# TritonDataCenter/node-zkstream

Measured on AMD Instinct MI355X. Metric: ZK ops/sec (whole node) + p50 get() RTT, 1M-znode synthetic tree, higher is better.
Workload: dtype uint8

## Files before the change

### csrc/kernels/decode.hip

```cpp
#include "zk_common.h"

namespace zk {

constexpr int DEC_T = 256;

ZK_DEV void read_stat_regs(const uint32_t* w, const ZkReplyOut& o, int64_t i) {
  const int64_t c = o.cap;
  auto b32 = [&](int k) { return (int32_t)bswap32(w[k]); };
  auto b64 = [&](int k) {
    return (int64_t)(((uint64_t)bswap32(w[k]) << 32) | bswap32(w[k + 1]));
  };
  o.stat64[0 * c + i] = b64(0);
  o.stat64[1 * c + i] = b64(2);
  o.stat64[2 * c + i] = b64(4);
  o.stat64[3 * c + i] = b64(6);
  o.stat32[0 * c + i] = b32(8);
  o.stat32[1 * c + i] = b32(9);
  o.stat32[2 * c + i] = b32(10);
  o.stat64[4 * c + i] = b64(11);
  o.stat32[3 * c + i] = b32(13);
  o.stat32[4 * c + i] = b32(14);
  o.stat64[5 * c + i] = b64(15);
}

ZK_DEV bool read_stat(const uint8_t* p, const ZkReplyOut& o, int64_t i) {
  const int64_t c = o.cap;
  o.stat64[0 * c + i] = ld_be64(p + 0);
  o.stat64[1 * c + i] = ld_be64(p + 8);
  o.stat64[2 * c + i] = ld_be64(p + 16);
  o.stat64[3 * c + i] = ld_be64(p + 24);
  o.stat32[0 * c + i] = ld_be32(p + 32);
  o.stat32[1 * c + i] = ld_be32(p + 36);
  o.stat32[2 * c + i] = ld_be32(p + 40);
  o.stat64[4 * c + i] = ld_be64(p + 44);
  o.stat32[3 * c + i] = ld_be32(p + 52);
  o.stat32[4 * c + i] = ld_be32(p + 56);
  o.stat64[5 * c + i] = ld_be64(p + 60);
  return true;
}


struct ZkGetCheck {
  const int64_t* idx;
  const int32_t* xid;
  const int32_t* data_len;
  unsigned long long* acc;
  int32_t slots;
  int64_t* tick;
  const uint8_t* slab;
  const int64_t* slot_off;
};
constexpr int CHK_SAMPLE = 16;

ZK_DEV bool wave_bytes_equal(const uint8_t* a, const uint8_t* b, int32_t n,
                             int lane) {
  uint32_t diff = 0;
  for (int32_t o = 16 * lane; o < n; o += 1024) {
    const uintptr_t ua = (uintptr_t)(a + o);
    const uint32_t* wa = (const uint32_t*)(ua & ~(uintptr_t)3);
    const uint32_t sh = (uint32_t)(ua & 3);
    const uint32_t* wb = (const uint32_t*)(b + o);
    uint32_t va[5], vb[4];
#pragma unroll
    for (int q = 0; q < 5; ++q) va[q] = wa[q];
#pragma unroll
    for (int q = 0; q < 4; ++q) vb[q] = wb[q];
    const int32_t rem = n - o;
#pragma unroll
    for (int q = 0; q < 4; ++q) {
      const int32_t keep = rem - 4 * q;
      const uint32_t mask = keep >= 4 ? 0xFFFFFFFFu
                          : keep <= 0 ? 0u : (1u << (8 * keep)) - 1u;
      diff |= (__builtin_amdgcn_alignbyte(va[q + 1], va[q], sh) ^ vb[q]) &
              mask;
    }
  }
  return __ballot(diff != 0) == 0;
}

template <bool CHECK>
__global__ __launch_bounds__(DEC_T) void decode_replies_k(
    const uint8_t* __restrict__ buf, const int64_t* __restrict__ foff,
    const int32_t* __restrict__ flen, const int64_t* __restrict__ n_dev,
    int64_t ncap, const int64_t* __restrict__ xid_tab, int64_t xid_mask,
    ZkReplyOut o, ZkGetCheck chk) {
  const uint32_t nwg = gridDim.x;
  const int64_t i = (int64_t)xcd_remap(blockIdx.x, nwg) * DEC_T + threadIdx.x;
  const bool live = i < ncap && i < *n_dev;
  if (!CHECK && !live) return;
  int64_t good = 0;
  const int64_t salt = CHECK && chk.tick != nullptr ? chk.tick[1] : 0;
  bool samp = false;
  int64_t s_off = 0, s_node = 0;
  int32_t s_len = 0;
  if (live) {
  const uint8_t* p = buf + foff[i];
  const int64_t L = flen[i];
  int32_t status = ST_OK;
  int32_t op = OP_UNKNOWN;
  int64_t poff = -1;
  int32_t plen = 0, a0 = 0, a1 = 0;
  int32_t xid = 0, err = 0;
  int64_t zxid = 0;
  uint32_t hw[4] = {0, 0, 0, 0};
  if (L >= 16) __builtin_memcpy(hw, p, 16);
  const bool tail_ok = L >= 16 + STAT_BYTES;
  uint32_t sw[STAT_BYTES / 4];
  if (L < 16) {
    status = ST_BAD_DECODE;
  } else {
    xid = (int32_t)bswap32(hw[0]);
    zxid = (int64_t)(((uint64_t)bswap32(hw[1]) << 32) | bswap32(hw[2]));
    err = (int32_t)bswap32(hw[3]);
    switch (xid) {
      case XID_NOTIFICATION: op = OP_NOTIFICATION; break;
      case XID_PING: op = OP_PING; break;
      case XID_AUTH: op = OP_AUTH; break;
      case XID_SET_WATCHES: op = OP_SET_WATCHES; break;
      default: {
        const int64_t e = xid_tab[xid & xid_mask];
        if (xid >= 0 && (int32_t)(e >> 32) == xid) op = (int32_t)e;
        else status = ST_NO_XID;
      }
    }
  }
  if (tail_ok) __builtin_memcpy(sw, p + L - STAT_BYTES, STAT_BYTES);
  if (status == ST_OK && err == ERR_OK) {
    const uint8_t* b = p + 16;
    const int64_t A = L - 16;
    switch (op) {
      case OP_GET_DATA: {
        if (A < 4) { status = ST_BAD_DECODE; break; }
        int32_t dl = ld_be32(b);
        if (dl < 0) dl = 0;
        if (4 + (int64_t)dl + STAT_BYTES > A) { status = ST_BAD_DECODE; break; }
        poff = foff[i] + 20;
        plen = dl;
        if (tail_ok && 4 + (int64_t)dl + STAT_BYTES == A) read_stat_regs(sw, o, i);
        else read_stat(b + 4 + dl, o, i);
        break;
      }
      case OP_EXISTS: case OP_SET_DATA:
        if (A < STAT_BYTES) { status = ST_BAD_DECODE; break; }
        if (tail_ok && A == STAT_BYTES) read_stat_regs(sw, o, i);
        else read_stat(b, o, i);
        break;
      case OP_CREATE: {
        if (A < 4) { status = ST_BAD_DECODE; break; }
        int32_t l = ld_be32(b);
        if (l < 0) l = 0;
        if (4 + (int64_t)l > A) { status = ST_BAD_DECODE; break; }
        poff = foff[i] + 20;
        plen = l;
        break;
      }
      case OP_GET_CHILDREN: case OP_GET_CHILDREN2: {
        if (A < 4) { status = ST_BAD_DECODE; break; }
        const int32_t cnt = max(ld_be32(b), 0);
        const int64_t k = skip_strings(b + 4, A - 4, cnt);
        if (k < 0) { status = ST_BAD_DECODE; break; }
        if (op == OP_GET_CHILDREN2 && 4 + k + STAT_BYTES > A) {
          status = ST_BAD_DECODE;
          break;
        }
        poff = foff[i] + 20;
        plen = (int32_t)k;
        a0 = cnt;
        if (op == OP_GET_CHILDREN2) {
          if (tail_ok && 4 + k + STAT_BYTES == A) read_stat_regs(sw, o, i);
          else read_stat(b + 4 + k, o, i);
        }
        break;
      }
      case OP_GET_ACL: {
        if (A < 4) { status = ST_BAD_DECODE; break; }
        const int32_t cnt = max(ld_be32(b), 0);
        const int64_t k = skip_acl(b + 4, A - 4, cnt);
        if (k < 0 || 4 + k + STAT_BYTES > A) { status = ST_BAD_DECODE; break; }
        poff = foff[i] + 20;
        plen = (int32_t)k;
        a0 = cnt;
        if (tail_ok && 4 + k + STAT_BYTES == A) read_stat_regs(sw, o, i);
        else read_stat(b + 4 + k, o, i);
        break;
      }
      case OP_NOTIFICATION: {
        if (A < 12) { status = ST_BAD_DECODE; break; }
        int32_t l = ld_be32(b + 8);
        if (l < 0) l = 0;
        if (12 + (int64_t)l > A) { status = ST_BAD_DECODE; break; }
        a0 = ld_be32(b);
        a1 = ld_be32(b + 4);
        poff = foff[i] + 28;
        plen = l;
        break;
      }
      case OP_PING: case OP_SYNC: case OP_DELETE: case OP_SET_WATCHES:
      case OP_CLOSE_SESSION: case OP_AUTH:
        break;
      default:
        status = ST_BAD_OPCODE;
    }
  }
  o.xid[i] = xid;
  o.err[i] = err;
  o.opcode[i] = op;
  o.zxid[i] = zxid;
  o.status[i] = status;
  o.pay_off[i] = poff;
  o.pay_len[i] = plen;
  o.aux0[i] = a0;
  o.aux1[i] = a1;
  if (CHECK && status == ST_OK && err == ERR_OK && op == OP_GET_DATA) {
    const int64_t v = chk.idx[i];
    good = xid == chk.xid[i] && o.stat64[i] == v + 1 &&
           plen == chk.data_len[v];
    samp = good && chk.slab != nullptr && plen > 0 &&
           ((i + salt) & (CHK_SAMPLE - 1)) == 0;
    s_off = poff;
    s_node = v;
    s_len = plen;
  }
  }
  if (CHECK) {
    uint64_t pend = __ballot(samp);
    const int lane = threadIdx.x & 63;
    while (pend) {
      const int l = (int)__builtin_ctzll(pend);
      pend &= pend - 1;
      const int64_t po = __shfl(s_off, l, 64);
      const int64_t vn = __shfl(s_node, l, 64);
      const int32_t pl = __shfl(s_len, l, 64);
      const bool eq = wave_bytes_equal(
          buf + po, chk.slab + chk.slot_off[vn] + ZK_SLOT_DATA, pl, lane);
      if (lane == l && !eq) good = 0;
    }
    if (chk.tick != nullptr && blockIdx.x == 0 && threadIdx.x == 0)
      chk.tick[1] += 1;
    __shared__ int64_t sm[DEC_T / 64 + 1];
    int64_t tot;
    block_excl_scan(good, sm, &tot);
    if (threadIdx.x == 0 && tot)
      atomicAdd(&chk.acc[blockIdx.x % (uint32_t)chk.slots],
                (unsigned long long)tot);
  }
}

__global__ __launch_bounds__(DEC_T) void expand_strings_k(
    const uint8_t* __restrict__ buf, const int64_t* __restrict__ region,
    const int32_t* __restrict__ count, const int64_t* __restrict__ base,
    int64_t n, int64_t* __restrict__ soff, int32_t* __restrict__ slen) {
  const int64_t i = (int64_t)blockIdx.x * DEC_T + threadIdx.x;
  if (i >= n) return;
  const int32_t c = count[i];
  if (c <= 0 || region[i] < 0) return;
  int64_t k = region[i];
  int64_t w = base[i];
  for (int32_t j = 0; j < c; ++j) {
    int32_t l = ld_be32(buf + k);
    if (l < 0) l = 0;
    soff[w + j] = k + 4;
    slen[w + j] = l;
    k += 4 + l;
  }
}

__global__ __launch_bounds__(DEC_T) void expand_acl_k(
    const uint8_t* __restrict__ buf, const int64_t* __restrict__ region,
    const int32_t* __restrict__ count, const int64_t* __restrict__ base,
    int64_t n, int32_t* __restrict__ perms, int64_t* __restrict__ s_off,
    int32_t* __restrict__ s_len, int64_t* __restrict__ i_off,
    int32_t* __restrict__ i_len) {
  const int64_t i = (int64_t)blockIdx.x * DEC_T + threadIdx.x;
  if (i >= n) return;
  const int32_t c = count[i];
  if (c <= 0 || region[i] < 0) return;
  int64_t k = region[i];
  int64_t w = base[i];
  for (int32_t j = 0; j < c; ++j) {
    perms[w + j] = ld_be32(buf + k);
    k += 4;
    int32_t l = max(ld_be32(buf + k), 0);
    s_off[w + j] = k + 4;
    s_len[w + j] = l;
    k += 4 + l;
    l = max(ld_be32(buf + k), 0);
    i_off[w + j] = k + 4;
    i_len[w + j] = l;
    k += 4 + l;
  }
}

__global__ __launch_bounds__(DEC_T) void decode_requests_k(
    const uint8_t* __restrict__ buf, const int64_t* __restrict__ foff,
    const int32_t* __restrict__ flen, const int64_t* __restrict__ n_dev,
    int64_t ncap, ZkReqOut o) {
  const uint32_t nwg = gridDim.x;
  const int64_t i = (int64_t)xcd_remap(blockIdx.x, nwg) * DEC_T + threadIdx.x;
  if (i >= ncap || i >= *n_dev) return;
  const ReqFields f = parse_request(buf, foff[i], flen[i]);
  o.xid[i] = f.xid;
  o.opcode[i] = f.op;
  o.status[i] = f.status;
  o.path_off[i] = f.poff;
  o.path_len[i] = f.pl;
  o.data_off[i] = f.doff;
  o.data_len[i] = f.dl;
  o.arg[i] = f.arg;
  o.vec_off[i] = f.voff;
  o.vec_count[i] = f.vc;
  o.rel_zxid[i] = f.rel;
}

__global__ __launch_bounds__(DEC_T) void decode_connect_k(
    const uint8_t* __restrict__ buf, const int64_t* __restrict__ foff,
    const int32_t* __restrict__ flen, int64_t n, int32_t* __restrict__ proto,
    int32_t* __restrict__ tmo, int64_t* __restrict__ sid,
    int64_t* __restrict__ pw_off, int32_t* __restrict__ pw_len,
    int32_t* __restrict__ status) {
  const int64_t i = (int64_t)blockIdx.x * DEC_T + threadIdx.x;
  if (i >= n) return;
  const uint8_t* p = buf + foff[i];
  const int64_t L = flen[i];
  int32_t st = ST_OK, pv = 0, to = 0, pl = 0;
  int64_t s = 0, po = -1;
  if (L < 20) {
    st = ST_BAD_DECODE;
  } else {
    pv = ld_be32(p);
    to = ld_be32(p + 4);
    s = ld_be64(p + 8);
    int32_t l = ld_be32(p + 16);
    if (l < 0) l = 0;
    if (20 + (int64_t)l > L) st = ST_BAD_DECODE;
    else { po = foff[i] + 20; pl = l; }
  }
  proto[i] = pv; tmo[i] = to; sid[i] = s; pw_off[i] = po; pw_len[i] = pl;
  status[i] = st;
}

static inline unsigned nblk(int64_t n) {
  return (unsigned)((n + DEC_T - 1) / DEC_T);
}

}

extern "C" {

int zk_decode_replies(const uint8_t* buf, const int64_t* foff,
                      const int32_t* flen, const int64_t* n_dev, int64_t ncap,
                      const int64_t* xid_tab, int64_t xid_mask,
                      const ZkReplyOut* o, hipStream_t st) {
  if (ncap <= 0) return 0;
  zk::decode_replies_k<false><<<zk::nblk(ncap), zk::DEC_T, 0, st>>>(
      buf, foff, flen, n_dev, ncap, xid_tab, xid_mask, *o,
      zk::ZkGetCheck{nullptr, nullptr, nullptr, nullptr, 1, nullptr, nullptr,
                     nullptr});
  ZK_LAUNCH_CHECK();
  return 0;
}

int zk_decode_replies_check(const uint8_t* buf, const int64_t* foff,
                            const int32_t* flen, const int64_t* n_dev,
                            int64_t ncap, const int64_t* xid_tab,
                            int64_t xid_mask, const ZkReplyOut* o,
                            const int64_t* idx, const int32_t* xid,
                            const int32_t* data_len, unsigned long long* acc,
                            int32_t slots, int64_t* tick,
                            const uint8_t* slab, const int64_t* slot_off,
                            hipStream_t st) {
  if (ncap <= 0) return 0;
  if (slots < 1 || slots > 64) return (int)hipErrorInvalidValue;
  if ((slab == nullptr) != (slot_off == nullptr))
    return (int)hipErrorInvalidValue;
  zk::decode_replies_k<true><<<zk::nblk(ncap), zk::DEC_T, 0, st>>>(
      buf, foff, flen, n_dev, ncap, xid_tab, xid_mask, *o,
      zk::ZkGetCheck{idx, xid, data_len, acc, slots, tick, slab, slot_off});
  ZK_LAUNCH_CHECK();
  return 0;
}

int zk_expand_strings(const uint8_t* buf, const int64_t* region,
                      const int32_t* count, const int64_t* base, int64_t n,
                      int64_t* soff, int32_t* slen, hipStream_t st) {
  if (n <= 0) return 0;
  zk::expand_strings_k<<<zk::nblk(n), zk::DEC_T, 0, st>>>(buf, region, count,
                                                          base, n, soff, slen);
  ZK_LAUNCH_CHECK();
  return 0;
}

int zk_expand_acl(const uint8_t* buf, const int64_t* region,
                  const int32_t* count, const int64_t* base, int64_t n,
                  int32_t* perms, int64_t* s_off, int32_t* s_len,
                  int64_t* i_off, int32_t* i_len, hipStream_t st) {
  if (n <= 0) return 0;
  zk::expand_acl_k<<<zk::nblk(n), zk::DEC_T, 0, st>>>(
      buf, region, count, base, n, perms, s_off, s_len, i_off, i_len);
  ZK_LAUNCH_CHECK();
  return 0;
}

int zk_decode_connect_responses(const uint8_t* buf, const int64_t* foff,
                                const int32_t* flen, int64_t n,
                                int32_t* proto, int32_t* tmo, int64_t* sid,
                                int64_t* pw_off, int32_t* pw_len,
                                int32_t* status, hipStream_t st) {
  if (n <= 0) return 0;
  zk::decode_connect_k<<<zk::nblk(n), zk::DEC_T, 0, st>>>(
      buf, foff, flen, n, proto, tmo, sid, pw_off, pw_len, status);
  ZK_LAUNCH_CHECK();
  return 0;
}

int zk_decode_requests(const uint8_t* buf, const int64_t* foff,
                       const int32_t* flen, const int64_t* n_dev,
                       int64_t ncap, const ZkReqOut* o, hipStream_t st) {
  if (ncap <= 0) return 0;
  zk::decode_requests_k<<<zk::nblk(ncap), zk::DEC_T, 0, st>>>(
      buf, foff, flen, n_dev, ncap, *o);
  ZK_LAUNCH_CHECK();
  return 0;
}

}
```

### csrc/kernels/frame_scan.hip

```cpp
#include "zk_common.h"

namespace zk {

constexpr int FT_S = 4096;
constexpr int FT_LMAX = FT_S / 4;
constexpr int FT_STAGE = FT_S + 16;
constexpr int64_t TERM = (int64_t)1 << 62;
constexpr int64_t TBAD = (int64_t)1 << 60;
constexpr int64_t FC_MAXP = (int64_t)1 << 24;
constexpr int FC_WIN = 4096;
constexpr int FL_T = 512;
constexpr int FL_U = 8;
constexpr int FL_NB = 2;
constexpr int FL_GW = FL_NB + 1;
constexpr int FL_BROUNDS = 8;
constexpr int FL_DBG_BLOCKS = 16;
constexpr int FL_DBG_ROWS = 6;
constexpr uint32_t FL_CHASE_WALKS = 16;
constexpr int FK_T = 64;
constexpr int LW_MINS = 4, LW_LAST = 6, LW_NOSPEC = 7, LW_GRID = 8;
constexpr int LW_BIG = 16;
constexpr int LW_END = 32;
static_assert(LW_GRID + FL_GW <= LW_BIG, "grid words");
constexpr unsigned FL_BIG_NOSPEC = 256;
constexpr int FL_GROUNDS = 6;
constexpr uint64_t FT_WAIT_TICKS = 200000;

ZK_DEV int64_t stream_len(const int64_t* n_dev, int64_t n_cap) {
  if (n_dev == nullptr) return n_cap;
  const int64_t v = *n_dev;
  return v < 0 ? 0 : (v < n_cap ? v : n_cap);
}

ZK_DEV uint64_t lb_load(const uint64_t* p) {
  return __hip_atomic_load(p, __ATOMIC_RELAXED, __HIP_MEMORY_SCOPE_AGENT);
}
ZK_DEV void lb_store(uint64_t* p, uint64_t v) {
  __hip_atomic_store(p, v, __ATOMIC_RELAXED, __HIP_MEMORY_SCOPE_AGENT);
}
ZK_DEV int64_t ld_agent(const int64_t* p) {
  return __hip_atomic_load(p, __ATOMIC_RELAXED, __HIP_MEMORY_SCOPE_AGENT);
}
ZK_DEV void st_agent(int64_t* p, int64_t v) {
  __hip_atomic_store(p, v, __ATOMIC_RELAXED, __HIP_MEMORY_SCOPE_AGENT);
}

ZK_DEV void fc_stat(uint64_t* stats, int k, uint32_t v) {
  __hip_atomic_fetch_add((uint32_t*)&stats[k], v, __ATOMIC_RELAXED,
                         __HIP_MEMORY_SCOPE_AGENT);
}

ZK_DEV int32_t lds_be32(const uint8_t* sb, int32_t p) {
  const int32_t a = p & ~3;
  const uint32_t lo = *(const uint32_t*)(sb + a);
  const uint32_t hi = *(const uint32_t*)(sb + a + 4);
  return (int32_t)bswap32(__builtin_amdgcn_alignbyte(hi, lo, p & 3));
}

constexpr int FT_BITS = FT_S / 32;
constexpr int FT_XW = 2048 / 32;

struct FcWalk {
  int64_t exit;
  int32_t cnt;
  int32_t np;
  int32_t js;
  bool term, bad;
};
ZK_DEV int64_t fc_meta(const FcWalk& w) {
  return (int64_t)w.cnt | ((int64_t)w.np << 11) | ((int64_t)(w.js + 1) << 22) |
         ((int64_t)w.term << 33) | ((int64_t)w.bad << 34);
}
ZK_DEV int32_t m_cnt(int64_t m) { return (int32_t)(m & 0x7FF); }
ZK_DEV int32_t m_np(int64_t m) { return (int32_t)((m >> 11) & 0x7FF); }
ZK_DEV int32_t m_js(int64_t m) { return (int32_t)((m >> 22) & 0x7FF) - 1; }
ZK_DEV bool m_term(int64_t m) { return (m >> 33) & 1; }
ZK_DEV bool m_bad(int64_t m) { return (m >> 34) & 1; }
constexpr int64_t M_STALE = (int64_t)1 << 35;
ZK_DEV bool m_stale(int64_t m) { return (m >> 35) & 1; }

ZK_DEV void fc_join_end(FcWalk& r, int64_t send, int64_t n) {
  if (send & TERM) {
    const int64_t q = send & ~(TERM | TBAD);
    if (q >= n && !(send & TBAD)) {
      r.exit = n;
    } else {
      r.exit = q; r.term = true; r.bad = (send & TBAD) != 0;
    }
  } else {
    r.exit = send;
  }
}

template <typename LoadL>
ZK_DEV int32_t fc_member(uint32_t crel, int32_t m0, int32_t& lb, uint32_t& lv,
                         int lane, LoadL loadL) {
  while (lb + 64 < m0 &&
         crel > (uint32_t)__builtin_amdgcn_readlane((int)lv, 63)) {
    lb += 64;
    lv = lb + lane < m0 ? loadL(lb + lane) : 0xFFFFFFFFu;
  }
  const uint64_t hit = __ballot(lv == crel);
  return hit ? lb + (int32_t)__builtin_ctzll(hit) : -1;
}

ZK_DEV void ft_record(uint16_t* L, int32_t& m, uint32_t& ent, int32_t c,
                      int lane) {
  ent = lane == (m & 63) ? (uint32_t)c : ent;
  ++m;
  if ((m & 63) == 0) L[m - 64 + lane] = (uint16_t)ent;
}

constexpr int64_t FC_DEAD = -1;
constexpr int64_t FC_LIVE = -2;
constexpr int CX_SHIFT = 48;
ZK_DEV int64_t cx_exit(int64_t v) {
  return v < 0 ? v : v & (((int64_t)1 << CX_SHIFT) - 1);
}
ZK_DEV int32_t cx_cnt(int64_t v) { return v < 0 ? 0 : (int32_t)(v >> CX_SHIFT); }

ZK_DEV int64_t ft_cand(const uint8_t* sb, const uint32_t* sbits, int32_t e,
                       int32_t nrel, int32_t maxp, int64_t send, int64_t n,
                       int64_t ts, int32_t m, int lane) {
  int32_t c = e;
  int32_t hops = 0;
  for (;;) {
    if (c >= FT_S) return (ts + c) | ((int64_t)hops << CX_SHIFT);
    if (ts + c >= n) return FC_LIVE;
    const uint32_t smw = sbits[c >> 5];
    const int32_t lraw = lds_be32(sb, c);
    if ((smw >> (c & 31)) & 1u) {
      if (send & TERM) return (send & TBAD) ? FC_DEAD : FC_LIVE;
      const int32_t cw = c >> 5;
      int32_t below = 0;
#pragma unroll
      for (int h = 0; h < 2; ++h) {
        const int32_t wi = lane + 64 * h;
        const uint32_t wd = sbits[wi];
        below += wi < cw ? __popc(wd)
                         : (wi == cw ? __popc(wd & ((1u << (c & 31)) - 1u))
                                     : 0);
      }
#pragma unroll
      for (int d = 32; d >= 1; d >>= 1) below += __shfl_xor(below, d, 64);
      return send | ((int64_t)(hops + m - below) << CX_SHIFT);
    }
    if (c + 4 > nrel) return FC_LIVE;
    const int32_t len = __builtin_amdgcn_readfirstlane(lraw);
    if ((uint32_t)len > (uint32_t)maxp) return FC_DEAD;
    const int32_t nx = c + 4 + len;
    if (nx > nrel) return FC_LIVE;
    ++hops;
    c = nx;
  }
}

constexpr int FT_NMAX = 512;
constexpr int FT_SLOTS = 352;
constexpr int32_t FT_LIMIT = FT_S;
enum : uint32_t {
  RK_NODE = 0, RK_EXIT = 1, RK_END = 2, RK_PART = 3, RK_BAD = 4, RK_SHORT = 5
};
// ... 1107 lines not shown
        x0 = y0; x1 = y1; x2 = y2; x3 = y3;
      }
      {
        const bool c = r & 2;
        const uint4 y0 = sel(c, x2, x0), y1 = sel(c, x3, x1),
                    y2 = sel(c, x0, x2), y3 = sel(c, x1, x3);
        x0 = y0; x1 = y1; x2 = y2; x3 = y3;
      }
      d[0] = x0.x; d[1] = x0.y; d[2] = x0.z; d[3] = x0.w;
      d[4] = x1.x; d[5] = x1.y; d[6] = x1.z; d[7] = x1.w;
      d[8] = x2.x; d[9] = x2.y; d[10] = x2.z; d[11] = x2.w;
      d[12] = x3.x; d[13] = x3.y; d[14] = x3.z; d[15] = x3.w;
      const uint32_t nx = (uint32_t)__shfl_down((int)d[0], 1, 64);
      d[16] = lane == 63 ? pad : nx;
    }
    const uint32_t lim = P0 < W ? (uint32_t)(maxp32 - minb + 1)
                         : LONG ? (uint32_t)(FT_LIMIT - minb)
                                : (uint32_t)(W - 3 - minb);
    uint32_t lo = 0, hi = 0;
#pragma unroll
    for (int j = 0; j < 32; ++j) {
      const uint32_t v = (uint32_t)be32_of(d[j >> 2], d[(j >> 2) + 1], j);
      lo |= ((v - (uint32_t)minb) < lim ? 1u : 0u) << j;
    }
#pragma unroll
    for (int j = 32; j < 64; ++j) {
      const uint32_t v = (uint32_t)be32_of(d[j >> 2], d[(j >> 2) + 1], j);
      hi |= ((v - (uint32_t)minb) < lim ? 1u : 0u) << (j - 32);
    }
    uint64_t mask = (uint64_t)hi << 32 | lo;
    const int32_t room = nrel - 4 - P0;
    if (room < 63) mask = room < 0 ? 0 : mask & ((2ull << room) - 1);
    const uint32_t c = (uint32_t)__popcll(mask);
    uint32_t incl = c;
#pragma unroll
    for (int s = 1; s < 64; s <<= 1) {
      const uint32_t y = __shfl_up(incl, s, 64);
      if (lane >= s) incl += y;
    }
    N = __builtin_amdgcn_readlane((int)incl, 63);
    const uint32_t base = incl - c;
    bmask[lane] = mask;
    bbase[lane] = (uint16_t)base;
    if (N <= FT_NMAX) {
      uint32_t k = base;
      uint64_t m = mask;
      while (m) {
        C.pos[k++] = (uint16_t)(P0 + __builtin_ctzll(m));
        m &= m - 1;
      }
    }
  }
  __builtin_amdgcn_wave_barrier();
  C.t_d = dbg ? wall_clock64() : 0;
  C.buf = buf; C.list = list; C.pre = pre; C.sx = sx; C.lbw = lbw;
  C.rec_entry = rec_entry; C.rec_exit = rec_exit; C.rec_meta = rec_meta;
  C.rcount = rcount; C.dbg = dbg; C.cx = cx;
  C.stats = &lbw[2 * ntiles_cap];
  C.n = n; C.t = t; C.ts = ts; C.tend = tend;
  C.nrel = nrel; C.maxp32 = maxp32; C.minb = minb; C.N = N;
  C.nospec = tflags & 1;
  C.misspec = tflags >> 8;
  C.lane = lane;
  static_assert(FT_NMAX == 512, "node buckets");
  if constexpr (G > 1) {
    static_assert(!LONG, "groups: frames within the window");
    if (N <= 128) fs_group_rest<W, 2, G>(C);
    else if (N <= 256) fs_group_rest<W, 4, G>(C);
    else if (N <= FT_NMAX) fs_group_rest<W, 8, G>(C);
    else {
      const int64_t s0 = fs_tile_rest<W, LONG, 1>(C, false);
      FtTileRegs nxt;
      if (t + 1 < (n + FT_S - 1) / FT_S) ft_load(buf, n, ts + FT_S, lane, nxt);
      ft_group_tail<W, G>(C, s0, s0 >= 0, nxt);
    }
  } else {
    if (N <= 128) fs_tile_rest<W, LONG, 2>(C, true);
    else if (N <= 256) fs_tile_rest<W, LONG, 4>(C, true);
    else if (N <= FT_NMAX) fs_tile_rest<W, LONG, 8>(C, true);
    else fs_tile_rest<W, LONG, 1>(C, false);
  }
}


template <int WIN>
ZK_DEV void fc_stage(const uint8_t* __restrict__ buf, int64_t n, int64_t wb,
                     uint8_t* win, int lane) {
  constexpr int PER = WIN / 1024;
  uint4 v[PER];
#pragma unroll
  for (int j = 0; j < PER; ++j) {
    const int64_t g = wb + 16 * (lane + 64 * j);
    v[j] = make_uint4(0, 0, 0, 0);
    if (g + 16 <= n) {
      __builtin_memcpy(&v[j], buf + g, 16);
    } else if (g < n) {
      uint8_t* b = (uint8_t*)&v[j];
      for (int k = 0; k < 16; ++k) b[k] = g + k < n ? buf[g + k] : 0;
    }
  }
#pragma unroll
  for (int j = 0; j < PER; ++j) *(uint4*)(win + 16 * (lane + 64 * j)) = v[j];
  __builtin_amdgcn_wave_barrier();
  asm volatile("s_waitcnt lgkmcnt(0)" ::: "memory");
  __builtin_amdgcn_wave_barrier();
}

template <int WIN = FC_WIN>
ZK_DEV FcWalk fc_walk(const uint8_t* __restrict__ buf, int64_t n,
                      int64_t maxp, int64_t ts, int64_t E, const uint16_t* L,
                      int32_t m0, int64_t send, uint8_t* win, uint16_t* pre,
                      int lane) {
  FcWalk r{E, 0, 0, -1, false, false};
  const int64_t tend = ts + FT_S;
  int64_t c = E;
  int64_t wb = -(int64_t)WIN;
  int32_t lb = 0;
  uint32_t lv = lane < m0 ? (uint32_t)L[lane] : 0xFFFFFFFFu;
  int32_t np = 0;
  for (;;) {
    if (c >= tend) { r.exit = c; break; }
    if (c >= n) { r.exit = n; break; }
    const uint32_t crel = (uint32_t)(c - ts);
    if (m0 > 0) {
      const int32_t j = fc_member(crel, m0, lb, lv, lane,
                                  [&](int i) { return (uint32_t)L[i]; });
      if (j >= 0) { r.js = j; break; }
    }
    if (c + 4 > n) { r.exit = c; r.term = true; break; }
    if (c < wb || c + 8 > wb + WIN) {
      wb = c & ~(int64_t)15;
      fc_stage<WIN>(buf, n, wb, win, lane);
    }
    const int32_t len =
        __builtin_amdgcn_readfirstlane(lds_be32(win, (int32_t)(c - wb)));
    if (len < 0 || (int64_t)len > maxp) {
      r.exit = c; r.term = true; r.bad = true; break;
    }
    const int64_t nx = c + 4 + len;
    if (nx > n) { r.exit = c; r.term = true; break; }
    if (lane == 0) pre[np] = (uint16_t)crel;
    ++np;
    c = nx;
  }
  r.np = np;
  r.cnt = np;
  if (r.js >= 0) {
    r.cnt = np + (m0 - r.js);
    fc_join_end(r, send, n);
  }
  return r;
}

constexpr unsigned long long FL_SMALL = 1024;

ZK_DEV int64_t rfl64(int64_t v) {
  const uint32_t lo = (uint32_t)__builtin_amdgcn_readfirstlane((int)(uint32_t)v);
  const uint32_t hi =
      (uint32_t)__builtin_amdgcn_readfirstlane((int)(uint32_t)((uint64_t)v >> 32));
  return (int64_t)(((uint64_t)hi << 32) | lo);
}

ZK_DEV bool fl_accept(const int64_t* rec_entry, const int64_t* rec_exit,
                      int64_t ntiles, int64_t k, int64_t E, int64_t x) {
  if (ld_agent(&rec_exit[k - 1]) != E) return false;
  if (k < 2) return true;
  const bool suspect = ld_agent(&rec_entry[k - 1]) != ld_agent(&rec_exit[k - 2]);
  if (!suspect) return true;
  const int64_t ox = ld_agent(&rec_exit[k]);
  if (x == ox || k + 1 >= ntiles) return true;
  return ld_agent(&rec_entry[k + 1]) != ox;
}

ZK_DEV uint32_t fl_local_round(const uint8_t* __restrict__ buf, int64_t n,
                               int64_t ntiles, int64_t maxp,
                               const int64_t* __restrict__ sx,
                               const uint16_t* __restrict__ list,
                               const int32_t* __restrict__ rcount,
                               uint16_t* pre, int64_t* rec_entry,
                               int64_t* rec_exit, int64_t* rec_meta,
                               const int32_t* lloc, int nloc, uint8_t* win) {
  const int lane = threadIdx.x & 63, wv = threadIdx.x >> 6;
  uint8_t* mywin = win + (size_t)wv * (FC_WIN + 16);
  uint32_t walked = 0;
  for (int j = wv; j < nloc; j += FL_T / 64) {
    const int64_t k = lloc[j];
    const int64_t E = rfl64(ld_agent(&rec_exit[k - 1]));
    if (E < k * FT_S ||
        __builtin_amdgcn_readfirstlane(m_term(ld_agent(&rec_meta[k - 1]))))
// ... 104 lines not shown
    if (E < k * FT_S) continue;
    const int32_t m0 = __builtin_amdgcn_readfirstlane(rcount[k]);
    const FcWalk fw = fc_walk(buf, n, maxp, k * FT_S, E, list + k * FT_LMAX,
                              m0, sx[k], mywin, pre + k * FT_LMAX, lane);
    ++walked;
    if (lane == 0) {
      if (fl_accept(rec_entry, rec_exit, ntiles, k, E, fw.exit)) {
        st_agent(&rec_entry[k], E);
        st_agent(&rec_exit[k], fw.exit);
        st_agent(&rec_meta[k], fc_meta(fw));
      } else {
        st_agent(&rec_entry[k], -1);
      }
    }
  }
  if (lane == 0 && walked) fc_stat(stats, 2, walked);
  if (bid == 0 && tid == 0) fc_stat(stats, 3, 1);
  return fl_sync(g);
}

ZK_DEV void fl_check(int64_t ntiles, const int64_t* __restrict__ rec_entry,
                     const int64_t* __restrict__ rec_exit,
                     const int64_t* __restrict__ rec_meta, int64_t* base,
                     int64_t* bsum, uint64_t* mins,
                     unsigned long long* nbroken, int32_t* blist) {
  const int lane = threadIdx.x & 63;
  const int64_t INF = INT64_MAX;
  const int64_t nw = (int64_t)gridDim.x * (FL_T / 64);
  const int64_t nbl = (ntiles + FK_T - 1) / FK_T;
  int64_t fb = INF, fterm = INF;
  for (int64_t b = (int64_t)blockIdx.x * (FL_T / 64) + (threadIdx.x >> 6);
       b < nbl; b += nw) {
    const int64_t k = b * FK_T + lane;
    int64_t cnt = 0;
    bool brk = false;
    if (k < ntiles) {
      const int64_t mk = rec_meta[k];
      const bool nxt = k + 1 < ntiles;
      const int64_t e = nxt ? rec_entry[k + 1] : 0;
      const int64_t x = rec_exit[k];
      cnt = m_cnt(mk);
      if (m_term(mk)) {
        fterm = min(fterm, k);
      } else if (nxt && (e < 0 || e != x)) {
        brk = true;
        fb = min(fb, k + 1);
      }
    }
    const uint64_t bm = __ballot(brk);
    if (bm) {
      unsigned long long b0 = 0;
      if (lane == 0) b0 = atomicAdd(nbroken, (unsigned long long)__popcll(bm));
      b0 = __shfl(b0, 0, 64);
      if (brk) {
        const uint64_t below = lane ? (bm & ((~0ull) >> (64 - lane))) : 0ull;
        __hip_atomic_store(&blist[b0 + __popcll(below)], (int32_t)(k + 1),
                           __ATOMIC_RELAXED, __HIP_MEMORY_SCOPE_AGENT);
      }
    }
    int64_t inc = cnt;
#pragma unroll
    for (int d = 1; d < 64; d <<= 1) {
      const int64_t v = __shfl_up(inc, d, 64);
      if (lane >= d) inc += v;
    }
    if (k < ntiles) st_agent(&base[k], inc - cnt);
    if (lane == 63) st_agent(&bsum[b], inc);
  }
  for (int d = 32; d >= 1; d >>= 1) {
    fb = min(fb, (int64_t)__shfl_xor(fb, d, 64));
    fterm = min(fterm, (int64_t)__shfl_xor(fterm, d, 64));
  }
  if (lane == 0) {
    if (fb != INF) atomicMax((unsigned long long*)&mins[0],
                             (unsigned long long)(ntiles - fb));
    if (fterm != INF) atomicMax((unsigned long long*)&mins[1],
                                (unsigned long long)(ntiles - fterm));
  }
}

ZK_DEV void fl_bases(int64_t n, int64_t ntiles, int64_t ft,
                     const int64_t* rec_exit, const int64_t* rec_meta,
                     const int64_t* base, int64_t* bsum, int64_t cap,
                     int64_t* result, int64_t* lastk, int64_t* red) {
  const int tid = threadIdx.x;
  const int64_t INF = INT64_MAX;
  const int64_t last = ft == INF ? ntiles - 1 : ft;
  const int64_t nbl = last / FK_T + 1;
  const int64_t per = (nbl + FL_T - 1) / FL_T;
  const int64_t b0 = (int64_t)tid * per;
  const int64_t b1 = min(b0 + per, nbl);
  int64_t sum = 0;
  for (int64_t b = b0; b < b1; ++b) sum += ld_agent(&bsum[b]);
  int64_t tot;
  int64_t run = block_excl_scan(sum, red, &tot);
  const int64_t blast = last / FK_T;
  for (int64_t b = b0; b < b1; ++b) {
    const int64_t v = ld_agent(&bsum[b]);
    bsum[b] = run;
    if (b == blast) {
      const int64_t ml = ld_agent(&rec_meta[last]);
      const int64_t total = run + ld_agent(&base[last]) + m_cnt(ml);
      *lastk = last;
      result[0] = total;
      result[3] = total > cap ? 1 : 0;
      if (ft == INF) {
        result[1] = n;
        result[2] = 0;
      } else {
        result[1] = ld_agent(&rec_exit[ft]);
        result[2] = m_bad(ml) ? 1 : 0;
      }
    }
    run += v;
  }
}

constexpr int FL_WL = 1024;
constexpr int FL_HS = 2048;
constexpr int FL_WR = 48;
constexpr int FL_DB = 8192;
static_assert(FL_SMALL <= FL_WL, "the check's list fits the first round");

struct FlChase {
  uint32_t* dirty;
  int* overflow;
  uint64_t* stats;
  int64_t* clk;
};

ZK_DEV void fl_dirty(FlChase& ch, int64_t t) {
  const int64_t b = t / FK_T;
  if (b < FL_DB) atomicOr(&ch.dirty[b >> 5], 1u << (b & 31));
}

ZK_DEV int live_count(const int64_t* c5) {
  int live = 0;
#pragma unroll
  for (int j = 0; j < 5; ++j) live += c5[j] != FC_DEAD;
  return live;
}


ZK_DEV uint64_t readlane64(uint64_t v, int l) {
  const uint32_t lo = (uint32_t)__builtin_amdgcn_readlane((int)(uint32_t)v, l);
  const uint32_t hi =
      (uint32_t)__builtin_amdgcn_readlane((int)(uint32_t)(v >> 32), l);
  return ((uint64_t)hi << 32) | lo;
}

ZK_DEV int64_t fl_chase_run(const uint8_t* __restrict__ buf, int64_t n,
                            int64_t ntiles, int64_t maxp,
                            const int64_t* __restrict__ sx,
                            const uint16_t* __restrict__ list,
                            const int32_t* __restrict__ rcount, uint16_t* pre,
                            int64_t* rec_entry, int64_t* rec_exit,
                            int64_t* rec_meta, const uint64_t* lbw,
                            const int64_t* cx,
                            uint8_t* mywin, FlChase& ch, int64_t k0,
                            bool exact, bool& term, uint32_t& walked,
                            uint32_t walk_budget = 0) {
  const int lane = threadIdx.x & 63;
  term = false;
  k0 = rfl64(k0);
  exact = __builtin_amdgcn_readfirstlane((int)exact) != 0;
  int64_t k = k0;
  int64_t E = rfl64(ld_agent(&rec_exit[k - 1]));
  if (E < k * FT_S ||
      __builtin_amdgcn_readfirstlane(m_term(ld_agent(&rec_meta[k - 1]))))
    return -1;
  if (!exact && rfl64(ld_agent(&rec_entry[k])) == E) return -1;
  bool first = true;
  for (;;) {
    if (E >= (k + 1) * FT_S) {
      if (!exact) return k - 1;
      const int64_t kend = min(E / FT_S, ntiles);
      const FcWalk cov{E, 0, 0, -1, false, false};
      for (int64_t c = k + lane; c < kend; c += 64) {
        st_agent(&rec_entry[c], E);
        st_agent(&rec_exit[c], E);
        st_agent(&rec_meta[c], fc_meta(cov));
        fl_dirty(ch, c);
      }
      if (kend >= ntiles) return kend - 1;
      k = kend;
      first = false;
      continue;
    }
    const int64_t tl = k + lane;
    const int64_t ts_l = tl * FT_S;
    uint64_t wd = 0;
    int64_t en = INT64_MIN, ent = INT64_MIN, ox = INT64_MIN + 1;
    int64_t c5[5];
    int32_t n5[5];
#pragma unroll
    for (int j = 0; j < 5; ++j) {
// ... 165 lines not shown
    ++rounds;
    const int nxt = cur ^ 1;
    for (int i = tid; i < FL_HS; i += FL_T) hs[i] = 0;
    if (tid == 0) s_n = 0;
    __syncthreads();
    auto push = [&](int64_t k) {
      const uint32_t key = (uint32_t)k + 1;
      uint32_t h = (key * 2654435761u) >> (32 - 11);
      for (;;) {
        const uint32_t old = atomicCAS(&hs[h], 0u, key);
        if (old == 0) break;
        if (old == key) return;
        h = (h + 1) & (FL_HS - 1);
      }
      const int i = atomicAdd(&s_n, 1);
      if (i < FL_WL) wl[nxt][i] = (int32_t)k;
      else *ch.overflow = 1;
    };
    int32_t lo = INT32_MAX;
    for (int j = lane; j < ncur; j += 64) lo = min(lo, wl[cur][j]);
    for (int d = 32; d >= 1; d >>= 1) lo = min(lo, __shfl_xor(lo, d, 64));
    for (int j = wv; j < ncur; j += FL_T / 64) {
      bool term;
      const bool ex = wl[cur][j] == lo;
      if (ex && ch.clk && lane == 0) ch.clk[6] = wall_clock64();
      const int64_t kend = fl_chase_run(buf, n, ntiles, maxp, sx, list,
                                        rcount, pre, rec_entry, rec_exit,
                                        rec_meta, lbw, cx, mywin,
                                        ch, wl[cur][j], wl[cur][j] == lo,
                                        term, walked);
      if (ex && ch.clk && lane == 0) ch.clk[7] = wall_clock64();
      if (lane == 0)
        wk[j] = kend < 0 ? 0 : (int32_t)(kend + 1) | (term ? (1 << 30) : 0);
    }
    __syncthreads();
    for (int j = tid; j < ncur; j += FL_T) {
      const int64_t k0 = wl[cur][j];
      if (ld_agent(&rec_entry[k0]) != ld_agent(&rec_exit[k0 - 1]) &&
          !m_term(ld_agent(&rec_meta[k0 - 1])))
        push(k0);
      const int32_t e = wk[j];
      if (e == 0 || (e & (1 << 30))) continue;
      const int64_t kend = (e & ((1 << 30) - 1)) - 1;
      if (kend + 1 < ntiles &&
          ld_agent(&rec_entry[kend + 1]) != ld_agent(&rec_exit[kend]))
        push(kend + 1);
    }
    __syncthreads();
    if (tid == 0) s_cur = *ch.overflow ? -1 : s_n;
    __syncthreads();
    ncur = s_cur;
    cur = nxt;
    __syncthreads();
    if (ncur < 0) break;
  }
  if (lane == 0 && walked) fc_stat(stats, 2, walked);
  if (tid == 0 && rounds) fc_stat(stats, 3, rounds);
  return ncur == 0 && !*ch.overflow;
}

ZK_DEV void fl_chase_recount(int64_t ntiles, const int64_t* rec_meta,
                             int64_t* base, int64_t* bsum, FlChase& ch) {
  static_assert(FK_T == 64, "a count block is a wave");
  const int lane = threadIdx.x & 63, wv = threadIdx.x >> 6;
  const int64_t nbl = (ntiles + FK_T - 1) / FK_T;
  for (int64_t b = wv; b < nbl; b += FL_T / 64) {
    if (!((ch.dirty[b >> 5] >> (b & 31)) & 1u)) continue;
    const int64_t k = b * FK_T + lane;
    const int64_t c = k < ntiles ? m_cnt(ld_agent(&rec_meta[k])) : 0;
    int64_t inc = c;
    for (int d = 1; d < 64; d <<= 1) {
      const int64_t v = __shfl_up(inc, d, 64);
      if (lane >= d) inc += v;
    }
    if (k < ntiles) st_agent(&base[k], inc - c);
    if (lane == 63) st_agent(&bsum[b], inc);
  }
  __syncthreads();
}

ZK_DEV void fl_count_scan(int64_t n, int64_t ntiles, int64_t ft,
                          const int64_t* rec_exit, const int64_t* rec_meta,
                          int64_t* base, int64_t* bsum, int64_t cap,
                          int64_t* result, int64_t* lastk, int64_t* red) {
  const int tid = threadIdx.x;
  const int64_t INF = INT64_MAX;
  const int64_t last = ft == INF ? ntiles - 1 : ft;
  const int64_t per = (last + 1 + FL_T - 1) / FL_T;
  const int64_t k0 = (int64_t)tid * per;
  const int64_t k1 = min(k0 + per, last + 1);
  int64_t sum = 0;
  for (int64_t kb = k0; kb < k1; kb += FL_U) {
    int64_t v[FL_U];
#pragma unroll
    for (int u = 0; u < FL_U; ++u)
      v[u] = kb + u < k1 ? ld_agent(&rec_meta[kb + u]) : 0;
#pragma unroll
    for (int u = 0; u < FL_U; ++u) sum += m_cnt(v[u]);
  }
  int64_t tot;
  int64_t run = block_excl_scan(sum, red, &tot);
  for (int64_t kb = k0; kb < k1; kb += FL_U) {
    int64_t v[FL_U];
#pragma unroll
    for (int u = 0; u < FL_U; ++u)
      v[u] = kb + u < k1 ? ld_agent(&rec_meta[kb + u]) : 0;
#pragma unroll
    for (int u = 0; u < FL_U; ++u) {
      if (kb + u < k1) base[kb + u] = run;
      run += m_cnt(v[u]);
    }
  }
  for (int64_t k = last + 1 + tid; k < ntiles; k += FL_T) base[k] = -1;
  for (int64_t b = tid; b <= last / FK_T; b += FL_T) bsum[b] = 0;
  if (tid == 0) {
    *lastk = last;
    result[0] = tot;
    result[3] = tot > cap ? 1 : 0;
    if (ft == INF) {
      result[1] = n;
      result[2] = 0;
    } else {
      const int64_t mf = ld_agent(&rec_meta[ft]);
      result[1] = ld_agent(&rec_exit[ft]);
      result[2] = m_term(mf) && m_bad(mf) ? 1 : 0;
    }
  }
}

ZK_DEV void fl_links(int64_t from, int64_t ntiles,
                     const int64_t* rec_entry, const int64_t* rec_exit,
                     const int64_t* rec_meta, int64_t* red, int64_t& fb_out,
                     int64_t& ft_out) {
  const int tid = threadIdx.x, lane = tid & 63, wv = tid >> 6;
  const int64_t INF = INT64_MAX;
  int64_t fb = INF, fterm = INF;
  for (int64_t k0 = max(from - 1, (int64_t)0) + tid; k0 < ntiles;
       k0 += FL_U * FL_T) {
    int64_t mk[FL_U], e[FL_U], x[FL_U];
#pragma unroll
    for (int u = 0; u < FL_U; ++u) {
      const int64_t k = k0 + (int64_t)u * FL_T;
      const bool in = k < ntiles, nx = k + 1 < ntiles;
      mk[u] = in ? ld_agent(&rec_meta[k]) : 0;
      e[u] = nx ? ld_agent(&rec_entry[k + 1]) : 0;
      x[u] = in ? ld_agent(&rec_exit[k]) : 0;
    }
#pragma unroll
    for (int u = 0; u < FL_U; ++u) {
      const int64_t k = k0 + (int64_t)u * FL_T;
      if (k >= ntiles) break;
      if (m_term(mk[u])) {
        fterm = min(fterm, k);
      } else if (k + 1 < ntiles && k + 1 >= from) {
        if (e[u] < 0 || e[u] != x[u]) fb = min(fb, k + 1);
      }
    }
  }
  for (int d = 32; d >= 1; d >>= 1) {
    fb = min(fb, (int64_t)__shfl_xor(fb, d, 64));
    fterm = min(fterm, (int64_t)__shfl_xor(fterm, d, 64));
  }
  if (lane == 0) { red[wv] = fb; red[FL_T / 64 + wv] = fterm; }
  __syncthreads();
  fb = INF;
  fterm = INF;
  for (int j = 0; j < FL_T / 64; ++j) {
    fb = min(fb, red[j]);
    fterm = min(fterm, red[FL_T / 64 + j]);
  }
  __syncthreads();
  fb_out = fb;
  ft_out = fterm;
}

ZK_DEV int64_t fl_list_broken(int64_t ntiles, const int64_t* rec_entry,
                              const int64_t* rec_exit, const int64_t* rec_meta,
                              int32_t* blist, int64_t* red, int64_t& fb_out,
                              int64_t& ft_out) {
  const int tid = threadIdx.x, lane = tid & 63, wv = tid >> 6;
  const int64_t INF = INT64_MAX;
  const int64_t per = (ntiles + FL_T - 1) / FL_T;
  const int64_t k0 = (int64_t)tid * per, k1 = min(k0 + per, ntiles);
  int64_t cnt = 0, fb = INF, fterm = INF;
  for (int pass = 0; pass < 2; ++pass) {
    int64_t w = 0;
    if (pass == 1) {
      int64_t tot;
      w = block_excl_scan(cnt, red, &tot);
      red[2 * (FL_T / 64) + 1] = tot;
      if (cnt == 0) break;
    }
    for (int64_t kb = k0; kb < k1; kb += FL_U) {
      int64_t mp[FL_U], mk[FL_U], e[FL_U], x[FL_U];
#pragma unroll
      for (int u = 0; u < FL_U; ++u) {
        const int64_t k = kb + u;
        const bool in = k < k1;
        mk[u] = in ? ld_agent(&rec_meta[k]) : 0;
        mp[u] = in && k >= 1 ? ld_agent(&rec_meta[k - 1]) : 0;
        e[u] = in ? ld_agent(&rec_entry[k]) : 0;
        x[u] = in && k >= 1 ? ld_agent(&rec_exit[k - 1]) : 0;
      }
#pragma unroll
      for (int u = 0; u < FL_U; ++u) {
        const int64_t k = kb + u;
        if (k >= k1) break;
        const bool brk = k >= 1 && !m_term(mp[u]) && e[u] != x[u];
        if (pass == 0) {
          if (brk) { ++cnt; fb = min(fb, k); }
          if (m_term(mk[u])) fterm = min(fterm, k);
        } else if (brk) {
          blist[w++] = (int32_t)k;
        }
      }
    }
  }
  __syncthreads();
  const int64_t total = red[2 * (FL_T / 64) + 1];
  __syncthreads();
  for (int d = 32; d >= 1; d >>= 1) {
    fb = min(fb, (int64_t)__shfl_xor(fb, d, 64));
    fterm = min(fterm, (int64_t)__shfl_xor(fterm, d, 64));
  }
  if (lane == 0) { red[wv] = fb; red[FL_T / 64 + wv] = fterm; }
  __syncthreads();
  fb = INF;
  fterm = INF;
  for (int j = 0; j < FL_T / 64; ++j) {
    fb = min(fb, red[j]);
    fterm = min(fterm, red[FL_T / 64 + j]);
  }
  __syncthreads();
  fb_out = fb;
  ft_out = fterm;
  return total;
}

__global__ __launch_bounds__(FL_T) void fs_link(
    const uint8_t* __restrict__ buf, const int64_t* __restrict__ n_dev,
    int64_t n_cap, int64_t maxp, const int64_t* __restrict__ sx,
    const uint16_t* __restrict__ list, const int32_t* __restrict__ rcount,
    uint16_t* pre, int64_t* rec_entry, int64_t* rec_exit, int64_t* rec_meta,
    int64_t* __restrict__ base, int64_t cap, int64_t* __restrict__ result,
    uint64_t* stats, int32_t* __restrict__ blist,
    int64_t* __restrict__ bsum, uint64_t* mins,
    int64_t* __restrict__ lastk, unsigned long long* g,
    const uint64_t* lbw, const int64_t* __restrict__ cx,
    int64_t* __restrict__ ldbg) {
  __shared__ __attribute__((aligned(16)))
      uint8_t win[(FL_T / 64) * (FC_WIN + 16)];
  __shared__ int64_t red[2 * (FL_T / 64) + 2];
  __shared__ int64_t s_next;
  const int tid = threadIdx.x, lane = tid & 63, wv = tid >> 6;
  const int64_t n = stream_len(n_dev, n_cap);
  const int64_t ntiles = (n + FT_S - 1) / FT_S;
  if (ntiles == 0) {
    if (blockIdx.x == 0) {
      if (tid < 4) result[tid] = 0;
      if (tid == 0) *lastk = -1;
    }
    return;
  }
  const int64_t INF = INT64_MAX;
  const int64_t t_in = ldbg != nullptr ? wall_clock64() : 0;
  fl_check(ntiles, rec_entry, rec_exit, rec_meta, base, bsum, mins, &g[FL_NB],
           blist);
  if (ldbg != nullptr && tid == 0 && blockIdx.x < FL_DBG_BLOCKS) {
    ldbg[8 + 2 * blockIdx.x] = t_in;
    ldbg[8 + 2 * blockIdx.x + 1] = wall_clock64();
  }
  const bool big = (uint32_t)ld_agent((const int64_t*)&stats[LW_NOSPEC]) >
                   FL_BIG_NOSPEC;
  if (big) {
    unsigned long long* gb = (unsigned long long*)(stats + LW_BIG);
    bool ok = fl_sync(gb);
    for (int r = 0; r < FL_GROUNDS && ok; ++r)
      ok = fl_round(buf, n, ntiles, maxp, sx, list, rcount, pre, rec_entry,
                    rec_exit, rec_meta, blist, gb, r, red, win, stats);
    if (blockIdx.x != 0) return;
    __syncthreads();
    if (tid == 0) {
      gb[2] = 0;
      for (int r = 0; r < FL_GROUNDS; ++r) gb[4 + 2 * r] = 0;
    }
  }
  __shared__ int s_last;
  __syncthreads();
  if (big) {
    if (tid == 0) s_last = 1;
  } else if (tid == 0) {
    __threadfence();
    const unsigned long long a = __hip_atomic_fetch_add(
        &g[0], 1ull, __ATOMIC_ACQ_REL, __HIP_MEMORY_SCOPE_AGENT);
    const int last = a + 1 == gridDim.x;
    if (last)
      __hip_atomic_store(&g[0], 0ull, __ATOMIC_RELAXED,
                         __HIP_MEMORY_SCOPE_AGENT);
    __threadfence();
    s_last = last;
  }
  __syncthreads();
  if (!s_last) return;
  const uint64_t mb0 = ld_agent((const int64_t*)&mins[0]);
  const uint64_t mt0 = ld_agent((const int64_t*)&mins[1]);
  const unsigned long long nb0 = __hip_atomic_load(
      &g[FL_NB], __ATOMIC_RELAXED, __HIP_MEMORY_SCOPE_AGENT);
  const int64_t fb0 = mb0 ? ntiles - (int64_t)mb0 : INF;
  const int64_t ft0 = mt0 ? ntiles - (int64_t)mt0 : INF;
  if (!big && (fb0 == INF || fb0 > ft0)) {
    if (ldbg != nullptr && tid == 0) ldbg[40] = wall_clock64();
    fl_bases(n, ntiles, ft0, rec_exit, rec_meta, base, bsum, cap, result,
             lastk, red);
    if (ldbg != nullptr && tid == 0) ldbg[41] = wall_clock64();
    return;
  }
  __shared__ uint32_t dirty[FL_DB / 32];
  __shared__ int s_ovf;
  FlChase ch{dirty, &s_ovf, stats, ldbg};
  for (int i = tid; i < FL_DB / 32; i += FL_T) dirty[i] = 0;
  if (tid == 0) s_ovf = 0;
  __syncthreads();
  const bool clk = ldbg != nullptr && tid == 0;
  if (clk) ldbg[5] = t_in;
  int64_t from = 1, ft = INF;
  int64_t nb = (int64_t)nb0;
  bool changed = big;
  if (!big && nb > (int64_t)FL_SMALL && fb0 != INF) {
    if (wv == 0) {
      bool term = false;
      uint32_t walked = 0;
      const int64_t kend = fl_chase_run(buf, n, ntiles, maxp, sx, list, rcount,
                                        pre, rec_entry, rec_exit, rec_meta, lbw,
                                        cx, win, ch, fb0, true, term, walked,
                                        FL_CHASE_WALKS);
      (void)kend;
      if (lane == 0) {
        if (walked) fc_stat(stats, 2, walked);
        fc_stat(stats, 3, 1);
      }
    }
    __syncthreads();
    changed = true;
  }
  for (int round = 0; round < FL_BROUNDS; ++round) {
    if (changed) {
      int64_t fbv, ftv;
      nb = fl_list_broken(ntiles, rec_entry, rec_exit, rec_meta, blist, red,
                          fbv, ftv);
      if (fbv == INF || fbv > ftv) {
        fl_count_scan(n, ntiles, ftv, rec_exit, rec_meta, base, bsum, cap,
                      result, lastk, red);
        if (clk) ldbg[4] = wall_clock64() | (2ll << 56);
        return;
      }
    }
    if (nb <= (int64_t)FL_SMALL && (ntiles + FK_T - 1) / FK_T <= FL_DB) {
      if (clk && round == 0) ldbg[0] = wall_clock64();
      const bool settled = fl_chase(buf, n, ntiles, maxp, sx, list, rcount,
                                    pre, rec_entry, rec_exit, rec_meta, lbw,
                                    cx, blist, (int)nb, win, stats, ch);
      if (clk && round == 0) ldbg[1] = ldbg[2] = wall_clock64();
      int64_t fbv, ftv;
      fl_links(1, ntiles, rec_entry, rec_exit, rec_meta, red, fbv, ftv);
      if (clk && round == 0) ldbg[3] = wall_clock64();
      if (settled && (fbv == INF || fbv > ftv)) {
        if (changed) {
          fl_count_scan(n, ntiles, ftv, rec_exit, rec_meta, base, bsum, cap,
                        result, lastk, red);
          if (clk) ldbg[4] = wall_clock64() | (2ll << 56);
          return;
        }
        fl_chase_recount(ntiles, rec_meta, base, bsum, ch);
        fl_bases(n, ntiles, ftv, rec_exit, rec_meta, base, bsum, cap, result,
                 lastk, red);
        if (clk) ldbg[4] = wall_clock64() | (1ll << 56);
        return;
      }
      if (!settled) break;
    } else {
      const uint32_t w = fl_local_round(buf, n, ntiles, maxp, sx, list,
                                        rcount, pre, rec_entry, rec_exit,
                                        rec_meta, blist, (int)nb, win);
      if (lane == 0 && w) fc_stat(stats, 2, w);
      if (tid == 0) fc_stat(stats, 3, 1);
      __syncthreads();
    }
    changed = true;
  }
  for (;;) {
    int64_t fb, fterm;
    fl_links(from, ntiles, rec_entry, rec_exit, rec_meta, red, fb, fterm);
    if (fb == INF || fb > fterm) {
      ft = fterm;
      break;
    }
    if (wv == 0) {
      bool term = false;
      uint32_t walked = 0;
      const int64_t kend = fl_chase_run(buf, n, ntiles, maxp, sx, list, rcount,
                                        pre, rec_entry, rec_exit, rec_meta, lbw,
                                        cx, win, ch, fb, true, term, walked);
      if (lane == 0) {
        s_next = kend < fb ? -fb : kend + 1;
        if (walked) fc_stat(stats, 2, walked);
        fc_stat(stats, 3, 1);
      }
    }
    __syncthreads();
    from = s_next;
    __syncthreads();
    if (from < 0) {
      ft = -from - 1;
      break;
    }
  }
  fl_count_scan(n, ntiles, ft, rec_exit, rec_meta, base, bsum, cap, result,
                lastk, red);
  if (clk) ldbg[4] = wall_clock64() | (3ll << 56);
}

__global__ __launch_bounds__(256) void fs_rows(
    const uint8_t* __restrict__ buf, const int64_t* __restrict__ n_dev,
    int64_t n_cap, const uint16_t* __restrict__ list,
    const uint16_t* __restrict__ pre, const int64_t* __restrict__ rec_meta,
    const int64_t* __restrict__ rec_entry,
    const int64_t* __restrict__ rec_exit,
    const int64_t* __restrict__ base, const int64_t* __restrict__ bsum,
    const int64_t* __restrict__ lastk, int64_t* __restrict__ foff,
    int32_t* __restrict__ flen, int64_t cap, uint64_t* __restrict__ lbw,
    uint64_t* __restrict__ lbw_tail) {
  __shared__ __attribute__((aligned(16))) uint8_t stage[4][FT_STAGE];
  const int lane = threadIdx.x & 63;
  const int wv = __builtin_amdgcn_readfirstlane((int)(threadIdx.x >> 6));
  const int64_t t = (int64_t)blockIdx.x * 4 + wv;
  const int64_t n = stream_len(n_dev, n_cap);
  if (t == 0) {
    if (lane == 0) {
      lbw_tail[LW_MINS] = 0;
      lbw_tail[LW_MINS + 1] = 0;
      lbw_tail[LW_NOSPEC] = 0;
      lbw_tail[LW_GRID + FL_NB] = 0;
    }
    if (lane < LW_END - LW_BIG) lbw_tail[LW_BIG + lane] = 0;
  }
  if (t * FT_S >= n) return;
  if (lane == 0) {
    lbw[2 * t] = 0;
    lbw[2 * t + 1] = 0;
  }
  if (t > *lastk) return;
  const int64_t b = bsum[t / FK_T] + base[t];
  const int64_t m = rec_meta[t];
  const int64_t x = rec_exit[t];
  const int32_t cnt = m_cnt(m), np = m_np(m), js = m_js(m);
  const int64_t ts = t * FT_S;
  const uint16_t* P = pre + t * FT_LMAX;
  const uint16_t* R = list + t * FT_LMAX + (js < 0 ? 0 : js);
  if (m_stale(m)) {
    uint8_t* sb = stage[wv];
    fc_stage<FT_S>(buf, n, ts, sb, lane);
    if (lane == 0) {
      uint8_t* pb = sb + FT_S;
      for (int k = 0; k < 16; ++k)
        pb[k] = ts + FT_S + k < n ? buf[ts + FT_S + k] : 0;
    }
    __builtin_amdgcn_wave_barrier();
    asm volatile("s_waitcnt lgkmcnt(0)" ::: "memory");
    int32_t c = __builtin_amdgcn_readfirstlane((int32_t)(rec_entry[t] - ts));
    int32_t ent = 0;
    for (int32_t k = 0; k < cnt; ++k) {
      ent = lane == (k & 63) ? c : ent;
      const int32_t len = __builtin_amdgcn_readfirstlane(lds_be32(sb, c));
      c += 4 + len;
      if ((k & 63) == 63 || k == cnt - 1) {
        const int32_t last = k & 63;
        const int32_t nxt = __shfl_down(ent, 1, 64);
        if (lane <= last) {
          const int64_t p = ts + ent;
          const int64_t q = lane < last ? ts + nxt
                                        : (k == cnt - 1 ? x : ts + c);
          const int64_t idx = b + (k & ~63) + lane;
          if (idx < cap) {
            foff[idx] = p + 4;
            flen[idx] = (int32_t)(q - p - 4);
          }
        }
      }
    }
    return;
  }
  for (int32_t k = lane; k < cnt; k += 64) {
    const int64_t p = ts + (k < np ? P[k] : R[k - np]);
    const int32_t k1 = k + 1;
    const int64_t q = k1 < cnt ? ts + (k1 < np ? P[k1] : R[k1 - np]) : x;
    const int64_t idx = b + k;
    if (idx < cap) {
      foff[idx] = p + 4;
      flen[idx] = (int32_t)(q - p - 4);
    }
  }
}

__global__ __launch_bounds__(64) void fs_small(
    const uint8_t* __restrict__ buf, const int64_t* __restrict__ n_dev,
    int64_t n_cap, int64_t maxp, int64_t* __restrict__ foff,
    int32_t* __restrict__ flen, int64_t cap, int64_t* __restrict__ result) {
  __shared__ __attribute__((aligned(16))) uint8_t sb[FT_STAGE];
  const int lane = threadIdx.x;
  const int64_t n = stream_len(n_dev, n_cap);
  fc_stage<FT_S>(buf, n, 0, sb, lane);
  int32_t c = 0, k = 0;
  bool bad = false;
  const int32_t n32 = (int32_t)n;
  while (c + 4 <= n32) {
    const int32_t len = __builtin_amdgcn_readfirstlane(lds_be32(sb, c));
    if (len < 0 || (int64_t)len > maxp) { bad = true; break; }
    if (c + 4 + len > n32) break;
    if (lane == 0 && k < cap) {
      foff[k] = c + 4;
      flen[k] = len;
    }
    ++k;
    c += 4 + len;
  }
  if (lane == 0) {
    result[0] = k;
    result[1] = c;
    result[2] = bad ? 1 : 0;
    result[3] = k > cap ? 1 : 0;
  }
}

struct FsPlan {
  int64_t tiles;
  size_t off_list, off_pre, off_sx, off_lbw, off_rent, off_rexit, off_rmeta,
      off_rcnt, off_base, off_blist, off_bsum, off_cx, total;
};

static FsPlan fs_plan(int64_t n) {
  FsPlan p{};
  const int64_t tiles = n > 0 ? (n + FT_S - 1) / FT_S : 1;
  p.tiles = tiles;
  size_t o = 0;
  auto take = [&](size_t bytes) { size_t r = o; o += (bytes + 255) & ~(size_t)255; return r; };
  p.off_list = take((size_t)tiles * FT_LMAX * 2);
  p.off_pre = take((size_t)tiles * FT_LMAX * 2);
  p.off_sx = take((size_t)tiles * 8);
  p.off_lbw = take((size_t)(2 * tiles + LW_END) * 8);
  p.off_rent = take((size_t)tiles * 8);
  p.off_rexit = take((size_t)tiles * 8);
  p.off_rmeta = take((size_t)tiles * 8);
  p.off_rcnt = take((size_t)tiles * 4);
  p.off_base = take((size_t)tiles * 8);
  p.off_blist = take((size_t)tiles * 4);
  p.off_bsum = take((size_t)(tiles / FK_T + 1) * 8);
  p.off_cx = take((size_t)tiles * 5 * 8);
  p.total = o;
  return p;
}

static unsigned fl_blocks() { return 16; }

static int32_t fs_minb() { return 8; }

constexpr int32_t FS_LONG = 2;

constexpr int32_t FS_WIN_LONG = 1 << 16;

constexpr int FS_TPB = 4;

static int fs_window(int32_t window) {
  window &= FS_WIN_LONG - 1;
  return window <= 256 ? 256 : window <= 512 ? 512
       : window <= 1024 ? 1024 : 2048;
}

static int64_t* g_dbg = nullptr;
static int64_t g_dbg_tiles = 0;
static int64_t* fs_dbg_buf(int64_t tiles) {
  static int on = -1;
  if (on < 0) on = getenv("ZKMI_FS_DBG") != nullptr;
  if (!on) return nullptr;
  if (tiles > g_dbg_tiles) {
    if (g_dbg) (void)hipFree(g_dbg);
    if (hipMalloc(&g_dbg, (tiles + FL_DBG_ROWS) * 8 * 8) != hipSuccess)
      return nullptr;
    (void)hipMemset(g_dbg, 0, (tiles + FL_DBG_ROWS) * 8 * 8);
    g_dbg_tiles = tiles;
  }
  return g_dbg;
}

}

extern "C" {

int64_t zk_frame_scan_workspace(int64_t n) {
  return (int64_t)zk::fs_plan(n).total;
}

int zk_frame_scan(const uint8_t* buf, const int64_t* n_dev, int64_t n_cap,
                  int64_t maxp, uint8_t* ws, int64_t ws_bytes, int64_t* foff,
                  int32_t* flen, int64_t cap, int64_t* result, int32_t window,
                  int32_t clean, int32_t flags, hipStream_t st) {
  using namespace zk;
  const int W = fs_window(window);
  if (window & FS_WIN_LONG) flags |= FS_LONG;
  if (maxp > FC_MAXP || maxp < 0) return -3;
  FsPlan p = fs_plan(n_cap);
  if ((int64_t)p.total > ws_bytes) return -1;
  const int64_t tiles = p.tiles;
  if (n_cap <= FT_S && !(flags & (1 | 0xFFFF00)) &&
      fs_dbg_buf(tiles) == nullptr) {
    fs_small<<<1, 64, 0, st>>>(buf, n_dev, n_cap, maxp, foff, flen, cap,
                               result);
    ZK_LAUNCH_CHECK();
    return 0;
  }
  uint16_t* list = (uint16_t*)(ws + p.off_list);
  uint16_t* pre = (uint16_t*)(ws + p.off_pre);
  int64_t* sx = (int64_t*)(ws + p.off_sx);
  uint64_t* lbw = (uint64_t*)(ws + p.off_lbw);
  int64_t* rent = (int64_t*)(ws + p.off_rent);
  int64_t* rexit = (int64_t*)(ws + p.off_rexit);
  int64_t* rmeta = (int64_t*)(ws + p.off_rmeta);
  int32_t* rcnt = (int32_t*)(ws + p.off_rcnt);
  int64_t* base = (int64_t*)(ws + p.off_base);
  int32_t* blist = (int32_t*)(ws + p.off_blist);
  int64_t* bsum = (int64_t*)(ws + p.off_bsum);
  int64_t* cx = (int64_t*)(ws + p.off_cx);
  uint64_t* mins = lbw + 2 * tiles + LW_MINS;
  int64_t* lastk = (int64_t*)(lbw + 2 * tiles + LW_LAST);
  unsigned long long* grid = (unsigned long long*)(lbw + 2 * tiles + LW_GRID);
  if (!clean &&
      hipMemsetAsync(lbw, 0, (size_t)(2 * tiles + LW_END) * 8, st) !=
          hipSuccess)
    return -4;
  int64_t* dbg = fs_dbg_buf(tiles);
  constexpr int tpb = FS_TPB;
  int G = ((flags >> 4) & 15) + 1;
  if ((flags & (FS_LONG | 1 | 0xFFFF00)) || W > 512) G = 1;
  G = G >= 8 ? 8 : G >= 4 ? 4 : G >= 2 ? 2 : 1;
  const int64_t waves = (tiles + G - 1) / G;
  const unsigned tblocks = (unsigned)((waves + tpb - 1) / tpb);
#define ZK_FS_TILE(WW, LL)                                                   \
  fs_tile<WW, LL, 1><<<tblocks, 64 * tpb, FT_LDS * tpb, st>>>(               \
      buf, n_dev, n_cap, maxp, list, pre, sx, lbw, rent, rexit, rmeta, rcnt, \
      tiles, dbg, fs_minb(), flags, cx)
#define ZK_FS_GROUP(WW, GG)                                                  \
  fs_tile<WW, false, GG><<<tblocks, 64 * tpb, FT_LDS * tpb, st>>>(           \
      buf, n_dev, n_cap, maxp, list, pre, sx, lbw, rent, rexit, rmeta, rcnt, \
      tiles, dbg, fs_minb(), flags, cx)
  if (G == 8) {
    if (W == 256) ZK_FS_GROUP(256, 8);
    else ZK_FS_GROUP(512, 8);
  } else if (G == 4) {
    if (W == 256) ZK_FS_GROUP(256, 4);
    else ZK_FS_GROUP(512, 4);
  } else if (G == 2) {
    if (W == 256) ZK_FS_GROUP(256, 2);
    else ZK_FS_GROUP(512, 2);
  } else if (flags & FS_LONG) {
    switch (W) {
      case 256: ZK_FS_TILE(256, true); break;
      case 512: ZK_FS_TILE(512, true); break;
      case 1024: ZK_FS_TILE(1024, true); break;
      default: ZK_FS_TILE(2048, true); break;
    }
  } else {
    switch (W) {
      case 256: ZK_FS_TILE(256, false); break;
      case 512: ZK_FS_TILE(512, false); break;
      case 1024: ZK_FS_TILE(1024, false); break;
      default: ZK_FS_TILE(2048, false); break;
    }
  }
#undef ZK_FS_TILE
#undef ZK_FS_GROUP
  ZK_LAUNCH_CHECK();
  fs_link<<<fl_blocks(), FL_T, 0, st>>>(buf, n_dev, n_cap, maxp, sx, list, rcnt,
                                 pre, rent, rexit, rmeta, base, cap, result,
                                 lbw + 2 * tiles, blist, bsum, mins, lastk,
                                 grid, lbw, cx, dbg ? dbg + 8 * tiles : nullptr);
  ZK_LAUNCH_CHECK();
  fs_rows<<<(unsigned)((tiles + 3) / 4), 256, 0, st>>>(
      buf, n_dev, n_cap, list, pre, rmeta, rent, rexit, base, bsum, lastk,
      foff, flen, cap, lbw, lbw + 2 * tiles);
  ZK_LAUNCH_CHECK();
  return 0;
}

int zk_frame_scan_stats(const uint8_t* ws, int64_t n_cap, int32_t window,
                        uint32_t* out4, hipStream_t st) {
  using namespace zk;
  (void)window;
  FsPlan p = fs_plan(n_cap);
  const uint64_t* lbw = (const uint64_t*)(ws + p.off_lbw);
  for (int k = 0; k < 4; ++k)
    if (hipMemcpyAsync(out4 + k, lbw + 2 * p.tiles + (k + 1) % 4, 4,
                       hipMemcpyDeviceToHost, st) != hipSuccess)
      return -1;
  if (hipStreamSynchronize(st) != hipSuccess) return -1;
  if (hipMemsetAsync((void*)(lbw + 2 * p.tiles), 0, 4 * 8, st) !=
      hipSuccess)
    return -1;
  return hipStreamSynchronize(st) == hipSuccess ? 0 : -1;
}

int zk_frame_scan_dbg(int64_t* host, int64_t tiles) {
  if (!zk::g_dbg || tiles > zk::g_dbg_tiles + zk::FL_DBG_ROWS) return -1;
  return hipMemcpy(host, zk::g_dbg, tiles * 8 * 8, hipMemcpyDeviceToHost) ==
                 hipSuccess ? 0 : -1;
}

}
```

### csrc/kernels/tree.hip

```cpp
#include "zk_tree.h"

namespace zk {

__global__ __launch_bounds__(TR_T) void tree_fill_k(ZkTree t, int64_t n0,
                                                   int64_t n,
                                                   const int32_t* __restrict__ nkids,
                                                   int64_t now_ms) {
  const int64_t v = n0 + (int64_t)blockIdx.x * TR_T + threadIdx.x;
  if (v >= n) return;
  const ZkNodeStore& s = t.store;
  uint8_t* slot = s.slab + s.slot_off[v];
  const int32_t dl = s.data_len[v];
  fill_stat(slot, v + 1, v + 1, now_ms, now_ms, 0, nkids[v], 0, 0, dl,
            nkids[v], v + 1);
  st_be32(slot + 68, 0);
  st_be32(slot + ZK_SLOT_LEN, dl > 0 ? dl : -1);
  t.cn[v] = cn_pack(nkids[v], nkids[v]);
  t.pzxid[v] = v + 1;
  t.eph[v] = 0;
  t.dirty[v] = 0;
}

__global__ __launch_bounds__(TR_T) void free_count_k(ZkTree t,
                                                    int64_t* __restrict__ bsum) {
  __shared__ int32_t c[TR_T / 64];
  const int64_t nn = min(t.counters[TC_NODES], t.store.cap);
  const int64_t v = (int64_t)blockIdx.x * TR_T + threadIdx.x;
  const bool f = v < nn && t.node_parent[v] == NODE_FREE;
  const uint64_t m = __ballot(f);
  if ((threadIdx.x & 63) == 0) c[threadIdx.x >> 6] = __popcll(m);
  __syncthreads();
  if (threadIdx.x == 0) {
    int64_t s = 0;
    for (int k = 0; k < TR_T / 64; ++k) s += c[k];
    bsum[blockIdx.x] = s;
  }
}

__global__ __launch_bounds__(TR_T) void free_scatter_k(
    ZkTree t, const int64_t* __restrict__ bbase,
    const int64_t* __restrict__ total) {
  __shared__ int32_t c[TR_T / 64];
  const int64_t head = t.counters[TC_FREE_HEAD];
  const int64_t nn = min(t.counters[TC_NODES], t.store.cap);
  const int64_t v = (int64_t)blockIdx.x * TR_T + threadIdx.x;
  const bool f = v < nn && t.node_parent[v] == NODE_FREE;
  const uint64_t m = __ballot(f);
  const int w = threadIdx.x >> 6;
  if ((threadIdx.x & 63) == 0) c[w] = __popcll(m);
  __syncthreads();
  int64_t r = bbase[blockIdx.x] +
              __builtin_amdgcn_mbcnt_hi((uint32_t)(m >> 32),
                                        __builtin_amdgcn_mbcnt_lo((uint32_t)m, 0));
  for (int k = 0; k < w; ++k) r += c[k];
  if (f) t.free_list[(head + r) % t.free_cap] = v;
  if (blockIdx.x == 0 && threadIdx.x == 0) {
    t.counters[TC_FREE_TAIL] = head + *total;
    t.counters[TC_FREE_PUB] = head + *total;
  }
}

__global__ __launch_bounds__(TR_T) void tree_build_k(ZkTree t, int64_t n0,
                                                    int64_t n) {
  const int64_t v = n0 + (int64_t)blockIdx.x * TR_T + threadIdx.x;
  if (v >= n || t.node_parent[v] == NODE_FREE) return;
  tree_insert(t, v, t.path_arena + t.node_path_off[v], t.node_path_len[v],
              t.store.data_len[v]);
}

}

extern "C" {

int zk_tree_fill(const ZkTree* t, int64_t n0, int64_t n, const int32_t* nkids,
                 int64_t now_ms, hipStream_t st) {
  if (n <= n0) return 0;
  const int64_t m = n - n0;
  zk::tree_fill_k<<<(unsigned)((m + zk::TR_T - 1) / zk::TR_T), zk::TR_T, 0,
                    st>>>(*t, n0, n, nkids, now_ms);
  ZK_LAUNCH_CHECK();
  return 0;
}

// ... 45 lines not shown
  int64_t node, zx, par, slot;
  const uint8_t* path;
};

ZK_DEV int64_t served_reply_size(int32_t op, int32_t err, int32_t dl,
                                 int32_t rpl) {
  const int64_t sz = 4 + 16;
  if (err != ERR_OK) return sz;
  switch (op) {
    case OP_GET_DATA: return sz + 4 + max(dl, 0) + STAT_BYTES;
    case OP_EXISTS: case OP_SET_DATA: return sz + STAT_BYTES;
    case OP_CREATE: return sz + 4 + max(rpl, 0);
    default: return sz;
  }
}

ZK_DEV int32_t seq_num(const ZkTree& t, int64_t i) {
  if (t.seqno == nullptr) return -1;
  const int64_t x = t.seqno[i];
  return x < 0 ? -1 : (int32_t)(uint32_t)x;
}
ZK_DEV int64_t seq_par(const ZkTree& t, int64_t i) {
  return t.seqno == nullptr || t.seqno[i] < 0 ? -1 : t.seqno[i] >> 32;
}

ZK_DEV int32_t do_create(const ZkTree& t, Lane& L, const uint8_t* data,
                         int32_t nacl, int64_t session, int64_t now_ms,
                         int64_t v, int64_t i) {
  const ZkNodeStore& s = t.store;
  const bool eph = L.flags & CF_EPHEMERAL, seq = L.flags & CF_SEQUENTIAL;
  const int32_t pre = seq ? seq_num(t, i) : -1;
  if (nacl <= 0) return ERR_INVALID_ACL;
  if (v < 0) return ERR_SYSTEM;
  const int64_t vpo = t.node_path_off[v];
  const int64_t vso = s.slot_off[v];
  const uint8_t* path = L.path;
  const int32_t pl = L.pl;
  int32_t cut = pl - 1;
  while (cut > 0 && path[cut] != '/') --cut;
  const int64_t par = cut > 0 ? tree_find(t, path, cut) : -1;
  if (cut > 0 && par < 0) return ERR_NO_NODE;
  if (par >= 0 && t.eph[par] != 0)
    return ERR_NO_CHILDREN_FOR_EPHEMERALS;
  const int32_t npl = pl + (seq ? 10 : 0);
  const bool taken = seq && par >= 0 && pre < 0;
  const int32_t seqno = !seq || par < 0 ? 0
                        : pre >= 0      ? pre
                                        : cn_cver(cn_add(t, par, 1, 1));
  uint8_t* pd = t.path_arena + vpo;
  copy_bytes(pd, path, pl);
  if (seq) put_seq10(pd + pl, seqno);
  const int32_t dl = L.dl;
  uint8_t* slot = s.slab + vso;
  fill_stat(slot, L.zx, L.zx, now_ms, now_ms, 0, 0, 0, eph ? session : 0, dl,
            0, L.zx);
  st_be32(slot + ZK_SLOT_LEN, dl > 0 ? dl : -1);
  copy_bytes(slot + ZK_SLOT_DATA, data, dl);
  t.node_path_len[v] = npl;
  s.data_len[v] = dl;
  t.cn[v] = 0;
  t.pzxid[v] = L.zx;
  t.node_parent[v] = par;
  t.node_pw[v] = pw_pack(pd - t.path_arena, npl);
  const int64_t ins = pre >= 0 ? tree_insert<true>(t, v, pd, npl, dl, vso)
                               : tree_insert(t, v, pd, npl, dl, vso);
  if (ins != v) {
    if (taken) cn_add(t, par, 0, -1);
    return ins == TREE_INSERT_TIMEOUT ? ERR_SYSTEM : ERR_NODE_EXISTS;
  }
  t.eph[v] = eph ? session : 0;
  if (par >= 0) {
    if (seq) {
      atomicMax((unsigned long long*)&t.pzxid[par], (unsigned long long)L.zx);
    } else {
      parent_touch(t, par, 1, true, L.zx);
    }
  }
  L.par = par;
  L.node = v;
  L.slot = s.slot_off[v];
  return ERR_OK;
}

template <bool PARSE, bool RO = false>
__global__ __launch_bounds__(TR_T) void tree_serve_k(
    ZkTree t, const uint8_t* __restrict__ rx, ZkReqOut q,
    const int64_t* __restrict__ foff, const int32_t* __restrict__ flen,
    const int64_t* __restrict__ n_dev, int64_t ncap, int32_t* __restrict__ r_op,
    int32_t* __restrict__ r_xid, int32_t* __restrict__ r_err,
    int64_t* __restrict__ r_node, int64_t* __restrict__ r_zxid,
    int64_t* __restrict__ r_path_off, int32_t* __restrict__ r_path_len,
    int64_t* __restrict__ r_slot, int64_t* __restrict__ r_sizes,
    int64_t* __restrict__ r_bsum, int64_t session, int64_t now_ms,
    const uint8_t* __restrict__ rank, int32_t pass, int32_t last_pass,
    int64_t snap_base, int64_t snap_cap, int64_t* __restrict__ snap_top,
    int32_t wslot, int64_t* __restrict__ fired) {
  session = sess_of(t, session);
  const uint32_t blk = xcd_remap(blockIdx.x, gridDim.x);
  const int64_t i = (int64_t)blk * TR_T + threadIdx.x;
  const bool in_batch = i < ncap && i < *n_dev;
  const int32_t rb = rank != nullptr && in_batch ? (int32_t)rank[i] : 0;
  const int32_t rk = rb & ORD_RANK;
  const bool live = in_batch && (rk == pass || (last_pass && rk > pass));
  const bool refused = live && rk > pass;
  ReqFields rq{ST_BAD_DECODE, 0, OP_PING, 0, 0, 0, 0, -1, -1, -1, 0};
  if (live) {
    if (PARSE) {
      rq = parse_request(rx, foff[i], flen[i]);
    } else {
      rq.status = q.status[i];
      rq.xid = q.xid[i];
      rq.op = q.opcode[i];
      rq.arg = q.arg[i];
      rq.pl = q.path_len[i];
      rq.dl = q.data_len[i];
      rq.vc = q.vec_count[i];
      rq.poff = q.path_off[i];
      rq.doff = q.data_off[i];
    }
  }
  const bool ok_req = live && !refused && rq.status == ST_OK;
  const ZkNodeStore& s = t.store;
  Lane L;
  L.op = live ? rq.op : OP_PING;
  L.err = refused ? ERR_SYSTEM : (live && !ok_req ? ERR_BAD_ARGUMENTS : ERR_OK);
  L.node = -1;
  L.slot = -1;
  L.dlen = 0;
  L.par = -1;
  L.flags = 0;
  L.path = nullptr;
  L.pl = L.dl = 0;
  if (ok_req) {
    L.path = rx + rq.poff;
    L.pl = rq.pl;
    L.dl = max(rq.dl, 0);
    L.flags = rq.arg;
  }
  const bool write = ok_req && (L.op == OP_CREATE || L.op == OP_SET_DATA ||
                                L.op == OP_DELETE);
  const int64_t zbase = t.counters[TC_ZXID];
  L.zx = write ? zbase + i + 1 : zbase;
  const bool create = !RO && ok_req && L.op == OP_CREATE;
  int64_t v = -1;
  int32_t npl = 0, cap = 0;
  if (create) {
    npl = L.pl + ((L.flags & CF_SEQUENTIAL) ? 10 : 0);
    cap = max(L.dl, 128);
  }
  if (RO && ok_req && L.op != OP_GET_DATA && L.op != OP_EXISTS)
    L.err = ERR_UNIMPLEMENTED;
  if (!RO) {
    const int64_t pub = t.counters[TC_FREE_PUB];
    const int64_t h = block_ticket(&t.counters[TC_FREE_HEAD], create);
    if (create && h < pub) v = t.free_list[h % t.free_cap];
    const bool fresh = create && v < 0;
    const int64_t nv = block_ticket(&t.counters[TC_NODES], fresh);
    if (fresh && nv < s.cap) v = nv;
    const bool new_path = v >= 0 && (fresh || npl > t.node_path_cap[v]);
    const bool new_slot = v >= 0 && (fresh || cap > s.slot_cap[v]);
    const int32_t pcap = (npl + 15) & ~15;
    const int64_t po = wave_bytes(&t.counters[TC_PATH_TOP],
                                  new_path ? pcap : 0);
    const int64_t sb = new_slot ? slot_bytes(cap) : 0;
    const int64_t so = wave_bytes(&t.counters[TC_SLAB_TOP], sb);
    if (new_path) {
      if (po + pcap <= t.path_cap) {
        t.node_path_off[v] = po;
        t.node_path_len[v] = npl;
        t.node_path_cap[v] = pcap;
      } else {
        t.node_path_len[v] = 0;
        t.node_path_cap[v] = 0;
      }
    }
    if (new_slot) {
      if (so + sb <= t.slab_cap) {
        s.slot_off[v] = so;
        s.slot_cap[v] = cap;
      } else {
        s.slot_cap[v] = -1;
      }
    }
    if (v >= 0 && ((new_path && po + pcap > t.path_cap) ||
                   (new_slot && so + sb > t.slab_cap))) {
      L.err = ERR_SYSTEM;
    }
  }
  int64_t freed = -1;
  bool numbered = !RO && live && seq_num(t, i) >= 0;
  if (ok_req && L.err == ERR_OK) {
// ... 73 lines not shown
      default:
        L.err = ERR_UNIMPLEMENTED;
    }
  }
  if (numbered) cn_add(t, seq_par(t, i), 0, -1);
  if (t.wt_key != nullptr && ok_req) {
    const bool wflag = rq.arg == 1;
    if (L.op == OP_GET_DATA && wflag && L.err == ERR_OK) {
      wt_arm(t, L.path, L.pl, WK_DATA, wslot);
    } else if (L.op == OP_EXISTS && wflag &&
               (L.err == ERR_OK || L.err == ERR_NO_NODE)) {
      wt_arm(t, L.path, L.pl, WK_DATA, wslot);
    } else if (L.err == ERR_OK && (L.op == OP_SET_DATA ||
                                   L.op == OP_CREATE ||
                                   L.op == OP_DELETE)) {
      const int64_t node = L.op == OP_DELETE ? freed : L.node;
      const int64_t pw = t.node_pw[node];
      const int64_t ppw = L.par >= 0 ? t.node_pw[L.par] : 0;
      const uint8_t* np = node_path(t, pw);
      const int32_t nl = pw_len(pw);
      uint64_t m0 = wt_fire(t, np, nl, WK_DATA), m1 = 0, m2 = 0;
      if (L.op == OP_DELETE) m1 = wt_fire(t, np, nl, WK_CHILD) & ~m0;
      if (L.op != OP_SET_DATA && L.par >= 0)
        m2 = wt_fire(t, node_path(t, ppw), pw_len(ppw), WK_CHILD);
      if (fired != nullptr) {
        int64_t* f = fired + (int64_t)WT_REC * i;
        f[0] = (int64_t)m0;
        f[1] = (int64_t)m1;
        f[2] = (int64_t)m2;
        f[3] = pw;
        f[4] = ppw;
      }
    }
  }
  if (rank != nullptr) {
    const bool snap = (rb & ORD_SNAP) && live && L.err == ERR_OK &&
                      (L.op == OP_GET_DATA || L.op == OP_EXISTS ||
                       L.op == OP_SET_DATA);
    const int64_t dl = snap && L.op == OP_GET_DATA ? L.dlen : 0;
    const int64_t sb = snap ? slot_bytes((int32_t)dl) : 0;
    const int64_t so = wave_bytes(snap_top, sb);
    if (snap) {
      if (so + sb <= snap_cap) {
        copy_bytes(s.slab + snap_base + so, s.slab + L.slot,
                   (int32_t)(ZK_SLOT_DATA + dl));
        L.slot = snap_base + so;
      } else {
        L.err = ERR_SYSTEM;
      }
    }
  }
  if (create && L.err != ERR_OK && v >= 0) freed = v;
  if (!RO) {
    wave_free(t, freed);
    wave_mark_dirty(t, L.err == ERR_OK ? L.par : -1);
  }
  if (r_sizes != nullptr) {
    __shared__ int64_t sm[TR_T / 64 + 1];
    int64_t sz = 0;
    if (live) {
      const bool get = L.err == ERR_OK && L.op == OP_GET_DATA;
      const bool mk = L.err == ERR_OK && L.op == OP_CREATE;
      sz = served_reply_size(L.op, L.err, get ? L.dlen : 0,
                             mk ? t.node_path_len[L.node] : 0);
      r_sizes[i] = sz;
    } else if (in_batch && rk < pass) {
      sz = r_sizes[i];
    } else if (!in_batch && i < ncap) {
      r_sizes[i] = 0;
    }
    int64_t tot;
    block_excl_scan(sz, sm, &tot);
    if (threadIdx.x == 0) r_bsum[blk] = tot;
  }
  if (!live) return;
  r_op[i] = L.op;
  r_xid[i] = rq.xid;
  r_err[i] = L.err;
  r_node[i] = L.op == OP_DELETE ? -1 : L.node;
  r_zxid[i] = L.zx;
  if (r_slot != nullptr) r_slot[i] = L.op == OP_DELETE ? -1 : L.slot;
}

int serve_launch(const ServeLaunch& s, hipStream_t st) {
  if (s.ncap <= 0) return 0;
  const ZkServeOut& o = *s.out;
  if ((o.sizes == nullptr) != (o.block_sums == nullptr)) return -1;
  const bool parse = s.q == nullptr;
  const auto k = !parse        ? tree_serve_k<false>
                 : s.read_only ? tree_serve_k<true, true>
                               : tree_serve_k<true>;
  k<<<(unsigned)((s.ncap + TR_T - 1) / TR_T), TR_T, 0, st>>>(
      *s.tree, s.rx, parse ? ZkReqOut{} : *s.q, s.foff, s.flen, s.n_dev,
      s.ncap, o.opcode, o.xid, o.err, o.node, o.zxid, o.path_off, o.path_len,
      o.slot, o.sizes, o.block_sums, s.session, s.now_ms, s.rank, s.pass,
      s.last_pass, s.snap_base, s.snap_cap, s.snap_top, s.wslot, s.fired);
  ZK_LAUNCH_CHECK();
  return 0;
}

}

extern "C" {

int zk_tree_serve(const ZkTree* t, const uint8_t* rx, const ZkReqOut* q,
                  const int64_t* n_dev, int64_t ncap, const ZkServeOut* out,
                  int64_t session, int64_t now_ms, hipStream_t st) {
  if (ncap <= 0) return 0;
  zk::ServeLaunch s;
  s.tree = t, s.rx = rx, s.q = q, s.n_dev = n_dev, s.ncap = ncap;
  s.out = out, s.session = session, s.now_ms = now_ms;
  const int rc = zk::serve_launch(s, st);
  return rc ? rc : zk::finish_launch(t, n_dev, 0, 1, st);
}

int zk_tree_serve_frames(const ZkTree* t, const uint8_t* rx,
                         const int64_t* foff, const int32_t* flen,
                         const int64_t* n_dev, int64_t ncap,
                         const ZkServeOut* out, int64_t session,
                         int64_t now_ms, int32_t wslot, int64_t* fired,
                         int32_t read_only, hipStream_t st) {
  zk::ServeLaunch s;
  s.tree = t, s.rx = rx, s.foff = foff, s.flen = flen, s.n_dev = n_dev;
  s.ncap = ncap, s.out = out, s.session = session, s.now_ms = now_ms;
  s.wslot = wslot, s.fired = fired, s.read_only = read_only;
  return zk::serve_launch(s, st);
}

}

namespace zk {

constexpr int FIN_T = 1024;

ZK_DEV void finish_body(const ZkTree& t, const int64_t* n_dev,
                        int64_t bump_zxid, int32_t publish) {
  int64_t* c = t.counters;
  const int64_t nd = __hip_atomic_load(&c[TC_DIRTY], __ATOMIC_RELAXED,
                                       __HIP_MEMORY_SCOPE_AGENT);
  for (int64_t k = threadIdx.x; k < nd; k += blockDim.x) {
    const int64_t p = __hip_atomic_load(&t.dirty_list[k], __ATOMIC_RELAXED,
                                        __HIP_MEMORY_SCOPE_AGENT);
    uint8_t* slot = t.store.slab + t.store.slot_off[p];
    const int64_t cn = __hip_atomic_load(&t.cn[p], __ATOMIC_RELAXED,
                                         __HIP_MEMORY_SCOPE_AGENT);
    st_be32(slot + 36, cn_cver(cn));
    st_be32(slot + 56, cn_nchild(cn));
    st_be64(slot + 60, __hip_atomic_load(&t.pzxid[p], __ATOMIC_RELAXED,
                                         __HIP_MEMORY_SCOPE_AGENT));
    t.dirty[p] = 0;
  }
  __syncthreads();
  if (threadIdx.x != 0) return;
  auto ld = [&](int k) {
    return __hip_atomic_load(&c[k], __ATOMIC_RELAXED, __HIP_MEMORY_SCOPE_AGENT);
  };
  if (publish) {
    if (ld(TC_FREE_HEAD) > ld(TC_FREE_PUB)) c[TC_FREE_HEAD] = ld(TC_FREE_PUB);
    c[TC_FREE_PUB] = ld(TC_FREE_TAIL);
  }
  c[TC_DIRTY] = 0;
  c[TC_ZXID] = ld(TC_ZXID) + (n_dev != nullptr ? *n_dev : bump_zxid);
}

template <int NT = FIN_T>
__global__ __launch_bounds__(NT) void tree_finish_k(ZkTree t,
                                                   const int64_t* n_dev,
                                                   int64_t bump_zxid,
                                                   int32_t publish) {
  finish_body(t, n_dev, bump_zxid, publish);
}

template <int NT>
__global__ __launch_bounds__(NT) void tree_finish_scan_k(
    ZkTree t, const int64_t* n_dev, int64_t bump_zxid, int32_t publish,
    const int64_t* __restrict__ bsum, int64_t nb, int64_t* __restrict__ bbase,
    int64_t* __restrict__ total) {
  if (blockIdx.x == 0) {
    finish_body(t, n_dev, bump_zxid, publish);
    return;
  }
  constexpr int FS_V = 8;
  __shared__ int64_t sm[NT / 64 + 1];
  int64_t carry = 0;
  for (int64_t c0 = 0; c0 < nb; c0 += (int64_t)NT * FS_V) {
    const int64_t b = c0 + (int64_t)threadIdx.x * FS_V;
    int64_t v[FS_V];
    int64_t s = 0;
#pragma unroll
    for (int j = 0; j < FS_V; ++j) {
      v[j] = b + j < nb ? bsum[b + j] : 0;
      s += v[j];
    }
    int64_t tot;
    int64_t p = carry + block_excl_scan(s, sm, &tot);
#pragma unroll
    for (int j = 0; j < FS_V; ++j) {
      if (b + j < nb) bbase[b + j] = p;
      p += v[j];
    }
    carry += tot;
  }
  if (threadIdx.x == 0) *total = carry;
}

template <bool DBG>
__global__ __launch_bounds__(TR_T) void tree_expire_k(
    ZkTree t, int64_t session, int64_t ncap,
// ... 155 lines not shown
```

### csrc/kernels/zk_abi.h

```cpp
#pragma once
#include <hip/hip_runtime_api.h>
#include <stddef.h>
#include <stdint.h>

extern "C" {


struct ZkReqBatch {
  const int32_t* opcode;
  const int32_t* xid;
  const int32_t* arg;
  const int64_t* path_off;
  const int32_t* path_len;
  const int64_t* data_off;
  const int32_t* data_len;
  const int32_t* acl_id;
  const uint8_t* path_arena;
  const uint8_t* data_arena;
  const int64_t* acl_off;
  const int32_t* acl_len;
  const uint8_t* acl_arena;
};

struct ZkNodeStore {
// ... 22 lines not shown

struct ZkReplyOut {
  int32_t* xid;
  int32_t* err;
  int32_t* opcode;
  int32_t* status;
  int64_t* zxid;
  int64_t* stat64;
  int32_t* stat32;
  int64_t* pay_off;
  int32_t* pay_len;
  int32_t* aux0;
  int32_t* aux1;
  int64_t cap;
};

struct ZkReqOut {
  int32_t* xid;
  int32_t* opcode;
  int32_t* status;
  int64_t* path_off;
  int32_t* path_len;
  int64_t* data_off;
  int32_t* data_len;
  int32_t* arg;
  int64_t* vec_off;
  int32_t* vec_count;
  int64_t* rel_zxid;
  int64_t cap;
};

struct ZkServeOut {
  int32_t *opcode, *xid, *err;
  int64_t *node, *zxid, *path_off;
  int32_t* path_len;
  int64_t *slot, *sizes, *block_sums;
};

struct ZkTree {
  int64_t* ht;
  int64_t mask;
  int64_t* node_path_off;
  int32_t* node_path_len;
  int64_t* node_parent;
  uint8_t* path_arena;
  int64_t path_cap;
  int64_t slab_cap;
  int64_t* counters;
  ZkNodeStore store;
  int64_t* free_list;
  int64_t free_cap;
  int64_t* cn;
  int64_t* pzxid;
  int32_t* dirty;
  int64_t* dirty_list;
  int64_t* node_pw;
  int32_t* node_path_cap;
  int64_t* eph;
  int64_t* wt_key;
  unsigned long long* wt_mask;
  int64_t wt_hmask;
  const int64_t* seqno;
};

struct ZkSessionTable {
  int64_t* sid;
  uint8_t* passwd;
  int32_t* timeout;
  int32_t* state;
  int64_t* next;
  int64_t cap;
  int64_t span;
};

struct ZkAclTable {
  int64_t* node_acl;
  int64_t cap;
  uint8_t* arena;
  int64_t arena_cap;
  int64_t* key;
  int64_t* val;
  int64_t hmask;
  int64_t* ctr;
};

int64_t zk_scan_workspace(int64_t n);
int zk_scan_set_mode(int mode);
int zk_scan_small_i64_mode(const int64_t*, int64_t*, int64_t, int64_t*, int,
                           hipStream_t);
int zk_scan_excl_i64(const int64_t*, int64_t*, int64_t, int64_t*, int64_t*,
                     hipStream_t);
int zk_scan_excl_i32(const int32_t*, int64_t*, int64_t, int64_t*, int64_t*,
                     hipStream_t);
int zk_encode_requests(const ZkReqBatch*, int64_t, int64_t*, int64_t*,
                       int64_t*, int64_t*, uint8_t*, int64_t, int64_t*,
                       int64_t, int32_t*, int32_t, hipStream_t);
int zk_encode_requests_presized(const ZkReqBatch*, int64_t, const int64_t*,
                                const int64_t*, int64_t*, int64_t*, int64_t*,
                                uint8_t*, int64_t, int64_t*, int64_t,
                                int32_t*, int32_t, hipStream_t);
int zk_encode_set_watches(const int64_t*, const int32_t*, const uint8_t*,
                          int64_t, int64_t, int64_t, int64_t, int64_t*,
                          int64_t*, int64_t*, int64_t*, uint8_t*, int64_t,
                          int32_t*, hipStream_t);
int zk_encode_connect_requests(const int32_t*, const int64_t*, const int32_t*,
                               const int64_t*, const int64_t*, const int32_t*,
                               const uint8_t*, int64_t, int64_t*, int64_t*,
                               int64_t*, int64_t*, uint8_t*, hipStream_t);
int zk_encode_responses(const ZkRespBatch*, const ZkNodeStore*,
                        const int64_t*, int64_t, int64_t*, int64_t*,
                        int64_t*, int64_t*, uint8_t*, int64_t, int32_t*,
                        int32_t, int32_t, hipStream_t);
int64_t zk_frame_scan_workspace(int64_t n);
int zk_frame_scan(const uint8_t*, const int64_t*, int64_t, int64_t,
                  uint8_t*, int64_t, int64_t*, int32_t*, int64_t, int64_t*,
                  int32_t, int32_t, int32_t, hipStream_t);
int zk_frame_scan_stats(const uint8_t*, int64_t, int32_t, uint32_t*,
                        hipStream_t);
int zk_frame_scan_dbg(int64_t* host, int64_t tiles);
int zk_decode_replies(const uint8_t*, const int64_t*, const int32_t*,
                      const int64_t*, int64_t, const int64_t*, int64_t,
                      const ZkReplyOut*, hipStream_t);
int zk_decode_replies_check(const uint8_t*, const int64_t*, const int32_t*,
                            const int64_t*, int64_t, const int64_t*, int64_t,
                            const ZkReplyOut*, const int64_t*, const int32_t*,
                            const int32_t*, unsigned long long*, int32_t,
                            int64_t*, const uint8_t*, const int64_t*,
                            hipStream_t);
int zk_expand_strings(const uint8_t*, const int64_t*, const int32_t*,
                      const int64_t*, int64_t, int64_t*, int32_t*,
                      hipStream_t);
int zk_expand_acl(const uint8_t*, const int64_t*, const int32_t*,
                  const int64_t*, int64_t, int32_t*, int64_t*, int32_t*,
                  int64_t*, int32_t*, hipStream_t);
int zk_decode_requests(const uint8_t*, const int64_t*, const int32_t*,
                       const int64_t*, int64_t, const ZkReqOut*, hipStream_t);
int zk_decode_connect_responses(const uint8_t*, const int64_t*,
                                const int32_t*, int64_t, int32_t*, int32_t*,
                                int64_t*, int64_t*, int32_t*, int32_t*,
                                hipStream_t);
int zk_tree_fill(const ZkTree*, int64_t, int64_t, const int32_t*, int64_t,
                 hipStream_t);
int zk_tree_build(const ZkTree*, int64_t, int64_t, hipStream_t);
int zk_tree_ht_reset(const ZkTree*, hipStream_t);
int64_t zk_tree_free_workspace(int64_t cap);
int zk_tree_free_compact(const ZkTree*, int64_t*, hipStream_t);
int zk_tree_serve(const ZkTree*, const uint8_t*, const ZkReqOut*,
                  const int64_t*, int64_t, const ZkServeOut*, int64_t,
                  int64_t, hipStream_t);
int zk_tree_serve_frames(const ZkTree*, const uint8_t*, const int64_t*,
                         const int32_t*, const int64_t*, int64_t,
                         const ZkServeOut*, int64_t, int64_t, int32_t,
                         int64_t*, int32_t, hipStream_t);
int zk_tree_finish_scan(const ZkTree*, const int64_t*, int64_t, int32_t,
                        int64_t, int64_t*, int64_t*, hipStream_t);
int zk_tree_serve_ordered(const ZkTree*, const uint8_t*, const ZkReqOut*,
                          const int64_t*, int64_t, const ZkServeOut*, int64_t,
                          int64_t, uint8_t*, int64_t, int32_t, int64_t,
                          int64_t, int32_t, int64_t*, hipStream_t);
int zk_watch_events(const int32_t*, const int32_t*, const int64_t*, int64_t,
                    const int64_t*, int64_t*, int64_t, int32_t*, int32_t*,
                    int64_t*, int32_t*, int64_t*, hipStream_t);
int zk_watch_resume(const ZkTree*, const uint8_t*, const int64_t*,
                    const int32_t*, const int64_t*, int64_t, int32_t,
                    int64_t*, int64_t, int64_t, int32_t*, int64_t*, int32_t*,
                    int64_t*, hipStream_t);
int64_t zk_tree_order_workspace(int64_t);
int64_t zk_tree_order_stats_offset(int64_t);
int zk_tree_expire(const ZkTree*, int64_t, int64_t, unsigned long long*,
                   hipStream_t);
int64_t zk_tree_seq_workspace(int64_t ncap);
int64_t zk_tree_seq_zeroed(int64_t ncap);
void zk_tree_seq_debug(int64_t* buf);
void zk_tree_expire_debug(int32_t* buf);
int zk_tree_seq_order(const ZkTree*, const uint8_t*, const int64_t*,
                      const int32_t*, const int64_t*, int64_t, uint8_t*,
                      int64_t, int64_t*, hipStream_t);
int zk_tree_digest(const ZkTree*, unsigned long long*, hipStream_t);
int64_t zk_tree_list_workspace(int64_t ncap);
int zk_tree_list(const ZkTree*, const uint8_t*, const int64_t*,
                 const int32_t*, const int64_t*, int64_t, int32_t, int64_t,
                 int32_t*, uint8_t*, int64_t, uint8_t*, int64_t, int64_t*,
                 int64_t*, int32_t*, int32_t, hipStream_t);
int64_t zk_tree_acl_workspace(int64_t ncap);
int zk_tree_acl_record(const ZkAclTable*, const uint8_t*, const int64_t*,
                       const int32_t*, const int64_t*, int64_t,
                       const int32_t*, const int32_t*, const int64_t*,
                       uint8_t*, int64_t, hipStream_t);
int zk_tree_acl_get(const ZkTree*, const ZkAclTable*, const uint8_t*,
                    const int64_t*, const int32_t*, const int64_t*, int64_t,
                    uint8_t*, int64_t, uint8_t*, int64_t, int64_t*, int64_t*,
                    int32_t*, int32_t, hipStream_t);
int zk_bench_gen_get(int64_t, uint64_t, int64_t, int64_t, int32_t,
                     const int64_t*, int64_t*, int32_t*, int64_t*, int32_t*,
                     const int64_t*, int64_t*, int64_t*, hipStream_t);
int zk_bench_xids(int64_t, const int64_t*, int32_t*, hipStream_t);
int zk_bench_storm_hs(int32_t, int32_t, int32_t, const int32_t*,
                      const int64_t*, const int32_t*, const int32_t*,
                      const int64_t*, const uint8_t*, const int64_t*,
                      int64_t*, uint8_t*, bool*, hipStream_t);
int zk_bench_check_writes(int64_t, const int32_t*, const int32_t*,
                          const int32_t*, const int32_t*, const int32_t*,
                          const int32_t*, int32_t, const int64_t*,
                          unsigned long long*, unsigned long long*,
                          hipStream_t);
int zk_bench_check_get(int64_t, const int32_t*, const int32_t*,
                       const int32_t*, const int32_t*, const int64_t*,
                       const int32_t*, const int64_t*, const int32_t*,
                       const int32_t*, unsigned long long*, hipStream_t);
int zk_bench_check_notif(int64_t, int64_t, const uint64_t*, const int64_t*,
                         int64_t, int64_t,
                         const int64_t*, const int32_t*, const uint8_t*,
                         const uint8_t*, const int32_t*, const int32_t*,
                         const int32_t*, const int32_t*, const int32_t*,
                         const int64_t*, const int32_t*, unsigned long long*,
                         hipStream_t);
int64_t zk_route_workspace(int64_t n, int32_t world);
int zk_route_requests(int64_t, int32_t, int32_t, const int64_t*,
                      const int32_t*, const uint8_t*, const int64_t*,
                      const int32_t*, int32_t*, int64_t*, int32_t*, int64_t*,
                      int32_t*, int64_t*, int64_t*, hipStream_t);
int zk_seg_pack(const uint8_t*, int64_t, const int64_t*, const int64_t*,
                int64_t, const int64_t*, const int64_t*, int32_t, int32_t,
                int64_t, uint8_t*, unsigned long long*, uint8_t*, int32_t,
                hipStream_t);
int zk_seg_unpack(const uint8_t*, int32_t, int32_t, int64_t, uint8_t*,
                  int64_t*, int64_t*, unsigned long long*, const uint8_t*,
                  int32_t, hipStream_t);
int zk_session_connect(const uint8_t*, const int64_t*, const int32_t*,
                       const int64_t*, int64_t, const ZkSessionTable*,
                       int64_t, uint64_t, int32_t, int32_t, const int64_t*,
                       uint8_t*, int64_t*, int32_t*, hipStream_t);
int zk_session_close(const ZkSessionTable*, const int64_t*, int64_t,
                     int64_t, hipStream_t);
int zk_session_install(const ZkSessionTable*, const int64_t*, int64_t,
                       int64_t, hipStream_t);
int zk_scan_small_i64(const int64_t*, int64_t*, int64_t, int64_t*,
                      hipStream_t);
}

static_assert(sizeof(void*) == 8, "LP64 only");
static_assert(sizeof(ZkReqBatch) == 13 * 8, "ZkReqBatch layout");
static_assert(sizeof(ZkNodeStore) == 5 * 8, "ZkNodeStore layout");
static_assert(sizeof(ZkRespBatch) == 10 * 8, "ZkRespBatch layout");
static_assert(sizeof(ZkReplyOut) == 12 * 8, "ZkReplyOut layout");
static_assert(sizeof(ZkReqOut) == 12 * 8, "ZkReqOut layout");
static_assert(sizeof(ZkServeOut) == 10 * 8, "ZkServeOut layout");
static_assert(sizeof(ZkSessionTable) == 7 * 8, "ZkSessionTable layout");
static_assert(sizeof(ZkAclTable) == 8 * 8, "ZkAclTable layout");
static_assert(offsetof(ZkAclTable, arena) == 2 * 8, "ZkAclTable.arena");
static_assert(offsetof(ZkAclTable, hmask) == 6 * 8, "ZkAclTable.hmask");
static_assert(sizeof(ZkTree) == 27 * 8, "ZkTree layout");
static_assert(offsetof(ZkTree, store) == 9 * 8, "ZkTree.store");
static_assert(offsetof(ZkTree, free_list) == 14 * 8, "ZkTree.free_list");
static_assert(offsetof(ZkTree, wt_hmask) == 25 * 8, "ZkTree.wt_hmask");
static_assert(offsetof(ZkRespBatch, slot) == 9 * 8, "ZkRespBatch.slot");
static_assert(offsetof(ZkReplyOut, cap) == 11 * 8, "ZkReplyOut.cap");
static_assert(offsetof(ZkReqOut, rel_zxid) == 10 * 8, "ZkReqOut.rel_zxid");
```

### csrc/kernels/zk_tree.h

```cpp
#pragma once
#include "zk_common.h"

namespace zk {

constexpr int TR_T = 256;
enum : int {
  TC_NODES = 0, TC_ZXID = 1, TC_PATH_TOP = 2, TC_SLAB_TOP = 3,
  TC_FREE_HEAD = 4, TC_FREE_TAIL = 5, TC_FREE_PUB = 6, TC_DIRTY = 7,
  TC_SESS = 8, TC_N = 9
};
constexpr int64_t SESS_DEV = -2;
ZK_DEV int64_t sess_of(const ZkTree& t, int64_t session) {
  return session == SESS_DEV ? t.counters[TC_SESS] : session;
}
constexpr int64_t NODE_FREE = -2;

constexpr int32_t ORD_RANK = 0x7f, ORD_SNAP = 0x80;

ZK_DEV int64_t slot_bytes(int32_t data_cap) {
  return ZK_SLOT_DATA + (((int64_t)data_cap + 15) & ~(int64_t)15) + 4;
}

ZK_DEV int lane_id() {
  return __builtin_amdgcn_mbcnt_hi(~0u, __builtin_amdgcn_mbcnt_lo(~0u, 0));
// ... 432 lines not shown
}

ZK_DEV uint64_t wt_fire(const ZkTree& t, const uint8_t* p, int32_t n,
                        int kind) {
  if (t.wt_key == nullptr) return 0;
  const int64_t s = wt_slot(t, path_hash(p, n) | 1ull, false);
  if (s < 0) return 0;
  unsigned long long* m = &t.wt_mask[2 * s + kind];
  if (__hip_atomic_load(m, __ATOMIC_RELAXED, __HIP_MEMORY_SCOPE_AGENT) == 0)
    return 0;
  return atomicExch(m, 0ull);
}

ZK_DEV const uint8_t* node_path(const ZkTree& t, int64_t pw) {
  return t.path_arena + (pw >> 24);
}
ZK_DEV int32_t pw_len(int64_t pw) { return (int32_t)(pw & 0xFFFFFF); }

ZK_DEV void fill_stat(uint8_t* st, int64_t cz, int64_t mz, int64_t ct,
                      int64_t mt, int32_t ver, int32_t cver, int32_t aver,
                      int64_t owner, int32_t dlen, int32_t nkids, int64_t pz) {
  st_be64(st + 0, cz); st_be64(st + 8, mz); st_be64(st + 16, ct);
  st_be64(st + 24, mt); st_be32(st + 32, ver); st_be32(st + 36, cver);
  st_be32(st + 40, aver); st_be64(st + 44, owner); st_be32(st + 52, dlen);
  st_be32(st + 56, nkids); st_be64(st + 60, pz);
}

ZK_DEV int64_t cn_pack(int32_t cver, int32_t nchild) {
  return (int64_t)((uint64_t)(uint32_t)cver << 32 | (uint32_t)nchild);
}
ZK_DEV int32_t cn_cver(int64_t x) { return (int32_t)((uint64_t)x >> 32); }
ZK_DEV int32_t cn_nchild(int64_t x) { return (int32_t)(uint32_t)x; }
ZK_DEV int64_t cn_add(const ZkTree& t, int64_t v, int32_t dc, int32_t dk) {
  return (int64_t)atomicAdd((unsigned long long*)&t.cn[v],
                            (unsigned long long)(((int64_t)dc << 32) + dk));
}

ZK_DEV void parent_touch(const ZkTree& t, int64_t par, int32_t dkids,
                         bool bump_cver, int64_t zx) {
  cn_add(t, par, bump_cver ? 1 : 0, dkids);
  atomicMax((unsigned long long*)&t.pzxid[par], (unsigned long long)zx);
}

ZK_DEV void wave_mark_dirty(const ZkTree& t, int64_t par) {
  bool first = false;
  if (par >= 0 && __hip_atomic_load(&t.dirty[par], __ATOMIC_RELAXED,
                                    __HIP_MEMORY_SCOPE_AGENT) == 0)
    first = atomicExch(&t.dirty[par], 1) == 0;
  const int64_t k = block_ticket(&t.counters[TC_DIRTY], first);
  if (first) t.dirty_list[k] = par;
}

ZK_DEV void wave_free(const ZkTree& t, int64_t v,
                      unsigned long long* count = nullptr) {
  if (v >= 0) t.node_parent[v] = NODE_FREE;
  const int64_t k = block_ticket(&t.counters[TC_FREE_TAIL], v >= 0, count);
  if (v >= 0) t.free_list[k % t.free_cap] = v;
}

ZK_DEV void wave_mark_dirty_at(const ZkTree& t, int64_t par, int32_t flag) {
  const bool first = par >= 0 && flag == 0 && atomicExch(&t.dirty[par], 1) == 0;
  const int64_t k = block_ticket(&t.counters[TC_DIRTY], first);
  if (first) t.dirty_list[k] = par;
}


struct ServeLaunch {
  const ZkTree* tree = nullptr;
  const uint8_t* rx = nullptr;
  const ZkReqOut* q = nullptr;
  const int64_t* foff = nullptr;
  const int32_t* flen = nullptr;
  const int64_t* n_dev = nullptr;
  int64_t ncap = 0;
  const ZkServeOut* out = nullptr;
  int64_t session = 0, now_ms = 0;
  const uint8_t* rank = nullptr;
  int32_t pass = 0, last_pass = 1;
  int64_t snap_base = 0, snap_cap = 0;
  int64_t* snap_top = nullptr;
  int32_t wslot = -1;
  int64_t* fired = nullptr;
  int32_t read_only = 0;
};
int serve_launch(const ServeLaunch& s, hipStream_t st);

int finish_launch(const ZkTree* t, const int64_t* n_dev, int64_t bump,
                  int32_t publish, hipStream_t st);

int bscan_launch(int64_t* bsum, int64_t nb, hipStream_t st);

}
```

### csrc/torch/zkmi_ops.cpp

```cpp
#include <ATen/ATen.h>
#include <c10/hip/HIPStream.h>
#include <torch/library.h>

#include <cstdint>
#include <string>
#include <vector>

#include "../kernels/zk_abi.h"


namespace {

using at::Tensor;
using c10::ScalarType;

hipStream_t cur_stream() { return c10::hip::getCurrentHIPStream().stream(); }

void hip_ok(int rc, const char* what) {
  TORCH_CHECK(rc == 0, "zkmi: ", what, " failed (hip error ", rc, ")");
}

const char* dtname(ScalarType t) { return c10::toString(t); }

template <typename T>
// ... 373 lines not shown
                int64_t window, bool clean, int64_t flags) {
  TORCH_CHECK(n_cap >= 0 && n_cap <= buf.numel(),
              "zkmi: frame_scan length ", n_cap, " past the buffer (",
              buf.numel(), " bytes)");
  TORCH_CHECK(ws.numel() >= zk_frame_scan_workspace(n_cap),
              "zkmi: frame_scan workspace too small");
  const int64_t cap = foff.numel();
  hip_ok(zk_frame_scan(
             P<uint8_t>(buf, U8, 1, "buf"),
             Popt<int64_t>(n_dev, I64, 1, "n", &buf), n_cap, max_packet,
             P<uint8_t>(ws, U8, 1, "ws", &buf), ws.numel(),
             P<int64_t>(foff, I64, 1, "frame_off", &buf),
             P<int32_t>(flen, I32, cap, "frame_len", &buf), cap,
             P<int64_t>(result, I64, 4, "result", &buf), (int32_t)window,
             clean ? 1 : 0, (int32_t)flags, cur_stream()),
         "frame_scan");
}

std::vector<int64_t> frame_scan_stats(const Tensor& ws, int64_t n_cap,
                                      int64_t window) {
  uint32_t o[4] = {0, 0, 0, 0};
  hip_ok(zk_frame_scan_stats(P<uint8_t>(ws, U8, 1, "ws"), n_cap,
                             (int32_t)window, o, cur_stream()),
         "frame_scan_stats");
  return {o[0], o[1], o[2], o[3]};
}

Tensor frame_scan_dbg(int64_t tiles) {
  Tensor out = at::zeros({tiles, 8}, at::kLong);
  hip_ok(zk_frame_scan_dbg(out.data_ptr<int64_t>(), tiles), "frame_scan_dbg");
  return out;
}

void decode_replies(const Tensor& buf, const Tensor& foff, const Tensor& flen,
                    const Tensor& n_dev, const Tensor& xid_tab,
                    int64_t xid_mask, const std::vector<Tensor>& out) {
  const int64_t cap = foff.numel();
  ZkReplyOut o = reply_out(out, cap, &buf);
  hip_ok(zk_decode_replies(
             P<uint8_t>(buf, U8, 1, "buf"),
             P<int64_t>(foff, I64, cap, "frame_off", &buf),
             P<int32_t>(flen, I32, cap, "frame_len", &buf),
             P<int64_t>(n_dev, I64, 1, "count", &buf), cap,
             P<int64_t>(xid_tab, I64, xid_mask + 1, "xid_tab", &buf),
             xid_mask, &o, cur_stream()),
         "decode_replies");
}

void decode_replies_check(const Tensor& buf, const Tensor& foff,
                          const Tensor& flen, const Tensor& n_dev,
                          const Tensor& xid_tab, int64_t xid_mask,
                          const std::vector<Tensor>& out, const Tensor& idx,
                          const Tensor& xid, const Tensor& data_len,
                          const Tensor& acc,
                          const c10::optional<Tensor>& tick,
                          const c10::optional<Tensor>& slab,
                          const c10::optional<Tensor>& slot_off) {
  const int64_t cap = foff.numel();
  ZkReplyOut o = reply_out(out, cap, &buf);
  const int32_t slots = (int32_t)std::min<int64_t>(acc.numel(), 64);
  TORCH_CHECK(slots >= 1, "zkmi: decode_replies_check needs an acc slot");
  TORCH_CHECK(slab.has_value() == slot_off.has_value(),
              "zkmi: decode_replies_check: slab and slot_off go together");
  if (slot_off.has_value())
    TORCH_CHECK(slot_off->numel() >= data_len.numel(),
                "zkmi: decode_replies_check: slot_off shorter than data_len");
  hip_ok(zk_decode_replies_check(
             P<uint8_t>(buf, U8, 1, "buf"),
             P<int64_t>(foff, I64, cap, "frame_off", &buf),
             P<int32_t>(flen, I32, cap, "frame_len", &buf),
             P<int64_t>(n_dev, I64, 1, "count", &buf), cap,
             P<int64_t>(xid_tab, I64, xid_mask + 1, "xid_tab", &buf),
             xid_mask, &o, P<int64_t>(idx, I64, cap, "idx", &buf),
             P<int32_t>(xid, I32, cap, "xid", &buf),
             P<int32_t>(data_len, I32, 1, "data_len", &buf),
             reinterpret_cast<unsigned long long*>(
                 P<int64_t>(acc, I64, slots, "acc", &buf)),
             slots, Popt<int64_t>(tick, I64, 2, "tick", &buf),
             Popt<uint8_t>(slab, U8, 1, "slab", &buf),
             Popt<int64_t>(slot_off, I64, 1, "slot_off", &buf), cur_stream()),
         "decode_replies_check");
}

void expand_strings(const Tensor& buf, const Tensor& region,
                    const Tensor& count, const Tensor& base,
                    const Tensor& soff, const Tensor& slen) {
  const int64_t n = region.numel();
  hip_ok(zk_expand_strings(
             P<uint8_t>(buf, U8, 1, "buf"),
             P<int64_t>(region, I64, n, "region", &buf),
             P<int32_t>(count, I32, n, "count", &buf),
             P<int64_t>(base, I64, n, "base", &buf), n,
             P<int64_t>(soff, I64, 1, "str_off", &buf),
             P<int32_t>(slen, I32, soff.numel(), "str_len", &buf),
             cur_stream()),
         "expand_strings");
}

void expand_acl(const Tensor& buf, const Tensor& region, const Tensor& count,
                const Tensor& base, const Tensor& perms, const Tensor& so,
                const Tensor& sl, const Tensor& io, const Tensor& il) {
  const int64_t n = region.numel();
  const int64_t m = perms.numel();
  hip_ok(zk_expand_acl(
             P<uint8_t>(buf, U8, 1, "buf"),
             P<int64_t>(region, I64, n, "region", &buf),
             P<int32_t>(count, I32, n, "count", &buf),
             P<int64_t>(base, I64, n, "base", &buf), n,
             P<int32_t>(perms, I32, 1, "perms", &buf),
             P<int64_t>(so, I64, m, "scheme_off", &buf),
             P<int32_t>(sl, I32, m, "scheme_len", &buf),
             P<int64_t>(io, I64, m, "id_off", &buf),
             P<int32_t>(il, I32, m, "id_len", &buf), cur_stream()),
         "expand_acl");
}

void decode_requests(const Tensor& buf, const Tensor& foff,
                     const Tensor& flen, const Tensor& n_dev,
                     const std::vector<Tensor>& out) {
  const int64_t cap = foff.numel();
  ZkReqOut o = req_out(out, cap, &buf);
  hip_ok(zk_decode_requests(
             P<uint8_t>(buf, U8, 1, "buf"),
             P<int64_t>(foff, I64, cap, "frame_off", &buf),
             P<int32_t>(flen, I32, cap, "frame_len", &buf),
             P<int64_t>(n_dev, I64, 1, "count", &buf), cap, &o,
             cur_stream()),
         "decode_requests");
}

void decode_connect_responses(const Tensor& buf, const Tensor& foff,
                              const Tensor& flen, int64_t n,
                              const Tensor& proto, const Tensor& tmo,
                              const Tensor& sid, const Tensor& pw_off,
                              const Tensor& pw_len, const Tensor& status) {
  const int64_t m = std::max<int64_t>(n, 1);
  hip_ok(zk_decode_connect_responses(
             P<uint8_t>(buf, U8, 1, "buf"),
             P<int64_t>(foff, I64, n, "frame_off", &buf),
             P<int32_t>(flen, I32, n, "frame_len", &buf), n,
             P<int32_t>(proto, I32, m, "proto", &buf),
             P<int32_t>(tmo, I32, m, "timeout", &buf),
             P<int64_t>(sid, I64, m, "sid", &buf),
             P<int64_t>(pw_off, I64, m, "passwd_off", &buf),
             P<int32_t>(pw_len, I32, m, "passwd_len", &buf),
             P<int32_t>(status, I32, m, "status", &buf), cur_stream()),
         "decode_connect_responses");
}

void tree_fill(const std::vector<Tensor>& t, int64_t n0, int64_t n,
               const Tensor& nkids, int64_t now_ms) {
  ZkTree s = tree(t);
  TORCH_CHECK(n0 >= 0 && n <= s.store.cap, "zkmi: tree_fill range");
  hip_ok(zk_tree_fill(&s, n0, n, P<int32_t>(nkids, I32, n, "nkids", &t[0]),
                      now_ms, cur_stream()),
         "tree_fill");
}

int64_t tree_free_workspace(int64_t cap) {
  return zk_tree_free_workspace(cap);
}

void tree_free_compact(const std::vector<Tensor>& t, const Tensor& ws) {
  ZkTree s = tree(t);
  hip_ok(zk_tree_free_compact(
             &s, P<int64_t>(ws, I64, zk_tree_free_workspace(s.store.cap),
                            "ws", &t[0]),
             cur_stream()),
         "tree_free_compact");
}

void tree_finish_scan(const std::vector<Tensor>& t,
                      const c10::optional<Tensor>& n_dev, int64_t bump,
                      bool publish, int64_t ncap, const Tensor& ws,
                      const Tensor& total) {
  ZkTree s = tree(t);
  const int64_t nb = (ncap + 255) / 256;
  hip_ok(zk_tree_finish_scan(&s, Popt<int64_t>(n_dev, I64, 1, "count", &t[0]),
                             bump, publish ? 1 : 0, ncap,
                             P<int64_t>(ws, I64, 2 * nb, "ws", &t[0]),
                             P<int64_t>(total, I64, 1, "total", &t[0]),
                             cur_stream()),
         "tree_finish_scan");
}

void tree_ht_reset(const std::vector<Tensor>& t) {
  ZkTree s = tree(t);
  hip_ok(zk_tree_ht_reset(&s, cur_stream()), "tree_ht_reset");
}

void tree_build(const std::vector<Tensor>& t, int64_t n0, int64_t n) {
  ZkTree s = tree(t);
  TORCH_CHECK(n0 >= 0 && n <= s.store.cap, "zkmi: tree_build range");
  hip_ok(zk_tree_build(&s, n0, n, cur_stream()), "tree_build");
}

void tree_serve(const std::vector<Tensor>& t, const Tensor& rx,
                const std::vector<Tensor>& q, const Tensor& n_dev,
                int64_t ncap, const std::vector<Tensor>& r, int64_t session,
                int64_t now_ms) {
  ZkTree s = tree(t);
  const Tensor* d = &t[0];
  ZkReqOut qo = req_out(q, ncap, d);
  ZkServeOut ro = serve_out(r, ncap, d);
  hip_ok(zk_tree_serve(&s, P<uint8_t>(rx, U8, 1, "rx", d), &qo,
                       P<int64_t>(n_dev, I64, 1, "count", d), ncap, &ro,
                       session, now_ms, cur_stream()),
         "tree_serve");
}

void tree_serve_frames(const std::vector<Tensor>& t, const Tensor& rx,
                       const Tensor& foff, const Tensor& flen,
                       const Tensor& n_dev, int64_t ncap,
                       const std::vector<Tensor>& r, int64_t session,
                       int64_t now_ms, int64_t wslot,
                       const c10::optional<Tensor>& fired,
                       const c10::optional<Tensor>& seqno, bool read_only) {
  ZkTree s = tree(t);
  const Tensor* d = &t[0];
  ZkServeOut ro = serve_out(r, ncap, d);
  s.seqno = Popt<int64_t>(seqno, I64, ncap, "seqno", d);
  TORCH_CHECK(wslot >= -1 && wslot < 64, "zkmi: watcher slot -1..63");
  hip_ok(zk_tree_serve_frames(
             &s, P<uint8_t>(rx, U8, 1, "rx", d),
             P<int64_t>(foff, I64, ncap, "frame_off", d),
             P<int32_t>(flen, I32, ncap, "frame_len", d),
             P<int64_t>(n_dev, I64, 1, "count", d), ncap, &ro, session,
             now_ms, (int32_t)wslot, Popt<int64_t>(fired, I64, 5 * ncap, "fired", d),
             read_only ? 1 : 0, cur_stream()),
         "tree_serve_frames");
}

int64_t tree_order_workspace(int64_t n) {
  TORCH_CHECK(n >= 0, "zkmi: tree_order_workspace n");
  return zk_tree_order_workspace(n);
}

int64_t tree_order_stats_offset(int64_t n) {
  TORCH_CHECK(n >= 0, "zkmi: tree_order_stats_offset n");
  return zk_tree_order_stats_offset(n);
}

void tree_serve_ordered(const std::vector<Tensor>& t, const Tensor& rx,
                        const std::vector<Tensor>& q, const Tensor& n_dev,
                        int64_t ncap, const std::vector<Tensor>& r,
                        int64_t session, int64_t now_ms, const Tensor& ws,
                        int64_t passes, const c10::optional<Tensor>& scratch,
                        int64_t wslot, const c10::optional<Tensor>& fired,
                        const c10::optional<Tensor>& seqno) {
  TORCH_CHECK(wslot >= -1 && wslot < 64, "zkmi: watcher slot -1..63");
  ZkTree s = tree(t);
  const Tensor* d = &t[0];
  s.seqno = Popt<int64_t>(seqno, I64, ncap, "seqno", d);
  ZkReqOut qo = req_out(q, ncap, d);
  ZkServeOut ro = serve_out(r, ncap, d);
  TORCH_CHECK(passes >= 1 && passes <= 127, "zkmi: passes in 1..127");
  const int64_t need_ws = zk_tree_order_workspace(ncap);
  uint8_t* w = P<uint8_t>(ws, U8, need_ws, "order workspace", d);
  int64_t snap_base = 0, snap_cap = 0;
  if (scratch.has_value() && scratch->defined()) {
    const Tensor& sc = *scratch;
    P<uint8_t>(sc, U8, 0, "scratch", d);
    TORCH_CHECK(sc.storage().is_alias_of(t[6].storage()),
                "zkmi: scratch must be a view of the tree's slab");
    snap_base = (int64_t)((const uint8_t*)sc.data_ptr() -
                          (const uint8_t*)t[6].data_ptr());
    TORCH_CHECK(snap_base >= s.slab_cap && snap_base % 16 == 0,
                "zkmi: scratch must start 16-aligned past the tree's slab");
    snap_cap = sc.numel();
  }
  hip_ok(zk_tree_serve_ordered(
             &s, P<uint8_t>(rx, U8, 1, "rx", d), &qo,
             P<int64_t>(n_dev, I64, 1, "count", d), ncap, &ro, session,
             now_ms, w, ws.numel(), (int32_t)passes, snap_base, snap_cap,
             (int32_t)wslot, Popt<int64_t>(fired, I64, 5 * ncap, "fired", d),
             cur_stream()),
         "tree_serve_ordered");
}

void watch_events(const Tensor& r_op, const Tensor& r_err, const Tensor& n_dev,
                  int64_t ncap, const Tensor& fired, const Tensor& bsum,
                  const Tensor& ev_slot, const Tensor& ev_type,
                  const Tensor& ev_poff, const Tensor& ev_plen,
                  const Tensor& ev_total) {
  const Tensor* d = &r_op;
  const int64_t cap = ev_slot.numel();
  hip_ok(zk_watch_events(
             P<int32_t>(r_op, I32, ncap, "r.opcode"),
             P<int32_t>(r_err, I32, ncap, "r.err", d),
             P<int64_t>(n_dev, I64, 1, "count", d), ncap,
             P<int64_t>(fired, I64, 5 * ncap, "fired", d),
             P<int64_t>(bsum, I64, (ncap + 255) / 256, "bsum", d), cap,
             P<int32_t>(ev_slot, I32, cap, "ev_slot", d),
             P<int32_t>(ev_type, I32, cap, "ev_type", d),
             P<int64_t>(ev_poff, I64, cap, "ev_path_off", d),
             P<int32_t>(ev_plen, I32, cap, "ev_path_len", d),
             P<int64_t>(ev_total, I64, 2, "ev_total", d), cur_stream()),
         "watch_events");
}

void watch_resume(const std::vector<Tensor>& t, const Tensor& rx,
                  const Tensor& foff, const Tensor& flen, const Tensor& n_dev,
                  int64_t ncap, int64_t wslot, const Tensor& ent,
                  const Tensor& ev_type, const Tensor& ev_poff,
                  const Tensor& ev_plen, const Tensor& out) {
  ZkTree s = tree(t);
  TORCH_CHECK(s.wt_key != nullptr, "zkmi: watch_resume needs a watch table");
  TORCH_CHECK(wslot >= 0 && wslot < 64, "zkmi: watcher slot 0..63");
  const Tensor* d = &t[0];
  const int64_t cap = ev_type.numel();
  hip_ok(zk_watch_resume(
             &s, P<uint8_t>(rx, U8, 1, "rx", d),
             P<int64_t>(foff, I64, ncap, "frame_off", d),
// ... 402 lines not shown
  ZkSessionTable s = session_table(tab, span);
  TORCH_CHECK(server_id >= 1 && server_id < 128 &&
                  (span == 0 || server_id * span <= s.cap),
              "zkmi: session_connect server_id out of range for the span");
  const Tensor* r = &buf;
  hip_ok(zk_session_connect(
             P<uint8_t>(buf, U8, 1, "buf"),
             P<int64_t>(foff, I64, ncap, "frame_off", r),
             P<int32_t>(flen, I32, ncap, "frame_len", r),
             P<int64_t>(n_dev, I64, 1, "count", r), ncap, &s, server_id,
             (uint64_t)secret, (int32_t)min_to, (int32_t)max_to,
             P<int64_t>(zxid_now, I64, 1, "zxid_now", r),
             P<uint8_t>(out, U8, 41 * ncap, "out", r),
             P<int64_t>(resp_sid, I64, ncap, "resp_sid", r),
             P<int32_t>(outcome, I32, ncap, "outcome", r), cur_stream()),
         "session_connect");
}

void session_close(const std::vector<Tensor>& tab, const Tensor& sids,
                   int64_t server_id, int64_t span) {
  ZkSessionTable s = session_table(tab, span);
  hip_ok(zk_session_close(&s, P<int64_t>(sids, I64, 0, "sids", &tab[0]),
                          sids.numel(), server_id, cur_stream()),
         "session_close");
}

void session_install(const std::vector<Tensor>& tab, const Tensor& rec,
                     int64_t server_id, int64_t span) {
  ZkSessionTable s = session_table(tab, span);
  TORCH_CHECK(rec.numel() % 4 == 0, "zkmi: session records are 4 x int64");
  hip_ok(zk_session_install(&s, P<int64_t>(rec, I64, 0, "records", &tab[0]),
                            rec.numel() / 4, server_id, cur_stream()),
         "session_install");
}

}

TORCH_LIBRARY(zkmi, m) {
  m.def("scan_workspace(int n) -> int", &scan_workspace);
  m.def("scan_set_mode(int mode) -> int", &scan_set_mode);
  m.def("scan_small(Tensor x, Tensor(a!) base, Tensor(b!) total, "
        "bool mfma) -> ()", &scan_small);
  m.def("scan_excl(Tensor x, Tensor(a!) base, Tensor(b!) total, "
        "Tensor(c!) ws) -> ()", &scan_excl);
  m.def("encode_requests(Tensor[] batch, int n, Tensor(a!) sizes, "
        "Tensor(b!) rec_off, Tensor(c!) total, Tensor(d!) ws, "
        "Tensor(e!) out, Tensor(f!)? xid_tab, int xid_mask, Tensor(g!) err, "
        "bool terminate) -> ()", &encode_requests);
  m.def("encode_requests_presized(Tensor[] batch, int n, Tensor sizes, "
        "Tensor bsum, Tensor(b!) rec_off, Tensor(c!) total, Tensor(d!) ws, "
        "Tensor(e!) out, Tensor(f!)? xid_tab, int xid_mask, Tensor(g!) err, "
        "bool terminate) -> ()", &encode_requests_presized);
  m.def("encode_set_watches(Tensor poff, Tensor plen, Tensor arena, int n, "
        "int c0, int c1, int rel_zxid, Tensor(a!) sizes, Tensor(b!) off, "
        "Tensor(c!) total, Tensor(d!) ws, Tensor(e!) out, Tensor(f!) err) "
        "-> ()", &encode_set_watches);
  m.def("encode_connect_requests(Tensor proto, Tensor zxid, Tensor timeout, "
        "Tensor sid, Tensor passwd_off, Tensor passwd_len, Tensor arena, "
        "int n, Tensor(a!) sizes, Tensor(b!) off, Tensor(c!) total, "
        "Tensor(d!) ws, Tensor(e!) out) -> ()", &encode_connect_requests);
  m.def("encode_responses(Tensor[] resp, Tensor? slot, Tensor[] store, "
        "Tensor count, int ncap, Tensor(a!) sizes, Tensor(b!) rec_off, "
        "Tensor(c!) total, Tensor(d!) ws, Tensor(e!) out, Tensor(f!) err, "
        "bool presized, bool terminate, bool prescanned=False) -> ()",
        &encode_responses);
  m.def("frame_scan_workspace(int n) -> int", &frame_scan_workspace);
  m.def("frame_scan(Tensor buf, Tensor? n, int n_cap, int max_packet, "
        "Tensor(a!) ws, Tensor(b!) frame_off, Tensor(c!) frame_len, "
        "Tensor(d!) result, int window, bool clean=False, int flags=0) "
        "-> ()",
        &frame_scan);
  m.def("frame_scan_stats(Tensor ws, int n_cap, int window) -> int[]",
        &frame_scan_stats);
  m.def("frame_scan_dbg(int tiles) -> Tensor", &frame_scan_dbg);
  m.def("decode_replies(Tensor buf, Tensor frame_off, Tensor frame_len, "
        "Tensor count, Tensor xid_tab, int xid_mask, Tensor(a!)[] out) -> ()",
        &decode_replies);
  m.def("decode_replies_check(Tensor buf, Tensor frame_off, Tensor frame_len, "
        "Tensor count, Tensor xid_tab, int xid_mask, Tensor(a!)[] out, "
        "Tensor idx, Tensor xid, Tensor data_len, Tensor(b!) acc, "
        "Tensor(c!)? tick=None, Tensor? slab=None, Tensor? slot_off=None) "
        "-> ()",
        &decode_replies_check);
  m.def("expand_strings(Tensor buf, Tensor region, Tensor count, "
        "Tensor base, Tensor(a!) str_off, Tensor(b!) str_len) -> ()",
        &expand_strings);
  m.def("expand_acl(Tensor buf, Tensor region, Tensor count, Tensor base, "
        "Tensor(a!) perms, Tensor(b!) scheme_off, Tensor(c!) scheme_len, "
        "Tensor(d!) id_off, Tensor(e!) id_len) -> ()", &expand_acl);
  m.def("decode_requests(Tensor buf, Tensor frame_off, Tensor frame_len, "
        "Tensor count, Tensor(a!)[] out) -> ()", &decode_requests);
  m.def("decode_connect_responses(Tensor buf, Tensor frame_off, "
        "Tensor frame_len, int n, Tensor(a!) proto, Tensor(b!) timeout, "
        "Tensor(c!) sid, Tensor(d!) passwd_off, Tensor(e!) passwd_len, "
        "Tensor(f!) status) -> ()", &decode_connect_responses);
  m.def("tree_fill(Tensor(a!)[] tree, int n0, int n, Tensor nkids, "
        "int now_ms) -> ()", &tree_fill);
  m.def("tree_build(Tensor(a!)[] tree, int n0, int n) -> ()", &tree_build);
  m.def("tree_ht_reset(Tensor(a!)[] tree) -> ()", &tree_ht_reset);
  m.def("tree_finish_scan(Tensor(a!)[] tree, Tensor? count, int bump, "
        "bool publish, int ncap, Tensor(b!) ws, Tensor(c!) total) -> ()",
        &tree_finish_scan);
  m.def("tree_free_workspace(int cap) -> int", &tree_free_workspace);
  m.def("tree_free_compact(Tensor(a!)[] tree, Tensor(b!) ws) -> ()",
        &tree_free_compact);
  m.def("tree_serve(Tensor(a!)[] tree, Tensor rx, Tensor[] requests, "
        "Tensor count, int ncap, Tensor(b!)[] out, int session, int now_ms) "
        "-> ()", &tree_serve);
  m.def("tree_serve_frames(Tensor(a!)[] tree, Tensor rx, Tensor frame_off, "
        "Tensor frame_len, Tensor count, int ncap, Tensor(b!)[] out, "
        "int session, int now_ms, int wslot=-1, Tensor(c!)? fired=None, "
        "Tensor? seqno=None, bool read_only=False) -> ()",
        &tree_serve_frames);
  m.def("tree_order_workspace(int n) -> int", &tree_order_workspace);
  m.def("tree_order_stats_offset(int n) -> int", &tree_order_stats_offset);
  m.def("tree_serve_ordered(Tensor(a!)[] tree, Tensor rx, Tensor[] requests, "
        "Tensor count, int ncap, Tensor(b!)[] out, int session, int now_ms, "
        "Tensor(c!) ws, int passes, Tensor? scratch, int wslot=-1, "
        "Tensor(d!)? fired=None, Tensor? seqno=None) -> ()",
        &tree_serve_ordered);
  m.def("tree_seq_workspace(int n) -> int", &tree_seq_workspace);
  m.def("tree_seq_zeroed(int n) -> int", &tree_seq_zeroed);
  m.def("tree_seq_debug(Tensor buf) -> ()", &tree_seq_debug);
  m.def("tree_expire_debug(Tensor buf) -> ()", &tree_expire_debug);
  m.def("tree_seq_order(Tensor(a!)[] tree, Tensor rx, Tensor frame_off, "
        "Tensor frame_len, Tensor count, int ncap, Tensor(b!) ws, "
        "Tensor(c!) seqno) -> ()", &tree_seq_order);
  m.def("tree_digest(Tensor[] tree, Tensor(a!) out) -> ()", &tree_digest);
  m.def("tree_list_workspace(int n) -> int", &tree_list_workspace);
  m.def("tree_list(Tensor(a!)[] tree, Tensor rx, Tensor frame_off, "
        "Tensor frame_len, Tensor count, int ncap, int wslot, int max_frame, "
        "Tensor(b!) want, Tensor(c!) ws, Tensor(d!) out, int out_cap, "
        "Tensor(e!) rec_off, Tensor(f!) total, Tensor(g!) err, "
        "bool terminate=False) -> ()",
        &tree_list);
  m.def("tree_acl_workspace(int n) -> int", &tree_acl_workspace);
  m.def("tree_acl_record(Tensor(a!)[] acl, Tensor rx, Tensor frame_off, "
        "Tensor frame_len, Tensor count, int ncap, Tensor r_op, "
        "Tensor r_err, Tensor r_node, Tensor(b!) ws) -> ()",
        &tree_acl_record);
  m.def("tree_acl_get(Tensor[] tree, Tensor[] acl, Tensor rx, "
        "Tensor frame_off, Tensor frame_len, Tensor count, int ncap, "
        "Tensor(a!) ws, Tensor(b!) out, int out_cap, Tensor(c!) rec_off, "
        "Tensor(d!) total, Tensor(e!) err, bool terminate=False) -> ()",
        &tree_acl_get);
  m.def("watch_events(Tensor r_op, Tensor r_err, Tensor count, int ncap, "
        "Tensor fired, Tensor(a!) bsum, Tensor(b!) ev_slot, "
        "Tensor(c!) ev_type, Tensor(d!) ev_path_off, Tensor(e!) ev_path_len, "
        "Tensor(f!) ev_total) -> ()", &watch_events);
  m.def("watch_resume(Tensor(a!)[] tree, Tensor rx, Tensor frame_off, "
        "Tensor frame_len, Tensor count, int ncap, int wslot, "
        "Tensor(b!) ent, Tensor(c!) ev_type, Tensor(d!) ev_path_off, "
        "Tensor(e!) ev_path_len, Tensor(f!) out) -> ()", &watch_resume);
  m.def("tree_expire(Tensor(a!)[] tree, int session, int ncap, "
        "Tensor(b!) removed) -> ()", &tree_expire);
  m.def("bench_gen_get(int n, int seed, int leaf0, int nleaves, "
        "int xid_base, Tensor node_pw, Tensor(a!) idx, Tensor(b!) xid, "
        "Tensor(c!) path_off, Tensor(d!) path_len, Tensor? state=None, "
        "Tensor(e!)? sizes=None, Tensor(f!)? bsum=None) -> ()",
        &bench_gen_get);
  m.def("bench_xids(int n, Tensor base, Tensor(a!) xid) -> ()", &bench_xids);
  m.def("bench_storm_hs(bool resume, bool prev, int timeout, Tensor status, "
        "Tensor sid, Tensor tmo, Tensor outcome, Tensor bound, Tensor resp, "
        "Tensor want, Tensor(a!) cred_sid, Tensor(b!) cred_pw, "
        "Tensor(c!) hs_ok) -> ()", &bench_storm_hs);
  m.def("bench_check_writes(int n, Tensor status, Tensor err, Tensor rxid, "
        "Tensor xid, Tensor pay_len, Tensor? want_len, int want_len_c, "
        "Tensor zxid, Tensor(a!) ok, Tensor(b!) zmax) -> ()",
        &bench_check_writes);
  m.def("bench_check_get(int n, Tensor[] reply, Tensor idx, Tensor xid, "
        "Tensor data_len, Tensor(a!) acc) -> ()", &bench_check_get);
  m.def("bench_check_notif(int total, int n_per, Tensor seeds, int leaf0, "
        "int nleaves, Tensor node_path_off, Tensor node_path_len, "
        "Tensor path_arena, Tensor rx, Tensor[] reply, Tensor(a!) acc, "
        "Tensor? want=None) -> ()", &bench_check_notif);
  m.def("route_workspace(int n, int world) -> int", &route_workspace);
  m.def("route_requests(int n, int world, Tensor path_off, Tensor path_len, "
        "Tensor arena, Tensor idx, Tensor xid, Tensor(a!) owner, "
        "Tensor(b!) idx_s, Tensor(c!) xid_s, Tensor(d!) path_off_s, "
        "Tensor(e!) path_len_s, Tensor(f!) counts, Tensor(g!) ws, "
        "int self=0) -> ()",
        &route_requests);
  m.def("seg_pack(Tensor src, Tensor rec_off, Tensor? nrec, int nrec_cap, "
        "Tensor total, Tensor counts, int world, int self, int slot_cap, "
        "Tensor(a!) out, Tensor(b!) stats, Tensor(c!)? self_out=None, "
        "bool inplace=False) -> ()",
        &seg_pack);
  m.def("seg_unpack(Tensor inp, int world, int self, int slot_cap, "
        "Tensor(a!) out, Tensor(b!) total, Tensor(c!) counts, "
        "Tensor(d!)? stats=None, Tensor? self_in=None, "
        "bool inplace=False) -> ()", &seg_unpack);
  m.def("session_connect(Tensor buf, Tensor frame_off, Tensor frame_len, "
        "Tensor count, int ncap, Tensor(a!)[] table, int server_id, "
        "int secret, int min_to, int max_to, Tensor zxid_now, Tensor(b!) out, "
        "Tensor(c!) resp_sid, Tensor(d!) outcome, int span=0) -> ()",
        &session_connect);
// ... 6 lines not shown
```

### zkmi/ops/batch.py

```python

from dataclasses import dataclass

import numpy as np

import torch

from .. import consts
from .. import jute
from . import _lib

SENTINEL_XID = -(1 << 63)
I64 = torch.int64
I32 = torch.int32
U8 = torch.uint8

_FS_GROUP = 8


def _dev(device):
    return torch.device(device) if device is not None else \
        torch.device('cuda', torch.cuda.current_device())


class XidTable(object):
# ... 153 lines not shown
    t_poff = torch.from_numpy(poff).to(dev)
    t_plen = torch.from_numpy(plen).to(dev)
    t_ar = torch.from_numpy(np.frombuffer(bytes(arena) or b'\0',
                                          np.uint8).copy()).to(dev)
    sizes = torch.empty(max(n, 1), dtype=I64, device=dev)
    off = torch.zeros(max(n, 1), dtype=I64, device=dev)
    total = torch.zeros(1, dtype=I64, device=dev)
    ws = torch.empty(L.scan_workspace(max(n, 1)), dtype=I64, device=dev)
    cap = 64 + len(arena) + 4 * n
    out = torch.empty(cap, dtype=U8, device=dev)
    err = torch.zeros(1, dtype=I32, device=dev)
    with _on(stream):
        L.encode_set_watches(t_poff, t_plen, t_ar, n, len(data_paths),
                             len(exist_paths), rel_zxid, sizes, off, total,
                             ws, out, err)
    frame_len = 32 + len(arena) + 4 * n
    return out[:frame_len]



def encode_connect_requests(reqs, device=None, stream=None):
    L = _lib.lib()
    dev = _dev(device)
    n = len(reqs)
    arena = bytearray()
    pwo, pwl = [], []
    for r in reqs:
        pw = r.get('passwd', b'\0' * 8)
        pwo.append(len(arena))
        pwl.append(len(pw))
        arena += pw
    T = lambda v, dt: torch.tensor(v, dtype=dt, device=dev)
    proto = T([r.get('protocolVersion', 0) for r in reqs], I32)
    zx = T([r.get('lastZxidSeen', 0) for r in reqs], I64)
    tmo = T([r['timeOut'] for r in reqs], I32)
    sid = T([r.get('sessionId', 0) for r in reqs], I64)
    t_pwo, t_pwl = T(pwo, I64), T(pwl, I32)
    t_ar = torch.from_numpy(np.frombuffer(bytes(arena) or b'\0',
                                          np.uint8).copy()).to(dev)
    sizes = torch.empty(max(n, 1), dtype=I64, device=dev)
    off = torch.empty(max(n, 1), dtype=I64, device=dev)
    total = torch.zeros(1, dtype=I64, device=dev)
    ws = torch.empty(L.scan_workspace(max(n, 1)), dtype=I64, device=dev)
    size = n * 32 + len(arena)
    cap = size + 16
    out = torch.empty(cap, dtype=U8, device=dev)
    with _on(stream):
        L.encode_connect_requests(proto, zx, tmo, sid, t_pwo, t_pwl, t_ar, n,
                                  sizes, off, total, ws, out)
    return out[:size]


def decode_connect_responses(buf, frames, n, stream=None):
    L = _lib.lib()
    dev = buf.device
    e = lambda dt: torch.empty(max(n, 1), dtype=dt, device=dev)
    o = {'protocolVersion': e(I32), 'timeOut': e(I32), 'sessionId': e(I64),
         'passwd_off': e(I64), 'passwd_len': e(I32), 'status': e(I32)}
    with _on(stream):
        L.decode_connect_responses(
            buf, frames.off, frames.length, n, o['protocolVersion'],
            o['timeOut'], o['sessionId'], o['passwd_off'], o['passwd_len'],
            o['status'])
    return {k: v[:n] for k, v in o.items()}



@dataclass
class FrameTable:
    off: torch.Tensor
    length: torch.Tensor
    result: torch.Tensor

    @property
    def count(self):
        return self.result[0:1]

    def host_result(self):
        r = self.result.cpu().tolist()
        return {'frames': r[0], 'consumed': r[1], 'bad': bool(r[2]),
                'overflow': bool(r[3])}


FS_WINDOWS = (256, 512, 1024, 2048)
FS_WIN_LONG = 1 << 16
FS_WINDOW_AUTO_MAX = 2048


def frame_window(max_frame):
    cap = FS_WINDOW_AUTO_MAX
    cap = min(max(cap, FS_WINDOWS[0]), FS_WINDOWS[-1])
    for w in FS_WINDOWS:
        if max_frame <= w and w <= cap:
            return w
    top = max(w for w in FS_WINDOWS if w <= cap)
    return top | FS_WIN_LONG


def _scan_len(buf, n):
    if n is None:
        return None, buf.numel()
    if isinstance(n, torch.Tensor):
        if n.dtype != I64 or n.device != buf.device or n.numel() < 1:
            raise TypeError('frame_scan: device length must be an int64 '
                            'tensor on the buffer\'s device')
        return n, buf.numel()
    n = int(n)
    if n > buf.numel():
        raise ValueError('frame_scan: n=%d past the buffer (%d bytes)'
                         % (n, buf.numel()))
    return None, n


class FrameScanner:

    def __init__(self, cap, device, window=2048,
                 max_packet=consts.MAX_PACKET, frame_hint=None, group=None):
        self.cap = cap
        self.window = window
        if group is None:
            group = _FS_GROUP if frame_hint is not None and \
                frame_hint >= 128 else 1
        self.group = group
        self.max_packet = max_packet
        self.table = FrameTable(torch.empty(cap, dtype=I64, device=device),
                                torch.empty(cap, dtype=I32, device=device),
                                torch.empty(4, dtype=I64, device=device))
        self.ws = torch.empty(0, dtype=U8, device=device)
        self.ws_for = -1
        self.clean_for = -1

    def scan(self, buf, n, stream=None, nospec=False, misspec=0):
        L = _lib.lib()
        n_dev, ncap = _scan_len(buf, n)
        if ncap > self.ws_for:
            cover = max(ncap, 2 * self.ws_for)
            wsb = L.frame_scan_workspace(cover)
            self.ws = torch.empty(max(wsb, 256), dtype=U8,
                                  device=buf.device)
            self.ws_for = cover
            self.clean_for = -1
        t = self.table
        with _on(stream):
            L.frame_scan(buf, n_dev, ncap, self.max_packet, self.ws, t.off,
                         t.length, t.result, int(self.window),
                         ncap == self.clean_for,
                         (1 if nospec else 0) | (int(misspec) << 8) |
                         ((self.group - 1) << 4))
        self.clean_for = ncap
        self.last_cap = ncap
        return t

    def chain_stats(self, stream=None):
        if getattr(self, 'last_cap', None) is None:
            return {'no_spec': 0, 'rewalked': 0, 'rounds': 0, 'looked_up': 0}
        with _on(stream):
            out = _lib.lib().frame_scan_stats(self.ws, self.last_cap,
                                              int(self.window))
        return {'no_spec': out[0], 'rewalked': out[1], 'rounds': out[2],
                'looked_up': out[3]}


def frame_scan(buf, n=None, max_packet=consts.MAX_PACKET, cap=None,
               stream=None, workspace=None, window=2048):
    L = _lib.lib()
    n_dev, ncap = _scan_len(buf, n)
    dev = buf.device
    if cap is None:
        cap = max(ncap // 4, 1)
    wsb = L.frame_scan_workspace(ncap)
    if workspace is None or workspace.numel() < wsb:
        workspace = torch.empty(max(wsb, 256), dtype=U8, device=dev)
    off = torch.empty(cap, dtype=I64, device=dev)
    ln = torch.empty(cap, dtype=I32, device=dev)
    res = torch.empty(4, dtype=I64, device=dev)
    with _on(stream):
        L.frame_scan(buf, n_dev, ncap, max_packet, workspace, off, ln, res,
                     int(window))
    return FrameTable(off, ln, res)



STAT64 = ('czxid', 'mzxid', 'ctime', 'mtime', 'ephemeralOwner', 'pzxid')
STAT32 = ('version', 'cversion', 'aversion', 'dataLength', 'numChildren')


@dataclass
class ReplyBatch:
    xid: torch.Tensor
    err: torch.Tensor
    opcode: torch.Tensor
    status: torch.Tensor
    zxid: torch.Tensor
    stat64: torch.Tensor
    stat32: torch.Tensor
    pay_off: torch.Tensor
    pay_len: torch.Tensor
    aux0: torch.Tensor
    aux1: torch.Tensor
    count: torch.Tensor

    def tensors(self):
        return [self.xid, self.err, self.opcode, self.status, self.zxid,
                self.stat64, self.stat32, self.pay_off, self.pay_len,
                self.aux0, self.aux1]


def alloc_replies(cap, device):
    dev = _dev(device)
    return ReplyBatch(
        torch.empty(cap, dtype=I32, device=dev),
        torch.empty(cap, dtype=I32, device=dev),
        torch.empty(cap, dtype=I32, device=dev),
        torch.empty(cap, dtype=I32, device=dev),
        torch.empty(cap, dtype=I64, device=dev),
        torch.zeros(6, cap, dtype=I64, device=dev),
        torch.zeros(5, cap, dtype=I32, device=dev),
        torch.empty(cap, dtype=I64, device=dev),
        torch.empty(cap, dtype=I32, device=dev),
        torch.empty(cap, dtype=I32, device=dev),
        torch.empty(cap, dtype=I32, device=dev),
        None)


def decode_replies(buf, frames, xid_table, out=None, stream=None,
                   check=None, tick=None):
    L = _lib.lib()
    cap = frames.off.numel()
    if out is None:
        out = alloc_replies(cap, buf.device)
    out.count = frames.count
    with _on(stream):
        if check is None:
            L.decode_replies(buf, frames.off, frames.length, frames.count,
                             xid_table.tab, xid_table.mask, out.tensors())
        else:
            idx, xid, data_len, acc = check[:4]
            slab, slot_off = check[4:6] if len(check) > 4 else (None, None)
            L.decode_replies_check(buf, frames.off, frames.length,
                                   frames.count, xid_table.tab,
                                   xid_table.mask, out.tensors(), idx, xid,
                                   data_len, acc, tick, slab, slot_off)
    return out


def exclusive_scan(x, stream=None):
    L = _lib.lib()
    n = x.numel()
    dev = x.device
    base = torch.empty(max(n, 1), dtype=I64, device=dev)
    total = torch.zeros(1, dtype=I64, device=dev)
    ws = torch.empty(L.scan_workspace(max(n, 1)), dtype=I64, device=dev)
    if x.dtype not in (torch.int32, torch.int64):
        raise TypeError('exclusive_scan: int32 or int64 input')
    with _on(stream):
        L.scan_excl(x, base, total, ws)
    return base[:n], total


def _scan_i32(counts, stream=None):
    L = _lib.lib()
    n = counts.numel()
    dev = counts.device
    base = torch.empty(max(n, 1), dtype=I64, device=dev)
    total = torch.zeros(1, dtype=I64, device=dev)
    ws = torch.empty(L.scan_workspace(max(n, 1)), dtype=I64, device=dev)
    with _on(stream):
        L.scan_excl(counts, base, total, ws)
    return base, total


def expand_strings(buf, region, count, stream=None):
    L = _lib.lib()
    n = region.numel()
    base, total = _scan_i32(count, stream)
    m = int(total.item())
    soff = torch.empty(max(m, 1), dtype=I64, device=buf.device)
    slen = torch.empty(max(m, 1), dtype=I32, device=buf.device)
    with _on(stream):
        L.expand_strings(buf, region, count, base[:n], soff, slen)
    return base[:n], soff[:m], slen[:m]


def expand_acl(buf, region, count, stream=None):
    L = _lib.lib()
    n = region.numel()
    base, total = _scan_i32(count, stream)
    m = int(total.item())
    dev = buf.device
    perms = torch.empty(max(m, 1), dtype=I32, device=dev)
    so = torch.empty(max(m, 1), dtype=I64, device=dev)
    sl = torch.empty(max(m, 1), dtype=I32, device=dev)
    io = torch.empty(max(m, 1), dtype=I64, device=dev)
    il = torch.empty(max(m, 1), dtype=I32, device=dev)
    with _on(stream):
        L.expand_acl(buf, region, count, base[:n], perms, so, sl, io, il)
    return base[:n], perms[:m], so[:m], sl[:m], io[:m], il[:m]



@dataclass
class RequestTable:
    xid: torch.Tensor
    opcode: torch.Tensor
    status: torch.Tensor
    path_off: torch.Tensor
    path_len: torch.Tensor
    data_off: torch.Tensor
    data_len: torch.Tensor
    arg: torch.Tensor
    vec_off: torch.Tensor
    vec_count: torch.Tensor
    rel_zxid: torch.Tensor
    count: torch.Tensor
# ... 128 lines not shown
```

Before: 2.055 billion.

## Fuse frame row emission into decode and serve kernels via deferred tile rows

Adds a deferred mode to frame_scan that skips the separate row-emission pass and records a frame-block to tile map instead. Decode and tree-serve kernels can then rebuild each frame's offset and length from the tile metadata themselves, writing the frame table as they go. This removes one kernel launch and a round trip of frame offsets through global memory. In exchange each consumer workgroup does extra tile lookups, and scan and consume must be paired through a pending-tiles handshake. The path is opt-in through rows=False and a tiles argument.

```diff
diff --git a/csrc/kernels/decode.hip b/csrc/kernels/decode.hip
--- a/csrc/kernels/decode.hip
+++ b/csrc/kernels/decode.hip
@@ -1,4 +1,5 @@
 #include "zk_common.h"
+#include "zk_frame_rows.h"
 
 namespace zk {
 
@@ -78,24 +79,41 @@
   return __ballot(diff != 0) == 0;
 }
 
-template <bool CHECK>
-__global__ __launch_bounds__(DEC_T) void decode_replies_k(
+static_assert(DEC_T == FR_T, "a workgroup per block of FR_T frames");
+template <bool CHECK, bool TILES>
+ZK_DEV void decode_replies_body(
     const uint8_t* __restrict__ buf, const int64_t* __restrict__ foff,
     const int32_t* __restrict__ flen, const int64_t* __restrict__ n_dev,
     int64_t ncap, const int64_t* __restrict__ xid_tab, int64_t xid_mask,
-    ZkReplyOut o, ZkGetCheck chk) {
+    const ZkReplyOut& o, const ZkGetCheck& chk, const ZkFrameTiles* T,
+    int64_t* __restrict__ rows_off, int32_t* __restrict__ rows_len) {
   const uint32_t nwg = gridDim.x;
-  const int64_t i = (int64_t)xcd_remap(blockIdx.x, nwg) * DEC_T + threadIdx.x;
-  const bool live = i < ncap && i < *n_dev;
-  if (!CHECK && !live) return;
+  const uint32_t blk = xcd_remap(blockIdx.x, nwg);
+  const int64_t i = (int64_t)blk * DEC_T + threadIdx.x;
+  bool live = i < ncap && i < *n_dev;
+  int64_t fo = 0;
+  int32_t fl = 0;
+  if (TILES) {
+    __shared__ FrLds rows;
+    const int64_t nf = *n_dev;
+    live = fr_row(*T, blk, nf < ncap ? nf : ncap, rows, fo, fl);
+    if (live) {
+      rows_off[i] = fo;
+      rows_len[i] = fl;
+    }
+    fr_housekeep(*T);
+  } else if (!CHECK && !live) {
+    return;
+  }
   int64_t good = 0;
   const int64_t salt = CHECK && chk.tick != nullptr ? chk.tick[1] : 0;
   bool samp = false;
   int64_t s_off = 0, s_node = 0;
   int32_t s_len = 0;
   if (live) {
-  const uint8_t* p = buf + foff[i];
-  const int64_t L = flen[i];
+  if (!TILES) fo = foff[i];
+  const uint8_t* p = buf + fo;
+  const int64_t L = TILES ? fl : flen[i];
   int32_t status = ST_OK;
   int32_t op = OP_UNKNOWN;
   int64_t poff = -1;
@@ -134,7 +152,7 @@
         int32_t dl = ld_be32(b);
         if (dl < 0) dl = 0;
         if (4 + (int64_t)dl + STAT_BYTES > A) { status = ST_BAD_DECODE; break; }
-        poff = foff[i] + 20;
+        poff = fo + 20;
         plen = dl;
         if (tail_ok && 4 + (int64_t)dl + STAT_BYTES == A) read_stat_regs(sw, o, i);
         else read_stat(b + 4 + dl, o, i);
@@ -150,7 +168,7 @@
         int32_t l = ld_be32(b);
         if (l < 0) l = 0;
         if (4 + (int64_t)l > A) { status = ST_BAD_DECODE; break; }
-        poff = foff[i] + 20;
+        poff = fo + 20;
         plen = l;
         break;
       }
@@ -163,7 +181,7 @@
           status = ST_BAD_DECODE;
           break;
         }
-        poff = foff[i] + 20;
+        poff = fo + 20;
         plen = (int32_t)k;
         a0 = cnt;
         if (op == OP_GET_CHILDREN2) {
@@ -177,7 +195,7 @@
         const int32_t cnt = max(ld_be32(b), 0);
         const int64_t k = skip_acl(b + 4, A - 4, cnt);
         if (k < 0 || 4 + k + STAT_BYTES > A) { status = ST_BAD_DECODE; break; }
-        poff = foff[i] + 20;
+        poff = fo + 20;
         plen = (int32_t)k;
         a0 = cnt;
         if (tail_ok && 4 + k + STAT_BYTES == A) read_stat_regs(sw, o, i);
@@ -191,7 +209,7 @@
         if (12 + (int64_t)l > A) { status = ST_BAD_DECODE; break; }
         a0 = ld_be32(b);
         a1 = ld_be32(b + 4);
-        poff = foff[i] + 28;
+        poff = fo + 28;
         plen = l;
         break;
       }
@@ -244,6 +262,28 @@
       atomicAdd(&chk.acc[blockIdx.x % (uint32_t)chk.slots],
                 (unsigned long long)tot);
   }
+}
+
+template <bool CHECK>
+__global__ __launch_bounds__(DEC_T) void decode_replies_k(
+    const uint8_t* __restrict__ buf, const int64_t* __restrict__ foff,
+    const int32_t* __restrict__ flen, const int64_t* __restrict__ n_dev,
+    int64_t ncap, const int64_t* __restrict__ xid_tab, int64_t xid_mask,
+    ZkReplyOut o, ZkGetCheck chk) {
+  decode_replies_body<CHECK, false>(buf, foff, flen, n_dev, ncap, xid_tab,
+                                    xid_mask, o, chk, nullptr, nullptr,
+                                    nullptr);
+}
+
+template <bool CHECK>
+__global__ __launch_bounds__(DEC_T) void decode_replies_tiles_k(
+    ZkFrameTiles T, int64_t* __restrict__ rows_off,
+    int32_t* __restrict__ rows_len, const int64_t* __restrict__ n_dev,
+    int64_t ncap, const int64_t* __restrict__ xid_tab, int64_t xid_mask,
+    ZkReplyOut o, ZkGetCheck chk) {
+  decode_replies_body<CHECK, true>(T.buf, nullptr, nullptr, n_dev, ncap,
+                                   xid_tab, xid_mask, o, chk, &T, rows_off,
+                                   rows_len);
 }
 
 __global__ __launch_bounds__(DEC_T) void expand_strings_k(
@@ -380,6 +420,39 @@
   return 0;
 }
 
+int zk_decode_replies_tiles(const ZkFrameTiles* tiles, int64_t* foff,
+                            int32_t* flen, const int64_t* n_dev, int64_t ncap,
+                            const int64_t* xid_tab, int64_t xid_mask,
+                            const ZkReplyOut* o, hipStream_t st) {
+  if (ncap <= 0) return (int)hipErrorInvalidValue;
+  zk::decode_replies_tiles_k<false><<<zk::nblk(ncap), zk::DEC_T, 0, st>>>(
+      *tiles, foff, flen, n_dev, ncap, xid_tab, xid_mask, *o,
+      zk::ZkGetCheck{nullptr, nullptr, nullptr, nullptr, 1, nullptr, nullptr,
+                     nullptr});
+  ZK_LAUNCH_CHECK();
+  return 0;
+}
+
+int zk_decode_replies_check_tiles(const ZkFrameTiles* tiles, int64_t* foff,
+                                  int32_t* flen, const int64_t* n_dev,
+                                  int64_t ncap, const int64_t* xid_tab,
+                                  int64_t xid_mask, const ZkReplyOut* o,
+                                  const int64_t* idx, const int32_t* xid,
+                                  const int32_t* data_len,
+                                  unsigned long long* acc, int32_t slots,
+                                  int64_t* tick, const uint8_t* slab,
+                                  const int64_t* slot_off, hipStream_t st) {
+  if (ncap <= 0) return (int)hipErrorInvalidValue;
+  if (slots < 1 || slots > 64) return (int)hipErrorInvalidValue;
+  if ((slab == nullptr) != (slot_off == nullptr))
+    return (int)hipErrorInvalidValue;
+  zk::decode_replies_tiles_k<true><<<zk::nblk(ncap), zk::DEC_T, 0, st>>>(
+      *tiles, foff, flen, n_dev, ncap, xid_tab, xid_mask, *o,
+      zk::ZkGetCheck{idx, xid, data_len, acc, slots, tick, slab, slot_off});
+  ZK_LAUNCH_CHECK();
+  return 0;
+}
+
 int zk_expand_strings(const uint8_t* buf, const int64_t* region,
                       const int32_t* count, const int64_t* base, int64_t n,
                       int64_t* soff, int32_t* slen, hipStream_t st) {
diff --git a/csrc/kernels/frame_scan.hip b/csrc/kernels/frame_scan.hip
--- a/csrc/kernels/frame_scan.hip
+++ b/csrc/kernels/frame_scan.hip
@@ -1,37 +1,22 @@
 #include "zk_common.h"
+#include "zk_frame_rows.h"
 
 namespace zk {
 
-constexpr int FT_S = 4096;
-constexpr int FT_LMAX = FT_S / 4;
-constexpr int FT_STAGE = FT_S + 16;
 constexpr int64_t TERM = (int64_t)1 << 62;
 constexpr int64_t TBAD = (int64_t)1 << 60;
 constexpr int64_t FC_MAXP = (int64_t)1 << 24;
 constexpr int FC_WIN = 4096;
 constexpr int FL_T = 512;
 constexpr int FL_U = 8;
-constexpr int FL_NB = 2;
-constexpr int FL_GW = FL_NB + 1;
 constexpr int FL_BROUNDS = 8;
 constexpr int FL_DBG_BLOCKS = 16;
 constexpr int FL_DBG_ROWS = 6;
 constexpr uint32_t FL_CHASE_WALKS = 16;
-constexpr int FK_T = 64;
-constexpr int LW_MINS = 4, LW_LAST = 6, LW_NOSPEC = 7, LW_GRID = 8;
-constexpr int LW_BIG = 16;
-constexpr int LW_END = 32;
-static_assert(LW_GRID + FL_GW <= LW_BIG, "grid words");
 constexpr unsigned FL_BIG_NOSPEC = 256;
 constexpr int FL_GROUNDS = 6;
 constexpr uint64_t FT_WAIT_TICKS = 200000;
 
-ZK_DEV int64_t stream_len(const int64_t* n_dev, int64_t n_cap) {
-  if (n_dev == nullptr) return n_cap;
-  const int64_t v = *n_dev;
-  return v < 0 ? 0 : (v < n_cap ? v : n_cap);
-}
-
 ZK_DEV uint64_t lb_load(const uint64_t* p) {
   return __hip_atomic_load(p, __ATOMIC_RELAXED, __HIP_MEMORY_SCOPE_AGENT);
 }
@@ -48,13 +33,6 @@
 ZK_DEV void fc_stat(uint64_t* stats, int k, uint32_t v) {
   __hip_atomic_fetch_add((uint32_t*)&stats[k], v, __ATOMIC_RELAXED,
                          __HIP_MEMORY_SCOPE_AGENT);
-}
-
-ZK_DEV int32_t lds_be32(const uint8_t* sb, int32_t p) {
-  const int32_t a = p & ~3;
-  const uint32_t lo = *(const uint32_t*)(sb + a);
-  const uint32_t hi = *(const uint32_t*)(sb + a + 4);
-  return (int32_t)bswap32(__builtin_amdgcn_alignbyte(hi, lo, p & 3));
 }
 
 constexpr int FT_BITS = FT_S / 32;
@@ -71,13 +49,6 @@
   return (int64_t)w.cnt | ((int64_t)w.np << 11) | ((int64_t)(w.js + 1) << 22) |
          ((int64_t)w.term << 33) | ((int64_t)w.bad << 34);
 }
-ZK_DEV int32_t m_cnt(int64_t m) { return (int32_t)(m & 0x7FF); }
-ZK_DEV int32_t m_np(int64_t m) { return (int32_t)((m >> 11) & 0x7FF); }
-ZK_DEV int32_t m_js(int64_t m) { return (int32_t)((m >> 22) & 0x7FF) - 1; }
-ZK_DEV bool m_term(int64_t m) { return (m >> 33) & 1; }
-ZK_DEV bool m_bad(int64_t m) { return (m >> 34) & 1; }
-constexpr int64_t M_STALE = (int64_t)1 << 35;
-ZK_DEV bool m_stale(int64_t m) { return (m >> 35) & 1; }
 
 ZK_DEV void fc_join_end(FcWalk& r, int64_t send, int64_t n) {
   if (send & TERM) {
@@ -1351,29 +1322,6 @@
   }
 }
 
-
-template <int WIN>
-ZK_DEV void fc_stage(const uint8_t* __restrict__ buf, int64_t n, int64_t wb,
-                     uint8_t* win, int lane) {
-  constexpr int PER = WIN / 1024;
-  uint4 v[PER];
-#pragma unroll
-  for (int j = 0; j < PER; ++j) {
-    const int64_t g = wb + 16 * (lane + 64 * j);
-    v[j] = make_uint4(0, 0, 0, 0);
-    if (g + 16 <= n) {
-      __builtin_memcpy(&v[j], buf + g, 16);
-    } else if (g < n) {
-      uint8_t* b = (uint8_t*)&v[j];
-      for (int k = 0; k < 16; ++k) b[k] = g + k < n ? buf[g + k] : 0;
-    }
-  }
-#pragma unroll
-  for (int j = 0; j < PER; ++j) *(uint4*)(win + 16 * (lane + 64 * j)) = v[j];
-  __builtin_amdgcn_wave_barrier();
-  asm volatile("s_waitcnt lgkmcnt(0)" ::: "memory");
-  __builtin_amdgcn_wave_barrier();
-}
 
 template <int WIN = FC_WIN>
 ZK_DEV FcWalk fc_walk(const uint8_t* __restrict__ buf, int64_t n,
@@ -1644,7 +1592,8 @@
 ZK_DEV void fl_bases(int64_t n, int64_t ntiles, int64_t ft,
                      const int64_t* rec_exit, const int64_t* rec_meta,
                      const int64_t* base, int64_t* bsum, int64_t cap,
-                     int64_t* result, int64_t* lastk, int64_t* red) {
+                     int64_t* result, int64_t* lastk, int64_t* red,
+                     int32_t* fblk) {
   const int tid = threadIdx.x;
   const int64_t INF = INT64_MAX;
   const int64_t last = ft == INF ? ntiles - 1 : ft;
@@ -1660,9 +1609,11 @@
   for (int64_t b = b0; b < b1; ++b) {
     const int64_t v = ld_agent(&bsum[b]);
     bsum[b] = run;
+    int64_t live = v;
     if (b == blast) {
       const int64_t ml = ld_agent(&rec_meta[last]);
       const int64_t total = run + ld_agent(&base[last]) + m_cnt(ml);
+      live = total - run;
       *lastk = last;
       result[0] = total;
       result[3] = total > cap ? 1 : 0;
@@ -1674,6 +1625,8 @@
         result[2] = m_bad(ml) ? 1 : 0;
       }
     }
+    for (int64_t j = (run + FR_T - 1) / FR_T; j * FR_T < run + live; ++j)
+      fblk[j] = (int32_t)b;
     run += v;
   }
 }
@@ -2005,7 +1958,8 @@
 ZK_DEV void fl_count_scan(int64_t n, int64_t ntiles, int64_t ft,
                           const int64_t* rec_exit, const int64_t* rec_meta,
                           int64_t* base, int64_t* bsum, int64_t cap,
-                          int64_t* result, int64_t* lastk, int64_t* red) {
+                          int64_t* result, int64_t* lastk, int64_t* red,
+                          int32_t* fblk) {
   const int tid = threadIdx.x;
   const int64_t INF = INT64_MAX;
   const int64_t last = ft == INF ? ntiles - 1 : ft;
@@ -2031,7 +1985,10 @@
 #pragma unroll
     for (int u = 0; u < FL_U; ++u) {
       if (kb + u < k1) base[kb + u] = run;
-      run += m_cnt(v[u]);
+      const int64_t end = run + m_cnt(v[u]);
+      for (int64_t j = (run + FR_T - 1) / FR_T; j * FR_T < end; ++j)
+        fblk[j] = (int32_t)((kb + u) / FK_T);
+      run = end;
     }
   }
   for (int64_t k = last + 1 + tid; k < ntiles; k += FL_T) base[k] = -1;
@@ -2170,7 +2127,7 @@
     int64_t* __restrict__ bsum, uint64_t* mins,
     int64_t* __restrict__ lastk, unsigned long long* g,
     const uint64_t* lbw, const int64_t* __restrict__ cx,
-    int64_t* __restrict__ ldbg) {
+    int64_t* __restrict__ ldbg, int32_t* __restrict__ fblk) {
   __shared__ __attribute__((aligned(16)))
       uint8_t win[(FL_T / 64) * (FC_WIN + 16)];
   __shared__ int64_t red[2 * (FL_T / 64) + 2];
@@ -2234,7 +2191,7 @@
   if (!big && (fb0 == INF || fb0 > ft0)) {
     if (ldbg != nullptr && tid == 0) ldbg[40] = wall_clock64();
     fl_bases(n, ntiles, ft0, rec_exit, rec_meta, base, bsum, cap, result,
-             lastk, red);
+             lastk, red, fblk);
     if (ldbg != nullptr && tid == 0) ldbg[41] = wall_clock64();
     return;
   }
@@ -2273,7 +2230,7 @@
                           fbv, ftv);
       if (fbv == INF || fbv > ftv) {
         fl_count_scan(n, ntiles, ftv, rec_exit, rec_meta, base, bsum, cap,
-                      result, lastk, red);
+                      result, lastk, red, fblk);
         if (clk) ldbg[4] = wall_clock64() | (2ll << 56);
         return;
       }
@@ -2290,13 +2247,13 @@
       if (settled && (fbv == INF || fbv > ftv)) {
         if (changed) {
           fl_count_scan(n, ntiles, ftv, rec_exit, rec_meta, base, bsum, cap,
-                        result, lastk, red);
+                        result, lastk, red, fblk);
           if (clk) ldbg[4] = wall_clock64() | (2ll << 56);
           return;
         }
         fl_chase_recount(ntiles, rec_meta, base, bsum, ch);
         fl_bases(n, ntiles, ftv, rec_exit, rec_meta, base, bsum, cap, result,
-                 lastk, red);
+                 lastk, red, fblk);
         if (clk) ldbg[4] = wall_clock64() | (1ll << 56);
         return;
       }
@@ -2339,7 +2296,7 @@
     }
   }
   fl_count_scan(n, ntiles, ft, rec_exit, rec_meta, base, bsum, cap, result,
-                lastk, red);
+                lastk, red, fblk);
   if (clk) ldbg[4] = wall_clock64() | (3ll << 56);
 }
 
@@ -2376,52 +2333,24 @@
   const int64_t b = bsum[t / FK_T] + base[t];
   const int64_t m = rec_meta[t];
   const int64_t x = rec_exit[t];
-  const int32_t cnt = m_cnt(m), np = m_np(m), js = m_js(m);
-  const int64_t ts = t * FT_S;
-  const uint16_t* P = pre + t * FT_LMAX;
-  const uint16_t* R = list + t * FT_LMAX + (js < 0 ? 0 : js);
-  if (m_stale(m)) {
-    uint8_t* sb = stage[wv];
-    fc_stage<FT_S>(buf, n, ts, sb, lane);
-    if (lane == 0) {
-      uint8_t* pb = sb + FT_S;
-      for (int k = 0; k < 16; ++k)
-        pb[k] = ts + FT_S + k < n ? buf[ts + FT_S + k] : 0;
-    }
-    __builtin_amdgcn_wave_barrier();
-    asm volatile("s_waitcnt lgkmcnt(0)" ::: "memory");
-    int32_t c = __builtin_amdgcn_readfirstlane((int32_t)(rec_entry[t] - ts));
-    int32_t ent = 0;
-    for (int32_t k = 0; k < cnt; ++k) {
-      ent = lane == (k & 63) ? c : ent;
-      const int32_t len = __builtin_amdgcn_readfirstlane(lds_be32(sb, c));
-      c += 4 + len;
-      if ((k & 63) == 63 || k == cnt - 1) {
-        const int32_t last = k & 63;
-        const int32_t nxt = __shfl_down(ent, 1, 64);
-        if (lane <= last) {
-          const int64_t p = ts + ent;
-          const int64_t q = lane < last ? ts + nxt
-                                        : (k == cnt - 1 ? x : ts + c);
-          const int64_t idx = b + (k & ~63) + lane;
-          if (idx < cap) {
-            foff[idx] = p + 4;
-            flen[idx] = (int32_t)(q - p - 4);
-          }
-        }
-      }
-    }
-    return;
-  }
-  for (int32_t k = lane; k < cnt; k += 64) {
-    const int64_t p = ts + (k < np ? P[k] : R[k - np]);
-    const int32_t k1 = k + 1;
-    const int64_t q = k1 < cnt ? ts + (k1 < np ? P[k1] : R[k1 - np]) : x;
+  const int32_t cnt = m_cnt(m);
+  auto row = [&](int32_t k, int64_t p, int64_t q) {
     const int64_t idx = b + k;
     if (idx < cap) {
       foff[idx] = p + 4;
       flen[idx] = (int32_t)(q - p - 4);
     }
+  };
+  if (m_stale(m)) {
+    const int32_t c = __builtin_amdgcn_readfirstlane(
+        (int32_t)(rec_entry[t] - t * FT_S));
+    fr_walk_stale<false>(buf, n, t, c, cnt, x, stage[wv], lane, row);
+    return;
+  }
+  for (int32_t k = lane; k < cnt; k += 64) {
+    int64_t p, q;
+    fr_bounds(list, pre, t, m, x, k, p, q);
+    row(k, p, q);
   }
 }
 
@@ -2458,7 +2387,7 @@
 struct FsPlan {
   int64_t tiles;
   size_t off_list, off_pre, off_sx, off_lbw, off_rent, off_rexit, off_rmeta,
-      off_rcnt, off_base, off_blist, off_bsum, off_cx, total;
+      off_rcnt, off_base, off_blist, off_bsum, off_cx, off_fblk, total;
 };
 
 static FsPlan fs_plan(int64_t n) {
@@ -2479,6 +2408,7 @@
   p.off_blist = take((size_t)tiles * 4);
   p.off_bsum = take((size_t)(tiles / FK_T + 1) * 8);
   p.off_cx = take((size_t)tiles * 5 * 8);
+  p.off_fblk = take((size_t)(tiles * (FT_LMAX / FR_T) + 1) * 4);
   p.total = o;
   return p;
 }
@@ -2488,6 +2418,7 @@
 static int32_t fs_minb() { return 8; }
 
 constexpr int32_t FS_LONG = 2;
+constexpr int32_t FS_DEFER = 1 << 24;
 
 constexpr int32_t FS_WIN_LONG = 1 << 16;
 
@@ -2529,11 +2460,14 @@
                   int32_t clean, int32_t flags, hipStream_t st) {
   using namespace zk;
   const int W = fs_window(window);
+  const bool defer = (flags & FS_DEFER) != 0;
+  flags &= ~FS_DEFER;
   if (window & FS_WIN_LONG) flags |= FS_LONG;
   if (maxp > FC_MAXP || maxp < 0) return -3;
   FsPlan p = fs_plan(n_cap);
   if ((int64_t)p.total > ws_bytes) return -1;
   const int64_t tiles = p.tiles;
+  if (defer && n_cap <= FT_S) return -5;
   if (n_cap <= FT_S && !(flags & (1 | 0xFFFF00)) &&
       fs_dbg_buf(tiles) == nullptr) {
     fs_small<<<1, 64, 0, st>>>(buf, n_dev, n_cap, maxp, foff, flen, cap,
@@ -2553,6 +2487,7 @@
   int32_t* blist = (int32_t*)(ws + p.off_blist);
   int64_t* bsum = (int64_t*)(ws + p.off_bsum);
   int64_t* cx = (int64_t*)(ws + p.off_cx);
+  int32_t* fblk = (int32_t*)(ws + p.off_fblk);
   uint64_t* mins = lbw + 2 * tiles + LW_MINS;
   int64_t* lastk = (int64_t*)(lbw + 2 * tiles + LW_LAST);
   unsigned long long* grid = (unsigned long long*)(lbw + 2 * tiles + LW_GRID);
@@ -2605,12 +2540,38 @@
   fs_link<<<fl_blocks(), FL_T, 0, st>>>(buf, n_dev, n_cap, maxp, sx, list, rcnt,
                                  pre, rent, rexit, rmeta, base, cap, result,
                                  lbw + 2 * tiles, blist, bsum, mins, lastk,
-                                 grid, lbw, cx, dbg ? dbg + 8 * tiles : nullptr);
+                                 grid, lbw, cx, dbg ? dbg + 8 * tiles : nullptr,
+                                 fblk);
   ZK_LAUNCH_CHECK();
+  if (defer) return 0;
   fs_rows<<<(unsigned)((tiles + 3) / 4), 256, 0, st>>>(
       buf, n_dev, n_cap, list, pre, rmeta, rent, rexit, base, bsum, lastk,
       foff, flen, cap, lbw, lbw + 2 * tiles);
   ZK_LAUNCH_CHECK();
+  return 0;
+}
+
+int zk_frame_tiles(const uint8_t* buf, const int64_t* n_dev, int64_t n_cap,
+                   uint8_t* ws, int64_t ws_bytes, ZkFrameTiles* out) {
+  using namespace zk;
+  if (n_cap <= FT_S) return -2;
+  FsPlan p = fs_plan(n_cap);
+  if ((int64_t)p.total > ws_bytes) return -1;
+  uint64_t* lbw = (uint64_t*)(ws + p.off_lbw);
+  out->buf = buf;
+  out->n_dev = n_dev;
+  out->n_cap = n_cap;
+  out->list = (const uint16_t*)(ws + p.off_list);
+  out->pre = (const uint16_t*)(ws + p.off_pre);
+  out->rec_meta = (const int64_t*)(ws + p.off_rmeta);
+  out->rec_entry = (const int64_t*)(ws + p.off_rent);
+  out->rec_exit = (const int64_t*)(ws + p.off_rexit);
+  out->base = (const int64_t*)(ws + p.off_base);
+  out->bsum = (const int64_t*)(ws + p.off_bsum);
+  out->lastk = (const int64_t*)(lbw + 2 * p.tiles + LW_LAST);
+  out->fblk = (const int32_t*)(ws + p.off_fblk);
+  out->lbw = lbw;
+  out->tiles = p.tiles;
   return 0;
 }
 
diff --git a/csrc/kernels/tree.hip b/csrc/kernels/tree.hip
--- a/csrc/kernels/tree.hip
+++ b/csrc/kernels/tree.hip
@@ -1,4 +1,5 @@
 #include "zk_tree.h"
+#include "zk_frame_rows.h"
 
 namespace zk {
 
@@ -210,9 +211,10 @@
   return ERR_OK;
 }
 
-template <bool PARSE, bool RO = false>
-__global__ __launch_bounds__(TR_T) void tree_serve_k(
-    ZkTree t, const uint8_t* __restrict__ rx, ZkReqOut q,
+static_assert(TR_T == FR_T, "a workgroup per block of FR_T frames");
+template <bool PARSE, bool RO, bool TILES>
+ZK_DEV void tree_serve_body(
+    const ZkTree& t, const uint8_t* __restrict__ rx, const ZkReqOut& q,
     const int64_t* __restrict__ foff, const int32_t* __restrict__ flen,
     const int64_t* __restrict__ n_dev, int64_t ncap, int32_t* __restrict__ r_op,
     int32_t* __restrict__ r_xid, int32_t* __restrict__ r_err,
@@ -222,11 +224,23 @@
     int64_t* __restrict__ r_bsum, int64_t session, int64_t now_ms,
     const uint8_t* __restrict__ rank, int32_t pass, int32_t last_pass,
     int64_t snap_base, int64_t snap_cap, int64_t* __restrict__ snap_top,
-    int32_t wslot, int64_t* __restrict__ fired) {
+    int32_t wslot, int64_t* __restrict__ fired, const ZkFrameTiles* T,
+    int64_t* __restrict__ rows_off, int32_t* __restrict__ rows_len) {
   session = sess_of(t, session);
   const uint32_t blk = xcd_remap(blockIdx.x, gridDim.x);
   const int64_t i = (int64_t)blk * TR_T + threadIdx.x;
   const bool in_batch = i < ncap && i < *n_dev;
+  int64_t fo = 0;
+  int32_t fl = 0;
+  if (TILES) {
+    __shared__ FrLds rows;
+    const int64_t nf = *n_dev;
+    if (fr_row(*T, blk, nf < ncap ? nf : ncap, rows, fo, fl)) {
+      rows_off[i] = fo;
+      rows_len[i] = fl;
+    }
+    fr_housekeep(*T);
+  }
   const int32_t rb = rank != nullptr && in_batch ? (int32_t)rank[i] : 0;
   const int32_t rk = rb & ORD_RANK;
   const bool live = in_batch && (rk == pass || (last_pass && rk > pass));
@@ -234,7 +248,8 @@
   ReqFields rq{ST_BAD_DECODE, 0, OP_PING, 0, 0, 0, 0, -1, -1, -1, 0};
   if (live) {
     if (PARSE) {
-      rq = parse_request(rx, foff[i], flen[i]);
+      rq = TILES ? parse_request(rx, fo, fl)
+                 : parse_request(rx, foff[i], flen[i]);
     } else {
       rq.status = q.status[i];
       rq.xid = q.xid[i];
@@ -474,10 +489,53 @@
   if (r_slot != nullptr) r_slot[i] = L.op == OP_DELETE ? -1 : L.slot;
 }
 
+template <bool PARSE, bool RO = false>
+__global__ __launch_bounds__(TR_T) void tree_serve_k(
+    ZkTree t, const uint8_t* __restrict__ rx, ZkReqOut q,
+    const int64_t* __restrict__ foff, const int32_t* __restrict__ flen,
+    const int64_t* __restrict__ n_dev, int64_t ncap, int32_t* __restrict__ r_op,
+    int32_t* __restrict__ r_xid, int32_t* __restrict__ r_err,
+    int64_t* __restrict__ r_node, int64_t* __restrict__ r_zxid,
+    int64_t* __restrict__ r_path_off, int32_t* __restrict__ r_path_len,
+    int64_t* __restrict__ r_slot, int64_t* __restrict__ r_sizes,
+    int64_t* __restrict__ r_bsum, int64_t session, int64_t now_ms,
+    const uint8_t* __restrict__ rank, int32_t pass, int32_t last_pass,
+    int64_t snap_base, int64_t snap_cap, int64_t* __restrict__ snap_top,
+    int32_t wslot, int64_t* __restrict__ fired) {
+  tree_serve_body<PARSE, RO, false>(
+      t, rx, q, foff, flen, n_dev, ncap, r_op, r_xid, r_err, r_node, r_zxid,
+      r_path_off, r_path_len, r_slot, r_sizes, r_bsum, session, now_ms, rank,
+      pass, last_pass, snap_base, snap_cap, snap_top, wslot, fired, nullptr,
+      nullptr, nullptr);
+}
+
+template <bool RO>
+__global__ __launch_bounds__(TR_T) void tree_serve_tiles_k(
+    ZkTree t, ZkFrameTiles T, int64_t* __restrict__ rows_off,
+    int32_t* __restrict__ rows_len, const int64_t* __restrict__ n_dev,
+    int64_t ncap, ZkServeOut o, int64_t session, int64_t now_ms,
+    int32_t wslot, int64_t* __restrict__ fired) {
+  tree_serve_body<true, RO, true>(
+      t, T.buf, ZkReqOut{}, nullptr, nullptr, n_dev, ncap, o.opcode, o.xid,
+      o.err, o.node, o.zxid, o.path_off, o.path_len, o.slot, o.sizes,
+      o.block_sums, session, now_ms, nullptr, 0, 1, 0, 0, nullptr, wslot,
+      fired, &T, rows_off, rows_len);
+}
+
 int serve_launch(const ServeLaunch& s, hipStream_t st) {
   if (s.ncap <= 0) return 0;
   const ZkServeOut& o = *s.out;
   if ((o.sizes == nullptr) != (o.block_sums == nullptr)) return -1;
+  if (s.tiles != nullptr) {
+    if (s.q != nullptr || s.rank != nullptr) return -1;
+    const auto kt = s.read_only ? tree_serve_tiles_k<true>
+                                : tree_serve_tiles_k<false>;
+    kt<<<(unsigned)((s.ncap + TR_T - 1) / TR_T), TR_T, 0, st>>>(
+        *s.tree, *s.tiles, s.rows_off, s.rows_len, s.n_dev, s.ncap, o,
+        s.session, s.now_ms, s.wslot, s.fired);
+    ZK_LAUNCH_CHECK();
+    return 0;
+  }
   const bool parse = s.q == nullptr;
   const auto k = !parse        ? tree_serve_k<false>
                  : s.read_only ? tree_serve_k<true, true>
@@ -516,6 +574,20 @@
   s.tree = t, s.rx = rx, s.foff = foff, s.flen = flen, s.n_dev = n_dev;
   s.ncap = ncap, s.out = out, s.session = session, s.now_ms = now_ms;
   s.wslot = wslot, s.fired = fired, s.read_only = read_only;
+  return zk::serve_launch(s, st);
+}
+
+int zk_tree_serve_tiles(const ZkTree* t, const ZkFrameTiles* tiles,
+                        int64_t* foff, int32_t* flen, const int64_t* n_dev,
+                        int64_t ncap, const ZkServeOut* out, int64_t session,
+                        int64_t now_ms, int32_t wslot, int64_t* fired,
+                        int32_t read_only, hipStream_t st) {
+  if (ncap <= 0) return (int)hipErrorInvalidValue;
+  zk::ServeLaunch s;
+  s.tree = t, s.rx = tiles->buf, s.tiles = tiles, s.rows_off = foff;
+  s.rows_len = flen, s.n_dev = n_dev, s.ncap = ncap, s.out = out;
+  s.session = session, s.now_ms = now_ms, s.wslot = wslot, s.fired = fired;
+  s.read_only = read_only;
   return zk::serve_launch(s, st);
 }
 
diff --git a/csrc/kernels/zk_abi.h b/csrc/kernels/zk_abi.h
--- a/csrc/kernels/zk_abi.h
+++ b/csrc/kernels/zk_abi.h
@@ -128,6 +128,23 @@
   int64_t* val;
   int64_t hmask;
   int64_t* ctr;
+};
+
+struct ZkFrameTiles {
+  const uint8_t* buf;
+  const int64_t* n_dev;
+  int64_t n_cap;
+  const uint16_t* list;
+  const uint16_t* pre;
+  const int64_t* rec_meta;
+  const int64_t* rec_entry;
+  const int64_t* rec_exit;
+  const int64_t* base;
+  const int64_t* bsum;
+  const int64_t* lastk;
+  const int32_t* fblk;
+  uint64_t* lbw;
+  int64_t tiles;
 };
 
 int64_t zk_scan_workspace(int64_t n);
@@ -164,6 +181,18 @@
 int zk_frame_scan_stats(const uint8_t*, int64_t, int32_t, uint32_t*,
                         hipStream_t);
 int zk_frame_scan_dbg(int64_t* host, int64_t tiles);
+int zk_frame_tiles(const uint8_t* buf, const int64_t* n_dev, int64_t n_cap,
+                   uint8_t* ws, int64_t ws_bytes, ZkFrameTiles* out);
+int zk_decode_replies_tiles(const ZkFrameTiles*, int64_t*, int32_t*,
+                            const int64_t*, int64_t, const int64_t*, int64_t,
+                            const ZkReplyOut*, hipStream_t);
+int zk_decode_replies_check_tiles(const ZkFrameTiles*, int64_t*, int32_t*,
+                                  const int64_t*, int64_t, const int64_t*,
+                                  int64_t, const ZkReplyOut*, const int64_t*,
+                                  const int32_t*, const int32_t*,
+                                  unsigned long long*, int32_t, int64_t*,
+                                  const uint8_t*, const int64_t*,
+                                  hipStream_t);
 int zk_decode_replies(const uint8_t*, const int64_t*, const int32_t*,
                       const int64_t*, int64_t, const int64_t*, int64_t,
                       const ZkReplyOut*, hipStream_t);
@@ -198,6 +227,10 @@
                          const int32_t*, const int64_t*, int64_t,
                          const ZkServeOut*, int64_t, int64_t, int32_t,
                          int64_t*, int32_t, hipStream_t);
+int zk_tree_serve_tiles(const ZkTree*, const ZkFrameTiles*, int64_t*,
+                        int32_t*, const int64_t*, int64_t, const ZkServeOut*,
+                        int64_t, int64_t, int32_t, int64_t*, int32_t,
+                        hipStream_t);
 int zk_tree_finish_scan(const ZkTree*, const int64_t*, int64_t, int32_t,
                         int64_t, int64_t*, int64_t*, hipStream_t);
 int zk_tree_serve_ordered(const ZkTree*, const uint8_t*, const ZkReqOut*,
@@ -297,6 +330,8 @@
 static_assert(offsetof(ZkAclTable, arena) == 2 * 8, "ZkAclTable.arena");
 static_assert(offsetof(ZkAclTable, hmask) == 6 * 8, "ZkAclTable.hmask");
 static_assert(sizeof(ZkTree) == 27 * 8, "ZkTree layout");
+static_assert(sizeof(ZkFrameTiles) == 14 * 8, "ZkFrameTiles layout");
+static_assert(offsetof(ZkFrameTiles, fblk) == 11 * 8, "ZkFrameTiles.fblk");
 static_assert(offsetof(ZkTree, store) == 9 * 8, "ZkTree.store");
 static_assert(offsetof(ZkTree, free_list) == 14 * 8, "ZkTree.free_list");
 static_assert(offsetof(ZkTree, wt_hmask) == 25 * 8, "ZkTree.wt_hmask");
diff --git a/csrc/kernels/zk_frame_rows.h b/csrc/kernels/zk_frame_rows.h
--- /dev/null
+++ b/csrc/kernels/zk_frame_rows.h
@@ -0,0 +1,264 @@
+#pragma once
+#include "zk_common.h"
+
+namespace zk {
+
+constexpr int FT_S = 4096;
+constexpr int FT_LMAX = FT_S / 4;
+constexpr int FT_STAGE = FT_S + 16;
+constexpr int FK_T = 64;
+constexpr int FL_NB = 2;
+constexpr int FL_GW = FL_NB + 1;
+constexpr int LW_MINS = 4, LW_LAST = 6, LW_NOSPEC = 7, LW_GRID = 8;
+constexpr int LW_BIG = 16;
+constexpr int LW_END = 32;
+static_assert(LW_GRID + FL_GW <= LW_BIG, "grid words");
+constexpr int FR_T = 256;
+constexpr int FR_W = 64;
+
+ZK_DEV int64_t stream_len(const int64_t* n_dev, int64_t n_cap) {
+  if (n_dev == nullptr) return n_cap;
+  const int64_t v = *n_dev;
+  return v < 0 ? 0 : (v < n_cap ? v : n_cap);
+}
+
+ZK_DEV int32_t lds_be32(const uint8_t* sb, int32_t p) {
+  const int32_t a = p & ~3;
+  const uint32_t lo = *(const uint32_t*)(sb + a);
+  const uint32_t hi = *(const uint32_t*)(sb + a + 4);
+  return (int32_t)bswap32(__builtin_amdgcn_alignbyte(hi, lo, p & 3));
+}
+
+ZK_DEV int32_t m_cnt(int64_t m) { return (int32_t)(m & 0x7FF); }
+ZK_DEV int32_t m_np(int64_t m) { return (int32_t)((m >> 11) & 0x7FF); }
+ZK_DEV int32_t m_js(int64_t m) { return (int32_t)((m >> 22) & 0x7FF) - 1; }
+ZK_DEV bool m_term(int64_t m) { return (m >> 33) & 1; }
+ZK_DEV bool m_bad(int64_t m) { return (m >> 34) & 1; }
+constexpr int64_t M_STALE = (int64_t)1 << 35;
+ZK_DEV bool m_stale(int64_t m) { return (m >> 35) & 1; }
+
+template <int WIN>
+ZK_DEV void fc_stage(const uint8_t* __restrict__ buf, int64_t n, int64_t wb,
+                     uint8_t* win, int lane) {
+  constexpr int PER = WIN / 1024;
+  uint4 v[PER];
+#pragma unroll
+  for (int j = 0; j < PER; ++j) {
+    const int64_t g = wb + 16 * (lane + 64 * j);
+    v[j] = make_uint4(0, 0, 0, 0);
+    if (g + 16 <= n) {
+      __builtin_memcpy(&v[j], buf + g, 16);
+    } else if (g < n) {
+      uint8_t* b = (uint8_t*)&v[j];
+      for (int k = 0; k < 16; ++k) b[k] = g + k < n ? buf[g + k] : 0;
+    }
+  }
+#pragma unroll
+  for (int j = 0; j < PER; ++j) *(uint4*)(win + 16 * (lane + 64 * j)) = v[j];
+  __builtin_amdgcn_wave_barrier();
+  asm volatile("s_waitcnt lgkmcnt(0)" ::: "memory");
+  __builtin_amdgcn_wave_barrier();
+}
+
+ZK_DEV void fr_stage_lean(const uint8_t* __restrict__ buf, int64_t n,
+                          int64_t wb, uint8_t* win, int lane) {
+#pragma unroll 1
+  for (int j = 0; j < FT_S / 1024; ++j) {
+    const int64_t g = wb + 16 * (lane + 64 * j);
+    uint4 v = make_uint4(0, 0, 0, 0);
+    if (g + 16 <= n) {
+      __builtin_memcpy(&v, buf + g, 16);
+    } else if (g < n) {
+      uint32_t w[4] = {0, 0, 0, 0};
+#pragma unroll 1
+      for (int k = 0; k < 16; ++k)
+        if (g + k < n) w[k >> 2] |= (uint32_t)buf[g + k] << (8 * (k & 3));
+      v = make_uint4(w[0], w[1], w[2], w[3]);
+    }
+    *(uint4*)(win + 16 * (lane + 64 * j)) = v;
+  }
+  __builtin_amdgcn_wave_barrier();
+  asm volatile("s_waitcnt lgkmcnt(0)" ::: "memory");
+  __builtin_amdgcn_wave_barrier();
+}
+
+ZK_DEV void fr_bounds(const uint16_t* __restrict__ list,
+                      const uint16_t* __restrict__ pre, int64_t t, int64_t m,
+                      int64_t x, int32_t k, int64_t& p, int64_t& q) {
+  const int32_t cnt = m_cnt(m), np = m_np(m), js = m_js(m);
+  const int64_t ts = t * FT_S;
+  const uint16_t* P = pre + t * FT_LMAX;
+  const uint16_t* R = list + t * FT_LMAX + (js < 0 ? 0 : js);
+  p = ts + (k < np ? P[k] : R[k - np]);
+  const int32_t k1 = k + 1;
+  q = k1 < cnt ? ts + (k1 < np ? P[k1] : R[k1 - np]) : x;
+}
+
+template <bool LEAN, typename Emit>
+ZK_DEV void fr_walk_stale(const uint8_t* __restrict__ buf, int64_t n,
+                          int64_t t, int32_t c, int32_t cnt, int64_t x,
+                          uint8_t* sb, int lane, Emit emit) {
+  const int64_t ts = t * FT_S;
+  if (LEAN) fr_stage_lean(buf, n, ts, sb, lane);
+  else fc_stage<FT_S>(buf, n, ts, sb, lane);
+  if (lane == 0) {
+    uint8_t* pb = sb + FT_S;
+#pragma unroll 1
+    for (int k = 0; k < 16; ++k)
+      pb[k] = ts + FT_S + k < n ? buf[ts + FT_S + k] : 0;
+  }
+  __builtin_amdgcn_wave_barrier();
+  asm volatile("s_waitcnt lgkmcnt(0)" ::: "memory");
+  int32_t ent = 0;
+  for (int32_t k = 0; k < cnt; ++k) {
+    ent = lane == (k & 63) ? c : ent;
+    const int32_t len = __builtin_amdgcn_readfirstlane(lds_be32(sb, c));
+    c += 4 + len;
+    if ((k & 63) == 63 || k == cnt - 1) {
+      const int32_t last = k & 63;
+      const int32_t nxt = __shfl_down(ent, 1, 64);
+      if (lane <= last) {
+        const int64_t p = ts + ent;
+        const int64_t q = lane < last ? ts + nxt
+                                      : (k == cnt - 1 ? x : ts + c);
+        emit((k & ~63) + lane, p, q);
+      }
+    }
+  }
+}
+
+
+struct FrLds {
+  __attribute__((aligned(16))) uint8_t stage[FT_STAGE];
+  int64_t off[FR_T];
+  int32_t len[FR_T];
+  int32_t rb[FR_W];
+  unsigned long long pick;
+};
+
+ZK_DEV int64_t fr_rowbase(const ZkFrameTiles& T, int64_t t) {
+  return T.bsum[t / FK_T] + T.base[t];
+}
+
+ZK_DEV bool fr_row(const ZkFrameTiles& T, uint32_t blk, int64_t nrows,
+                   FrLds& S, int64_t& foff, int32_t& flen) {
+  const int tid = threadIdx.x, lane = tid & 63;
+  const int64_t i0 = (int64_t)blk * FR_T;
+  if (i0 >= nrows) return false;
+  const bool act = i0 + tid < nrows;
+  const int64_t n = stream_len(T.n_dev, T.n_cap);
+  const int64_t lastk = *T.lastk;
+  int64_t w0;
+  {
+    const int64_t b = T.fblk[blk];
+    const int64_t t = b * FK_T + lane;
+    const bool le = t <= lastk && fr_rowbase(T, t) <= i0;
+    const uint64_t m = __ballot(le);
+    w0 = b * FK_T + (m ? 63 - (int64_t)__builtin_clzll(m) : 0);
+  }
+  int64_t t = -1;
+  int32_t k = 0;
+  bool placed = !act;
+  for (;;) {
+    if (tid < FR_W) {
+      const int64_t tw = w0 + tid;
+      int32_t r = 0x7FFFFFFF;
+      if (tw <= lastk) {
+        const int64_t d = fr_rowbase(T, tw) - i0;
+        r = d > FR_T ? FR_T : (int32_t)d;
+      }
+      S.rb[tid] = r;
+    }
+    __syncthreads();
+    if (!placed) {
+      int lo = 0;
+#pragma unroll
+      for (int s = FR_W / 2; s >= 1; s >>= 1)
+        if (S.rb[lo + s] <= tid) lo += s;
+      if (lo < FR_W - 1 || w0 + FR_W - 1 >= lastk) {
+        t = w0 + lo;
+        k = tid - S.rb[lo];
+        placed = true;
+      }
+    }
+    if (!__syncthreads_or(!placed)) break;
+    w0 += FR_W - 1;
+  }
+  int64_t m = 0, x = 0;
+  bool stale = false;
+  if (act) {
+    m = T.rec_meta[t];
+    x = T.rec_exit[t];
+    stale = m_stale(m);
+    foff = 0;
+    flen = 0;
+    if (!stale && (uint32_t)k < (uint32_t)m_cnt(m)) {
+      int64_t p, q;
+      fr_bounds(T.list, T.pre, t, m, x, k, p, q);
+      foff = p + 4;
+      flen = (int32_t)(q - p - 4);
+    }
+  }
+  if (__syncthreads_or(stale)) {
+    for (;;) {
+      if (tid == 0) S.pick = ~0ull;
+      __syncthreads();
+      if (stale) atomicMin(&S.pick, (unsigned long long)t);
+      __syncthreads();
+      const unsigned long long pk = S.pick;
+      if (pk == ~0ull) break;
+      const int64_t tt = (int64_t)pk;
+      if (stale && t == tt) {
+        S.off[tid] = 0;
+        S.len[tid] = 0;
+      }
+      __syncthreads();
+      if (tid < 64) {
+        const int64_t mt = T.rec_meta[tt];
+        const int64_t rel = fr_rowbase(T, tt) - i0;
+        const int32_t c = __builtin_amdgcn_readfirstlane(
+            (int32_t)(T.rec_entry[tt] - tt * FT_S));
+        fr_walk_stale<true>(T.buf, n, tt, c, m_cnt(mt), T.rec_exit[tt], S.stage,
+                      lane, [&](int32_t kk, int64_t p, int64_t q) {
+                        const int64_t r = rel + kk;
+                        if (r >= 0 && r < FR_T) {
+                          S.off[r] = p + 4;
+                          S.len[r] = (int32_t)(q - p - 4);
+                        }
+                      });
+      }
+      __syncthreads();
+      if (stale && t == tt) {
+        foff = S.off[tid];
+        flen = S.len[tid];
+        stale = false;
+      }
+      __syncthreads();
+    }
+  }
+  return act;
+}
+
+ZK_DEV void fr_housekeep(const ZkFrameTiles& T) {
+  const int64_t n = stream_len(T.n_dev, T.n_cap);
+  const int64_t ntiles = (n + FT_S - 1) / FT_S;
+  const int64_t step = (int64_t)gridDim.x * blockDim.x;
+  for (int64_t t = (int64_t)blockIdx.x * blockDim.x + threadIdx.x; t < ntiles;
+       t += step) {
+    T.lbw[2 * t] = 0;
+    T.lbw[2 * t + 1] = 0;
+  }
+  if (blockIdx.x == 0) {
+    uint64_t* tail = T.lbw + 2 * T.tiles;
+    const int tid = threadIdx.x;
+    if (tid == 0) {
+      tail[LW_MINS] = 0;
+      tail[LW_MINS + 1] = 0;
+      tail[LW_NOSPEC] = 0;
+      tail[LW_GRID + FL_NB] = 0;
+    }
+    if (tid < LW_END - LW_BIG) tail[LW_BIG + tid] = 0;
+  }
+}
+
+}
diff --git a/csrc/kernels/zk_tree.h b/csrc/kernels/zk_tree.h
--- a/csrc/kernels/zk_tree.h
+++ b/csrc/kernels/zk_tree.h
@@ -538,6 +538,9 @@
   int32_t wslot = -1;
   int64_t* fired = nullptr;
   int32_t read_only = 0;
+  const ZkFrameTiles* tiles = nullptr;
+  int64_t* rows_off = nullptr;
+  int32_t* rows_len = nullptr;
 };
 int serve_launch(const ServeLaunch& s, hipStream_t st);
 
diff --git a/csrc/torch/zkmi_ops.cpp b/csrc/torch/zkmi_ops.cpp
--- a/csrc/torch/zkmi_ops.cpp
+++ b/csrc/torch/zkmi_ops.cpp
@@ -479,6 +479,77 @@
          "decode_replies_check");
 }
 
+ZkFrameTiles frame_tiles(const Tensor& buf, const c10::optional<Tensor>& n_dev,
+                         int64_t n_cap, const Tensor& ws) {
+  TORCH_CHECK(n_cap >= 0 && n_cap <= buf.numel(),
+              "zkmi: frame tiles: length ", n_cap, " past the buffer (",
+              buf.numel(), " bytes)");
+  ZkFrameTiles t;
+  const int rc = zk_frame_tiles(
+      P<uint8_t>(buf, U8, 1, "buf"),
+      Popt<int64_t>(n_dev, I64, 1, "n", &buf), n_cap,
+      P<uint8_t>(ws, U8, 1, "ws", &buf), ws.numel(), &t);
+  TORCH_CHECK(rc != -2, "zkmi: a stream of one tile at most has no tile "
+              "lists (its scan writes the rows itself)");
+  TORCH_CHECK(rc == 0, "zkmi: frame tiles: workspace too small");
+  return t;
+}
+
+void decode_replies_tiles(const Tensor& buf,
+                          const c10::optional<Tensor>& n_bytes, int64_t n_cap,
+                          const Tensor& ws, const Tensor& foff,
+                          const Tensor& flen, const Tensor& n_dev,
+                          const Tensor& xid_tab, int64_t xid_mask,
+                          const std::vector<Tensor>& out) {
+  const int64_t cap = foff.numel();
+  TORCH_CHECK(cap >= 1, "zkmi: decode_replies_tiles: an empty frame table");
+  ZkReplyOut o = reply_out(out, cap, &buf);
+  ZkFrameTiles t = frame_tiles(buf, n_bytes, n_cap, ws);
+  hip_ok(zk_decode_replies_tiles(
+             &t, P<int64_t>(foff, I64, cap, "frame_off", &buf),
+             P<int32_t>(flen, I32, cap, "frame_len", &buf),
+             P<int64_t>(n_dev, I64, 1, "count", &buf), cap,
+             P<int64_t>(xid_tab, I64, xid_mask + 1, "xid_tab", &buf),
+             xid_mask, &o, cur_stream()),
+         "decode_replies_tiles");
+}
+
+void decode_replies_check_tiles(
+    const Tensor& buf, const c10::optional<Tensor>& n_bytes, int64_t n_cap,
+    const Tensor& ws, const Tensor& foff, const Tensor& flen,
+    const Tensor& n_dev, const Tensor& xid_tab, int64_t xid_mask,
+    const std::vector<Tensor>& out, const Tensor& idx, const Tensor& xid,
+    const Tensor& data_len, const Tensor& acc,
+    const c10::optional<Tensor>& tick, const c10::optional<Tensor>& slab,
+    const c10::optional<Tensor>& slot_off) {
+  const int64_t cap = foff.numel();
+  TORCH_CHECK(cap >= 1,
+              "zkmi: decode_replies_check_tiles: an empty frame table");
+  ZkReplyOut o = reply_out(out, cap, &buf);
+  const int32_t slots = (int32_t)std::min<int64_t>(acc.numel(), 64);
+  TORCH_CHECK(slots >= 1, "zkmi: decode_replies_check needs an acc slot");
+  TORCH_CHECK(slab.has_value() == slot_off.has_value(),
+              "zkmi: decode_replies_check: slab and slot_off go together");
+  if (slot_off.has_value())
+    TORCH_CHECK(slot_off->numel() >= data_len.numel(),
+                "zkmi: decode_replies_check: slot_off shorter than data_len");
+  ZkFrameTiles t = frame_tiles(buf, n_bytes, n_cap, ws);
+  hip_ok(zk_decode_replies_check_tiles(
+             &t, P<int64_t>(foff, I64, cap, "frame_off", &buf),
+             P<int32_t>(flen, I32, cap, "frame_len", &buf),
+             P<int64_t>(n_dev, I64, 1, "count", &buf), cap,
+             P<int64_t>(xid_tab, I64, xid_mask + 1, "xid_tab", &buf),
+             xid_mask, &o, P<int64_t>(idx, I64, cap, "idx", &buf),
+             P<int32_t>(xid, I32, cap, "xid", &buf),
+             P<int32_t>(data_len, I32, 1, "data_len", &buf),
+             reinterpret_cast<unsigned long long*>(
+                 P<int64_t>(acc, I64, slots, "acc", &buf)),
+             slots, Popt<int64_t>(tick, I64, 2, "tick", &buf),
+             Popt<uint8_t>(slab, U8, 1, "slab", &buf),
+             Popt<int64_t>(slot_off, I64, 1, "slot_off", &buf), cur_stream()),
+         "decode_replies_check_tiles");
+}
+
 void expand_strings(const Tensor& buf, const Tensor& region,
                     const Tensor& count, const Tensor& base,
                     const Tensor& soff, const Tensor& slen) {
@@ -626,6 +697,32 @@
              now_ms, (int32_t)wslot, Popt<int64_t>(fired, I64, 5 * ncap, "fired", d),
              read_only ? 1 : 0, cur_stream()),
          "tree_serve_frames");
+}
+
+void tree_serve_tiles(const std::vector<Tensor>& t, const Tensor& rx,
+                      const c10::optional<Tensor>& n_bytes, int64_t n_cap,
+                      const Tensor& ws, const Tensor& foff, const Tensor& flen,
+                      const Tensor& n_dev, int64_t ncap,
+                      const std::vector<Tensor>& r, int64_t session,
+                      int64_t now_ms, int64_t wslot,
+                      const c10::optional<Tensor>& fired,
+                      const c10::optional<Tensor>& seqno, bool read_only) {
+  ZkTree s = tree(t);
+  const Tensor* d = &t[0];
+  TORCH_CHECK(ncap >= 1, "zkmi: tree_serve_tiles: an empty frame table");
+  ZkServeOut ro = serve_out(r, ncap, d);
+  s.seqno = Popt<int64_t>(seqno, I64, ncap, "seqno", d);
+  TORCH_CHECK(wslot >= -1 && wslot < 64, "zkmi: watcher slot -1..63");
+  TORCH_CHECK(rx.device() == d->device(), "zkmi: rx on the tree's device");
+  ZkFrameTiles ft = frame_tiles(rx, n_bytes, n_cap, ws);
+  hip_ok(zk_tree_serve_tiles(
+             &s, &ft, P<int64_t>(foff, I64, ncap, "frame_off", d),
+             P<int32_t>(flen, I32, ncap, "frame_len", d),
+             P<int64_t>(n_dev, I64, 1, "count", d), ncap, &ro, session,
+             now_ms, (int32_t)wslot,
+             Popt<int64_t>(fired, I64, 5 * ncap, "fired", d),
+             read_only ? 1 : 0, cur_stream()),
+         "tree_serve_tiles");
 }
 
 int64_t tree_order_workspace(int64_t n) {
@@ -1194,6 +1291,17 @@
         "Tensor(c!)? tick=None, Tensor? slab=None, Tensor? slot_off=None) "
         "-> ()",
         &decode_replies_check);
+  m.def("decode_replies_tiles(Tensor buf, Tensor? n, int n_cap, "
+        "Tensor(a!) ws, Tensor(b!) frame_off, Tensor(c!) frame_len, "
+        "Tensor count, Tensor xid_tab, int xid_mask, Tensor(d!)[] out) -> ()",
+        &decode_replies_tiles);
+  m.def("decode_replies_check_tiles(Tensor buf, Tensor? n, int n_cap, "
+        "Tensor(a!) ws, Tensor(b!) frame_off, Tensor(c!) frame_len, "
+        "Tensor count, Tensor xid_tab, int xid_mask, Tensor(d!)[] out, "
+        "Tensor idx, Tensor xid, Tensor data_len, Tensor(e!) acc, "
+        "Tensor(f!)? tick=None, Tensor? slab=None, Tensor? slot_off=None) "
+        "-> ()",
+        &decode_replies_check_tiles);
   m.def("expand_strings(Tensor buf, Tensor region, Tensor count, "
         "Tensor base, Tensor(a!) str_off, Tensor(b!) str_len) -> ()",
         &expand_strings);
@@ -1224,6 +1332,12 @@
         "int session, int now_ms, int wslot=-1, Tensor(c!)? fired=None, "
         "Tensor? seqno=None, bool read_only=False) -> ()",
         &tree_serve_frames);
+  m.def("tree_serve_tiles(Tensor(a!)[] tree, Tensor rx, Tensor? n, "
+        "int n_cap, Tensor(b!) ws, Tensor(c!) frame_off, "
+        "Tensor(d!) frame_len, Tensor count, int ncap, Tensor(e!)[] out, "
+        "int session, int now_ms, int wslot=-1, Tensor(f!)? fired=None, "
+        "Tensor? seqno=None, bool read_only=False) -> ()",
+        &tree_serve_tiles);
   m.def("tree_order_workspace(int n) -> int", &tree_order_workspace);
   m.def("tree_order_stats_offset(int n) -> int", &tree_order_stats_offset);
   m.def("tree_serve_ordered(Tensor(a!)[] tree, Tensor rx, Tensor[] requests, "
diff --git a/zkmi/ops/batch.py b/zkmi/ops/batch.py
--- a/zkmi/ops/batch.py
+++ b/zkmi/ops/batch.py
@@ -259,6 +259,26 @@
                 'overflow': bool(r[3])}
 
 
+FS_DEFER = 1 << 24
+FS_TILE = 4096
+
+
+@dataclass
+class FrameTiles:
+    scanner: object
+    buf: torch.Tensor
+    n_dev: object
+    ncap: int
+    ws: torch.Tensor
+    table: object
+
+    def consumed(self):
+        sc = self.scanner
+        if sc.pending is self:
+            sc.pending = None
+            sc.clean_for = self.ncap
+
+
 FS_WINDOWS = (256, 512, 1024, 2048)
 FS_WIN_LONG = 1 << 16
 FS_WINDOW_AUTO_MAX = 2048
@@ -306,8 +326,10 @@
         self.ws = torch.empty(0, dtype=U8, device=device)
         self.ws_for = -1
         self.clean_for = -1
-
-    def scan(self, buf, n, stream=None, nospec=False, misspec=0):
+        self.pending = None
+        self.last_clean = False
+
+    def scan(self, buf, n, stream=None, nospec=False, misspec=0, rows=True):
         L = _lib.lib()
         n_dev, ncap = _scan_len(buf, n)
         if ncap > self.ws_for:
@@ -318,14 +340,24 @@
             self.ws_for = cover
             self.clean_for = -1
         t = self.table
+        if self.pending is not None:
+            self.pending = None
+            self.clean_for = -1
+        defer = not rows and ncap > FS_TILE
+        self.last_clean = ncap == self.clean_for
         with _on(stream):
             L.frame_scan(buf, n_dev, ncap, self.max_packet, self.ws, t.off,
                          t.length, t.result, int(self.window),
-                         ncap == self.clean_for,
+                         self.last_clean,
                          (1 if nospec else 0) | (int(misspec) << 8) |
-                         ((self.group - 1) << 4))
-        self.clean_for = ncap
+                         ((self.group - 1) << 4) |
+                         (FS_DEFER if defer else 0))
         self.last_cap = ncap
+        if defer:
+            self.clean_for = -1
+            self.pending = FrameTiles(self, buf, n_dev, ncap, self.ws, t)
+        else:
+            self.clean_for = ncap
         return t
 
     def chain_stats(self, stream=None):
@@ -401,12 +433,33 @@
 
 
 def decode_replies(buf, frames, xid_table, out=None, stream=None,
-                   check=None, tick=None):
+                   check=None, tick=None, tiles=None):
     L = _lib.lib()
     cap = frames.off.numel()
     if out is None:
         out = alloc_replies(cap, buf.device)
     out.count = frames.count
+    if tiles is not None:
+        if tiles.table is not frames or \
+                tiles.buf.data_ptr() != buf.data_ptr():
+            raise ValueError('decode_replies: tiles of another scan')
+        with _on(stream):
+            if check is None:
+                L.decode_replies_tiles(buf, tiles.n_dev, tiles.ncap, tiles.ws,
+                                       frames.off, frames.length,
+                                       frames.count, xid_table.tab,
+                                       xid_table.mask, out.tensors())
+            else:
+                idx, xid, data_len, acc = check[:4]
+                slab, slot_off = check[4:6] if len(check) > 4 else (None,
+                                                                    None)
+                L.decode_replies_check_tiles(
+                    buf, tiles.n_dev, tiles.ncap, tiles.ws, frames.off,
+                    frames.length, frames.count, xid_table.tab,
+                    xid_table.mask, out.tensors(), idx, xid, data_len, acc,
+                    tick, slab, slot_off)
+        tiles.consumed()
+        return out
     with _on(stream):
         if check is None:
             L.decode_replies(buf, frames.off, frames.length, frames.count,
```

New measurement: 2.102 billion, median of 6. +2.3%, better.
